# pinellolab/CRISPR-HAWK

Measured on AMD Instinct MI355X. Metric: candidate guides scored/sec, higher is better.
Workload: dtype u32

## Files before the change

### crispr-hawk_amd/crisprhawk_hip/_lib.py

```python

import ctypes as C
import os
from typing import Optional

_HERE = os.path.dirname(os.path.abspath(__file__))
LIB_PATH = os.environ.get("CRISPRHAWK_HIP_LIB", os.path.join(_HERE, "libhawk_hip.so"))

HAWK_OK = 0
HAWK_E_INVALID = -1
HAWK_E_HIP = -2
HAWK_E_CAPACITY = -3
HAWK_E_IUPAC = -4
HAWK_E_CFD = -5
HAWK_E_NODEVICE = -6
HAWK_E_UNSUPPORTED = -7
HAWK_E_COMM = -8
HAWK_E_OVERLAP = -9
HAWK_E_CLAMP = -10

EXPORTS = [
    "hawk_device_count", "hawk_init", "hawk_destroy", "hawk_strerror", "hawk_last_hip_error", "hawk_stream",
    "hawk_sync", "hawk_hapset_create", "hawk_hapset_destroy", "hawk_hapset_pack_ascii", "hawk_hapset_set_meta",
    "hawk_hapset_stride", "hawk_hapset_download_plane", "hawk_hapset_upload_planes", "hawk_pam_scan", "hawk_pam_scan_time",
    "hawk_search", "hawk_table_destroy", "hawk_table_counts", "hawk_table_download", "hawk_table_device_columns", "hawk_table_layout", "hawk_table_download_rows", "hawk_table_device_rows", "hawk_cfd",
    "hawk_genome_finalize", "hawk_offtarget_scan", "hawk_offtarget_summary", "hawk_deepcpf1", "hawk_azimuth", "hawk_tm_nn",
    "hawk_table_collapse", "hawk_table_collapse_download", "hawk_gt_parse", "hawk_gt_destroy", "hawk_gt_codes", "hawk_gt_lists",
    "hawk_gt_lists_download", "hawk_gt_lists_indels", "hawk_release_cached_memory", "hawk_xplan_run", "hawk_xplan_view", "hawk_xplan_cluster_stats", "hawk_xplan_cluster_rebuild", "hawk_host_gather_plan", "hawk_xplan_create_gt", "hawk_xplan_rows",
    "hawk_xplan_finish_meta", "hawk_xplan_segments", "hawk_xplan_install_meta", "hawk_host_alloc", "hawk_host_free", "hawk_hapset_rows_equal",
    "hawk_xplan_destroy", "hawk_hapset_set_ref_partner_range", "hawk_xplan_set_ref_partner_range", "hawk_table_collapse_ex", "hawk_table_collapse_export", "hawk_comm_unique_id", "hawk_comm_init",
    "hawk_comm_destroy", "hawk_comm_last_error", "hawk_comm_allgather_u64", "hawk_comm_gatherv", "hawk_table_gather", "hawk_host_ragged_join", "hawk_host_tsv_write", "hawk_host_vcf_index", "hawk_host_polish_rows", "hawk_host_variant_window", "hawk_host_polish_windows", "hawk_host_group_join", "hawk_host_group_samples", "hawk_gbt_predict", "hawk_gt_from_codes",
    "hawk_annot_create", "hawk_annot_query", "hawk_annot_download", "hawk_annot_free", "hawk_xplan_text",
]


class HawkLibraryError(RuntimeError):
    """libhawk_hip.so is missing or does not export the C ABI — build it (python -c
    'import __graft_entry__ as g; g.build()' or make -C crispr-hawk_amd/csrc)."""


class HawkDeviceError(RuntimeError):
    """No MI355X visible / HIP failure.  There is deliberately no CPU path."""


class HawkCommError(RuntimeError):
    """RCCL failure (or librccl.so missing) in the multi-GPU exchange."""


class HawkStatusError(RuntimeError):
    def __init__(self, status: int, where: str, detail: str = ""):
        self.status = status
        super().__init__(f"{where}: {strerror(status)} (status {status}){': ' + detail if detail else ''}")


class SearchParams(C.Structure):
    _fields_ = [
        ("pam_fwd", C.c_uint64), ("pam_rev", C.c_uint64), ("pamlen", C.c_uint32), ("guidelen", C.c_uint32),
        ("right", C.c_uint32), ("score_cfdon", C.c_uint32), ("cfd_mm", C.c_void_p), ("cfd_pam", C.c_void_p),
    ]


class Timing(C.Structure):
    _fields_ = [
        ("count_ms", C.c_float), ("offsets_ms", C.c_float), ("emit_ms", C.c_float), ("total_ms", C.c_float),
        ("scanned_positions", C.c_uint64), ("emit_list_ms", C.c_float), ("v_count_ms", C.c_float), ("v_emit_ms", C.c_float),
        ("v_templates_ms", C.c_float), ("v_path", C.c_uint32), ("v_emit_rows_ms", C.c_float), ("reserved", C.c_float),
    ]


class GbtModel(C.Structure):
    _fields_ = [("n_trees", C.c_uint32), ("n_nodes", C.c_uint32), ("tree_off", C.c_void_p), ("feature", C.c_void_p),
                ("left", C.c_void_p), ("right", C.c_void_p), ("threshold", C.c_void_p), ("value", C.c_void_p),
                ("init", C.c_double), ("learning_rate", C.c_double)]


class OtParams(C.Structure):
    _fields_ = [("pam_fwd", C.c_uint64), ("pam_rev", C.c_uint64), ("pamlen", C.c_uint32), ("guidelen", C.c_uint32),
                ("right", C.c_uint32), ("max_mm", C.c_uint32)]


class AnnotTiming(C.Structure):
    _fields_ = [("upload_ms", C.c_float), ("count_ms", C.c_float), ("scan_ms", C.c_float), ("fill_ms", C.c_float),
                ("reserved", C.c_float), ("total_ms", C.c_float), ("out_bytes", C.c_uint64), ("walk_steps", C.c_uint64)]


class OtTiming(C.Structure):
    _fields_ = [("scan_ms", C.c_float), ("sites_ms", C.c_float), ("match_ms", C.c_float), ("total_ms", C.c_float),
                ("n_sites", C.c_uint64), ("scanned_positions", C.c_uint64)]


_lib: Optional[C.CDLL] = None
_ctx = {}


def lib() -> C.CDLL:
    global _lib
    if _lib is None:
        if not os.path.exists(LIB_PATH):
            raise HawkLibraryError(f"{LIB_PATH} not found: the HIP extension has not been built")
        try:
            L = C.CDLL(LIB_PATH)
        except OSError as e:
            raise HawkLibraryError(f"cannot load {LIB_PATH}: {e}") from e
        missing = [s for s in EXPORTS if not hasattr(L, s)]
        if missing:
            raise HawkLibraryError(f"{LIB_PATH} lacks symbols {missing}")
        L.hawk_strerror.restype = C.c_char_p
        L.hawk_last_hip_error.restype = C.c_char_p
        L.hawk_stream.restype = C.c_void_p
        L.hawk_destroy.restype = None
        L.hawk_hapset_destroy.restype = None
# ... 112 lines not shown
```

### crispr-hawk_amd/crisprhawk_hip/hapset.py

```python

import ctypes as C
from dataclasses import dataclass
from typing import List, Optional, Sequence, Tuple

import numpy as np

from . import _lib

GUIDESEQPAD = 10
_CODE2CHAR = np.frombuffer(b"?ACMGRSVTWYHKDBN?acmgrsvtwyhkdbn", dtype=np.uint8)


def _p(a: Optional[np.ndarray]):
    return None if a is None else a.ctypes.data_as(C.c_void_p)


def _as_u8(seq) -> np.ndarray:
    if isinstance(seq, np.ndarray):
        return seq if seq.dtype == np.uint8 else seq.astype(np.uint8)
    if isinstance(seq, str):
        seq = seq.encode("ascii")
    return np.frombuffer(seq, dtype=np.uint8)


# ... 132 lines not shown
        nf, nr = int(off_f[-1]), int(off_r[-1])
        hf = np.empty(max(nf, 1), dtype=np.uint32)
        hr = np.empty(max(nr, 1), dtype=np.uint32)
        if rc == _lib.HAWK_E_CAPACITY:
            _lib.check(L.hawk_pam_scan(self._h, C.c_uint64(pam_bits), C.c_uint64(pam_bitsrc), pamlen, _p(hf), _p(hr),
                                       C.c_uint64(len(hf)), C.c_uint64(len(hr)), _p(off_f), _p(off_r)), "hawk_pam_scan")
        return [(hf[int(off_f[h]):int(off_f[h + 1])].copy(), hr[int(off_r[h]):int(off_r[h + 1])].copy())
                for h in range(self.n_hap)]

    def search(self, pam_bits: int, pam_bitsrc: int, pamlen: int, guidelen: int, right: bool,
               cfd_mm: Optional[np.ndarray] = None, cfd_pam: Optional[np.ndarray] = None,
               download: bool = True, collapse: bool = False, cfd_na_on_ambiguous: bool = False) -> "GuideTable":
        L = self._L
        sp = _lib.SearchParams()
        sp.pam_fwd, sp.pam_rev, sp.pamlen, sp.guidelen, sp.right = pam_bits, pam_bitsrc, pamlen, guidelen, int(bool(right))
        keep = []
        if cfd_mm is not None:
            mm = np.ascontiguousarray(cfd_mm, dtype=np.float64).reshape(20, 4, 4)
            pt = np.ascontiguousarray(cfd_pam, dtype=np.float64).reshape(16)
            keep = [mm, pt]
            sp.score_cfdon, sp.cfd_mm, sp.cfd_pam = (2 if cfd_na_on_ambiguous else 1), mm.ctypes.data, pt.ctypes.data
        t = C.c_void_p()
        tm = _lib.Timing()
        _lib.check(L.hawk_search(self._h, C.byref(sp), C.byref(t), C.byref(tm)), "hawk_search")
        del keep
        self.last_timing = tm
        tab = GuideTable(self, t, guidelen, pamlen, bool(right), tm)
        if collapse:
            tab.collapse()
        if download:
            tab.download()
        return tab


class ExpansionPlan:

    def __init__(self, handle, hap_len: np.ndarray, device: Optional[int] = None):
        self._L = _lib.lib()
        self._x = handle
        self.hap_len = np.asarray(hap_len, dtype=np.uint32)
        self.n_hap = len(self.hap_len)
        self.device = device
        self.ref_index = -1
        self.is_ref = None

    def run(self, want_hash: bool = False, timed: bool = False):
        handle = C.c_void_p()
        hashes = np.zeros((self.n_hap, 2), dtype=np.uint64) if want_hash else None
        ms = C.c_float(0)
        _lib.check(self._L.hawk_xplan_run(self._x, C.byref(handle), _p(hashes), C.byref(ms) if (timed or want_hash) else None),
                   "hawk_xplan_run")
        ds = DeviceHapSet.from_handle(handle, self.hap_len, self.device)
        ds.ref_index, ds.is_ref = self.ref_index, self.is_ref
        return ds, hashes, (ms.value if (timed or want_hash) else None)

    def view(self) -> "DeviceHapSet":
        v = getattr(self, "_view", None)
        if v is None or v._h is None:
            handle = C.c_void_p()
            _lib.check(self._L.hawk_xplan_view(self._x, C.byref(handle)), "hawk_xplan_view")
            v = DeviceHapSet.from_handle(handle, self.hap_len, self.device)
            v.ref_index, v.is_ref = self.ref_index, self.is_ref
            v._plan_ref = self
            for k in ("alias", "host_meta"):
                if hasattr(self, k):
                    setattr(v, k, getattr(self, k))
            self._view = v
        return v

    def text(self, rows=None, timed: bool = False):
        rows = np.arange(self.n_hap, dtype=np.uint32) if rows is None else np.ascontiguousarray(rows, dtype=np.uint32).reshape(-1)
        if len(rows) and int(rows.max()) >= self.n_hap:
            raise IndexError(f"row {int(rows.max())} of a plan of {self.n_hap} rows")
        off = np.zeros(len(rows) + 1, dtype=np.uint64)
        np.cumsum(self.hap_len[rows], dtype=np.uint64, out=off[1:])
        buf = _lib.pinned_empty(int(off[-1]), np.uint8, self.device)
        ms = C.c_float(0)
        _lib.check(self._L.hawk_xplan_text(self._x, len(rows), _p(rows), _p(off), _p(buf), C.byref(ms) if timed else None), "hawk_xplan_text")
        return (buf, off, ms.value) if timed else (buf, off)

    def rebuild_dictionary(self) -> None:
        _lib.check(self._L.hawk_xplan_cluster_rebuild(self._x), "hawk_xplan_cluster_rebuild")

    def cluster_stats(self) -> dict:
        u, ni, nd, st = C.c_uint32(), C.c_uint32(), C.c_uint32(), C.c_uint32()
        slots, ms = C.c_uint64(), C.c_float()
        _lib.check(self._L.hawk_xplan_cluster_stats(self._x, C.byref(u), C.byref(ni), C.byref(nd), C.byref(slots), C.byref(ms), C.byref(st)),
                   "hawk_xplan_cluster_stats")
        return {"usable": bool(u.value), "instances": ni.value, "distinct": nd.value, "template_slots": slots.value, "build_ms": ms.value,
                "status": st.value}

    def close(self) -> None:
        v = getattr(self, "_view", None)
        if v is not None:
            v._plan_ref = None
            v.close()
            self._view = None
        if getattr(self, "_x", None):
            self._L.hawk_xplan_destroy(self._x)
            self._x = None

    def __del__(self):
        try:
            self.close()
        except Exception:
            pass


def _meta_arrays(haps: Sequence["HostHaplotype"]):
    n = len(haps)
    is_ref = np.array([1 if h.is_ref else 0 for h in haps], dtype=np.uint8)
    ss = np.array([h.scan[0] for h in haps], dtype=np.int32)
    se = np.array([h.scan[1] for h in haps], dtype=np.int32)
    seg_off = np.zeros(n + 1, dtype=np.uint32)
    seg_off[1:] = np.cumsum([len(h.seg.rel) for h in haps])
    seg_rel = np.concatenate([h.seg.rel for h in haps]).astype(np.uint32)
    seg_gen = np.concatenate([h.seg.gen for h in haps]).astype(np.int64)
    refs = np.flatnonzero(is_ref)
    return is_ref, ss, se, seg_off, seg_rel, seg_gen, (int(refs[0]) if len(refs) else -1)


class GroupTable:

    def __init__(self, guidelen: int, pamlen: int, right: bool, n_groups: int, n_rows: int, device: Optional[int] = None):
        self.guidelen, self.pamlen, self.right, self.n_groups, self.n_rows = guidelen, pamlen, right, n_groups, n_rows
        ng = n_groups

        def pe(n, dt):
            return _lib.pinned_empty(n, dt, device)
        self.rep_row = pe(ng, np.uint32); self.pos = pe(ng, np.uint32); self.strand = np.empty(ng, np.uint8)
        self.start = pe(ng, np.int64); self.stop = pe(ng, np.int64); self.flags = np.empty(ng, np.uint8)
        self.cfdon = pe(ng, np.float64); self.win = pe(5 * ng, np.uint64).reshape(5, ng)
        self.member_hap = pe(n_rows, np.uint32)
        self.member_off = np.zeros(ng + 1, np.int64)
        self.gc_num = np.zeros(ng, np.uint8); self.gc_den = np.zeros(ng, np.uint8)

    @property
    def window_len(self) -> int:
        return self.guidelen + self.pamlen + 2 * GUIDESEQPAD

    def windows(self, rows: Optional[np.ndarray] = None) -> List[str]:
        return decode_windows(self.win if rows is None else self.win[:, rows], self.window_len)


def decode_windows(win: np.ndarray, W: int) -> List[str]:
    n = win.shape[1]
    if n == 0:
        return []
    sh = np.arange(W, dtype=np.uint64)
    code = np.zeros((n, W), dtype=np.uint8)
    for p in range(5):
        code |= (((win[p][:, None] >> sh) & np.uint64(1)).astype(np.uint8) << p)
    raw = _CODE2CHAR[code].tobytes()
    return [raw[i * W:(i + 1) * W].decode("ascii") for i in range(n)]


class GuideTable:

    def __init__(self, hs: DeviceHapSet, handle, guidelen: int, pamlen: int, right: bool, timing):
        self._hs, self._t = hs, handle
        self.guidelen, self.pamlen, self.right = guidelen, pamlen, right
        self._timing_struct = timing
        self.timing = {k: getattr(timing, k) for k, _ in timing._fields_}
        n, c, h = C.c_uint64(), C.c_uint64(), C.c_uint64()
        _lib.check(hs._L.hawk_table_counts(handle, C.byref(n), C.byref(c), C.byref(h)), "hawk_table_counts")
        self.n_rows, self.n_candidates, self.n_hits = n.value, c.value, h.value
# ... 101 lines not shown
```

### crispr-hawk_amd/csrc/hawk_api.hip

```cpp
#include <hip/hip_runtime.h>

#include <algorithm>
#include <cmath>
#include <cstdio>
#include <cstdlib>
#include <cstring>
#include <map>
#include <mutex>
#include <new>
#include <unordered_map>
#include <vector>

#include "hawk_host.h"

static thread_local char g_hip_err[256] = "";
char* hawk_hip_err_buf() { return g_hip_err; }

namespace {
struct DevPool {
  std::multimap<size_t, void*> free_;
  std::unordered_map<void*, size_t> live_;
  size_t cached = 0;
};
DevPool g_pool[HAWK_MAX_DEVICES];
// ... 34 lines not shown
    (void)hipGetLastError();
    pool_trim_locked(P);
    e = hipMalloc(p, want);
  }
  if (e != hipSuccess) {
    snprintf(g_hip_err, sizeof(g_hip_err), "hipMalloc(%zu bytes): %s", want, hipGetErrorString(e));
    *p = nullptr;
    return HAWK_E_HIP;
  }
  P->live_[*p] = want;
  return HAWK_OK;
}

void hawk_pool_free(void* p) {
  if (!p) return;
  std::lock_guard<std::mutex> g(g_pool_mu);
  for (int d = 0; d < HAWK_MAX_DEVICES; ++d) {
    DevPool* P = &g_pool[d];
    auto it = P->live_.find(p);
    if (it == P->live_.end()) continue;
    const size_t sz = it->second;
    P->live_.erase(it);
    if (P->cached + sz > pool_cap()) { (void)hipFree(p); return; }
    P->free_.emplace(sz, p);
    P->cached += sz;
    return;
  }
  (void)hipFree(p);
}

void hawk_pool_trim() {
  std::lock_guard<std::mutex> g(g_pool_mu);
  if (DevPool* P = cur_pool()) pool_trim_locked(P);
}

extern "C" {

const char* hawk_strerror(int s) {
  switch (s) {
    case HAWK_OK: return "ok";
    case HAWK_E_INVALID: return "invalid argument";
    case HAWK_E_HIP: return "HIP runtime error";
    case HAWK_E_CAPACITY: return "output capacity too small";
    case HAWK_E_IUPAC: return "non-IUPAC character in sequence";
    case HAWK_E_CFD: return "non-ACGT base under a CFD table lookup";
    case HAWK_E_NODEVICE: return "no GPU device visible";
    case HAWK_E_UNSUPPORTED: return "parameter outside supported range";
    case HAWK_E_COMM: return "RCCL failure";
    case HAWK_E_OVERLAP: return "a chromosome copy carries overlapping variants";
    case HAWK_E_CLAMP: return "variant beyond the original region length";
    default: return "unknown status";
  }
}
const char* hawk_last_hip_error(void) { return g_hip_err; }

int hawk_device_count(int* n) {
  int c = 0;
  hipError_t e = hipGetDeviceCount(&c);
  if (e != hipSuccess) { c = 0; (void)hipGetLastError(); }
  if (n) *n = c;
  return HAWK_OK;
}

namespace {
hawk_ctx* g_ctx_of[HAWK_MAX_DEVICES] = {};
int g_ctx_refs[HAWK_MAX_DEVICES] = {};
std::mutex g_ctx_mu;
}

int hawk_init(int device, hawk_ctx** out) {
  if (!out) return HAWK_E_INVALID;
  int c = 0;
  hawk_device_count(&c);
  if (c <= 0) return HAWK_E_NODEVICE;
  if (device < 0 || device >= c || device >= HAWK_MAX_DEVICES) return HAWK_E_INVALID;
  std::lock_guard<std::mutex> g(g_ctx_mu);
  if (g_ctx_of[device]) { ++g_ctx_refs[device]; *out = g_ctx_of[device]; return HAWK_OK; }
  HIPCHK(hipSetDevice(device));
  hawk_ctx* ctx = new (std::nothrow) hawk_ctx();
  if (!ctx) return HAWK_E_INVALID;
  ctx->device = device;
  HIPCHK(hipStreamCreateWithFlags(&ctx->stream, hipStreamNonBlocking));
  for (auto& e : ctx->ev) HIPCHK(hipEventCreate(&e));
  HIPCHK(hipHostMalloc(&ctx->pinned, 256, hipHostMallocDefault));
  g_ctx_of[device] = ctx; g_ctx_refs[device] = 1;
  *out = ctx;
  return HAWK_OK;
}

void hawk_destroy(hawk_ctx* ctx) {
  if (!ctx) return;
  {
    std::lock_guard<std::mutex> g(g_ctx_mu);
    const int d = ctx->device;
    if (d >= 0 && d < HAWK_MAX_DEVICES && g_ctx_of[d] == ctx) {
      if (--g_ctx_refs[d] > 0) return;
      g_ctx_of[d] = nullptr;
    }
  }
  (void)hipSetDevice(ctx->device);
  (void)hipStreamSynchronize(ctx->stream);
  for (auto& e : ctx->ev) (void)hipEventDestroy(e);
  (void)hipStreamDestroy(ctx->stream);
  if (ctx->pinned) (void)hipHostFree(ctx->pinned);
  delete ctx;
}

int hawk_host_alloc(hawk_ctx* ctx, uint64_t bytes, void** out) {
  if (!ctx || !out) return HAWK_E_INVALID;
  HIPCHK(hipSetDevice(ctx->device));
  HIPCHK(hipHostMalloc(out, std::max<uint64_t>(bytes, 1), hipHostMallocDefault));
  return HAWK_OK;
}
void hawk_host_free(void* p) { if (p) (void)hipHostFree(p); }

void* hawk_stream(hawk_ctx* ctx) { return ctx ? (void*)ctx->stream : nullptr; }
int hawk_sync(hawk_ctx* ctx) {
  if (!ctx) return HAWK_E_INVALID;
  HIPCHK(hipStreamSynchronize(ctx->stream));
  return HAWK_OK;
}

int hawk_release_cached_memory(hawk_ctx* ctx) {
  if (!ctx) return HAWK_E_INVALID;
  HIPCHK(hipSetDevice(ctx->device));
  HIPCHK(hipStreamSynchronize(ctx->stream));
  hawk_pool_trim();
  return HAWK_OK;
}

}
```

### crispr-hawk_amd/csrc/hawk_api_collapse.hip

```cpp
#include <hip/hip_runtime.h>

#include <algorithm>
#include <cmath>
#include <cstdio>
#include <cstdlib>
#include <cstring>
#include <map>
#include <mutex>
#include <new>
#include <unordered_map>
#include <vector>

#include "hawk_host.h"

extern "C" {

static int collapse_rows(hawk_table* t, uint32_t flank_up, uint32_t flank_down, uint64_t* n_groups, float* kernel_ms);
static int collapse_by_templates(hawk_table* t, uint32_t flank_up, uint32_t flank_down, uint64_t* n_groups, float* kernel_ms);
int hawk_table_collapse_ex(hawk_table* t, uint32_t flank_up, uint32_t flank_down, uint64_t* n_groups, float* kernel_ms) {
  if (!t || !n_groups || !t->hs || hawk_table_stale(t)) return HAWK_E_INVALID;
  if (flank_up > HAWK_PAD || flank_down > HAWK_PAD) return HAWK_E_UNSUPPORTED;
  if (t->by_cluster && t->n_rows) return collapse_by_templates(t, flank_up, flank_down, n_groups, kernel_ms);
  return collapse_rows(t, flank_up, flank_down, n_groups, kernel_ms);
}
// ... 46 lines not shown
          (rc = hs->ccnt.reserve(32)))
        return rc;
      for (int attempt = 0; attempt < 2; ++attempt) {
        unsigned long long hc[4] = {0, 0, 0, 0};
        HIPCHK(hipMemsetAsync(hs->ccnt.p, 0, 32, ctx->stream));
        HIPCHK(hipEventRecord(ctx->ev[0], ctx->stream));
        if (hawk_launch_collapse_hash1(ctx->stream, t->cols, hs->d_is_ref, n, (int)t->guidelen, (int)t->pamlen, (int)flank_up, (int)flank_down,
                                       hs->min_gen, 0x9e3779b97f4a7c15ull * (uint64_t)(attempt + 1), hs->ctemp.p, tb, hs->ctable.p, (uint32_t)C,
                                       hs->cocc.as<uint32_t>(), hs->cdense.as<uint32_t>(), hs->cgkey.as<uint64_t>(), hs->cgslot.as<uint32_t>(),
                                       hs->cflags.as<uint32_t>(), hs->ccnt.as<unsigned long long>()))
          return HAWK_E_HIP;
        HIPCHK(hipGetLastError());
        HIPCHK(hipMemcpyAsync(hc, hs->ccnt.p, 24, hipMemcpyDeviceToHost, ctx->stream));
        HIPCHK(hipStreamSynchronize(ctx->stream));
        if (hc[1]) { hs->last_groups = n; if (hs->plan_groups) *hs->plan_groups = n; break; }
        if (hc[0]) continue;
        const uint64_t ng = hc[2];
        if (hawk_launch_collapse_hash2(ctx->stream, t->cols, n, (uint32_t)ng, (int)t->guidelen, (int)t->pamlen, (int)t->right, end_bit, hs->ctemp.p, tb,
                                       hs->cgkey.as<uint64_t>(), hs->cgslot.as<uint32_t>(), (uint32_t)C, hs->cocc.as<uint32_t>(),
                                       hs->cflags.as<uint32_t>(), hs->ckeys.as<uint32_t>(), hs->cvals.as<uint32_t>(), hs->cgoff.as<uint64_t>(),
                                       hs->cgc.as<uint8_t>(), hs->cgc.as<uint8_t>() + n))
          return HAWK_E_HIP;
        if (verify) {
          if ((rc = hs->cfull.reserve(ng * 64 + 64))) return rc;
          hawk_launch_collapse_verify_rows(ctx->stream, t->cols, hs->d_is_ref, n, (uint32_t)ng, (int)t->guidelen, (int)t->pamlen, (int)flank_up,
                                           (int)flank_down, hs->cvals.as<uint32_t>() + n, hs->cflags.as<uint32_t>(), hs->cocc.as<uint32_t>(),
                                           hs->cgoff.as<uint64_t>(), hs->cfull.p, hs->ccnt.as<unsigned long long>() + 3);
        }
        HIPCHK(hipEventRecord(ctx->ev[1], ctx->stream));
        HIPCHK(hipGetLastError());
        HIPCHK(hipMemcpyAsync(hs->cgoff.as<uint64_t>() + ng, &n, 8, hipMemcpyHostToDevice, ctx->stream));
        HIPCHK(hipMemcpyAsync(&hc[3], hs->ccnt.as<unsigned long long>() + 3, 8, hipMemcpyDeviceToHost, ctx->stream));
        HIPCHK(hipStreamSynchronize(ctx->stream));
        if (kernel_ms) { float ms = 0.f; (void)hipEventElapsedTime(&ms, ctx->ev[0], ctx->ev[1]); *kernel_ms += ms; }
        if (hc[3]) { verified_bad = true; break; }
        hs->last_groups = ng;
        if (hs->plan_groups) *hs->plan_groups = ng;
        t->n_groups = ng; t->collapsed = true;
        *n_groups = ng;
        return HAWK_OK;
      }
    }
  }
  if (verified_bad) continue;
  unsigned long long cnt[3] = {0, 0, 0};
  for (int attempt = 0; attempt < 4; ++attempt) {
    HIPCHK(hipMemsetAsync(hs->ccnt.p, 0, 32, ctx->stream));
    HIPCHK(hipEventRecord(ctx->ev[0], ctx->stream));
    if (hawk_launch_collapse(ctx->stream, t->cols, hs->d_is_ref, n, (int)t->guidelen, (int)t->pamlen, (int)t->right, (int)flank_up,
                             (int)flank_down, hs->min_gen, exact ? 0u : begin_bit, end_bit, 0x9e3779b97f4a7c15ull * (uint64_t)(attempt + 1), hs->ctemp.p,
                             temp_bytes, hs->ckeys.as<uint64_t>(), hs->cvals.as<uint32_t>(), hs->cflags.as<uint32_t>(),
                             hs->cgidx.as<uint32_t>(), hs->ccnt.as<unsigned long long>(), hs->cgoff.as<uint64_t>(), hs->cgc.as<uint8_t>(),
                             hs->cgc.as<uint8_t>() + n, hs->cgidx.as<uint32_t>(), exact ? hs->cfull.p : nullptr, weak && !exact))
      return HAWK_E_HIP;
    if (verify && !exact)
      hawk_launch_collapse_verify(ctx->stream, t->cols, hs->d_is_ref, n, (int)t->guidelen, (int)t->pamlen, (int)flank_up, (int)flank_down,
                                  hs->cvals.as<uint32_t>() + n, hs->cgidx.as<uint32_t>(), hs->cflags.as<uint32_t>(), hs->cgoff.as<uint64_t>(),
                                  hs->ccnt.as<unsigned long long>() + 2);
    HIPCHK(hipEventRecord(ctx->ev[1], ctx->stream));
    HIPCHK(hipGetLastError());
    HIPCHK(hipMemcpyAsync(cnt, hs->ccnt.p, 24, hipMemcpyDeviceToHost, ctx->stream));
    HIPCHK(hipStreamSynchronize(ctx->stream));
    if (kernel_ms) { float ms = 0.f; (void)hipEventElapsedTime(&ms, ctx->ev[0], ctx->ev[1]); *kernel_ms += ms; }
    if (cnt[0] == cnt[1]) break;
  }
  if (cnt[0] != cnt[1]) { if (!exact) continue; return HAWK_E_UNSUPPORTED; }
  if (cnt[2]) continue;
  const uint64_t ng = cnt[1];
  HIPCHK(hipMemcpyAsync(hs->cgoff.as<uint64_t>() + ng, &n, 8, hipMemcpyHostToDevice, ctx->stream));
  HIPCHK(hipStreamSynchronize(ctx->stream));
  hs->last_groups = ng;
  if (hs->plan_groups) *hs->plan_groups = ng;
  t->n_groups = ng; t->collapsed = true;
  *n_groups = ng;
  return HAWK_OK;
  }
  return HAWK_E_UNSUPPORTED;
}

static int collapse_by_templates(hawk_table* t, uint32_t flank_up, uint32_t flank_down, uint64_t* n_groups, float* kernel_ms) {
  hawk_hapset* hs = t->hs;
  hawk_ctx* ctx = hs->ctx;
  HIPCHK(hipSetDevice(ctx->device));
  const hawk_xplan* vx = hs->vplan;
  if (!vx || !vx->cl.usable) return HAWK_E_INVALID;
  const uint64_t n = t->n_rows;
  if (n > 0xffffffffull) return HAWK_E_UNSUPPORTED;
  t->collapsed = false;
  *n_groups = 0;
  if (kernel_ms) *kernel_ms = 0.f;
  const uint32_t nu = vx->cl.n_uniq;
  PoolScope tmp;
  uint32_t* d_ucnt;
  uint64_t* d_moff;
  unsigned long long *d_partial, *d_shards;
  ScanTotals* d_tot;
  TEMPCHK(tmp, &d_ucnt, (size_t)std::max<uint32_t>(nu, 1) * 4);
  TEMPCHK(tmp, &d_moff, ((size_t)nu + 2) * 8);
  TEMPCHK(tmp, &d_partial, ((size_t)nu / 1024 + 2) * 8);
  TEMPCHK(tmp, &d_shards, 512 * 8);
  TEMPCHK(tmp, &d_tot, sizeof(ScanTotals));
  HIPCHK(hipMemsetAsync(d_shards, 0, 512 * 8, ctx->stream));
  HIPCHK(hipMemsetAsync(d_tot, 0, sizeof(ScanTotals), ctx->stream));
  uint64_t r0 = 0;
  ScanTotals tot;
  memset(&tot, 0, sizeof(tot));
  if (nu) {
    hawk_launch_cc_ucnt(ctx->stream, hs->cs_res.p, nu, d_ucnt);
    hawk_launch_mscan(ctx->stream, d_ucnt, nu, d_partial, d_shards, d_moff, d_tot);
    HIPCHK(hipMemcpyAsync(&tot, d_tot, sizeof(tot), hipMemcpyDeviceToHost, ctx->stream));
  }
  HIPCHK(hipMemcpyAsync(&r0, hs->offsets.as<uint64_t>() + t->plane_tiles, 8, hipMemcpyDeviceToHost, ctx->stream));
  HIPCHK(hipStreamSynchronize(ctx->stream));
  HIPCHK(hipGetLastError());
  const uint64_t t_live = tot.n_keep;
  const uint64_t nm = r0 + t_live;
  if (r0 > n || nm == 0 || nm > 0xffffffffull || r0 + 0 > n) return HAWK_E_INVALID;
  int rc;
  GuideCols mini;
  if ((rc = hawk_reserve_cols(hs->cmini, nm, &mini)) || (rc = hs->cm_gid.reserve(nm * 4))) return rc;
  float ms_a = 0.f, ms_b = 0.f, ms_c = 0.f;
  HIPCHK(hipEventRecord(ctx->ev[8], ctx->stream));
  hawk_launch_cc_mini(ctx->stream, t->cols, r0, hs->cs_trows.p, t_live, d_moff, hs->cs_tbase.as<uint32_t>(), nu, hs->ref_startp, mini);
  HIPCHK(hipEventRecord(ctx->ev[9], ctx->stream));
  HIPCHK(hipGetLastError());
  {
    const size_t tb_full = hawk_collapse_expand_temp_bytes(n);
    if ((rc = hs->ckeys.reserve(std::max<size_t>(2 * nm * 8, 2 * n * 4))) || (rc = hs->cvals.reserve(2 * n * 4)) ||
        (rc = hs->cgoff.reserve((nm + 1) * 8)) || (rc = hs->cgc.reserve(2 * n)) || (rc = hs->ctemp.reserve(tb_full + 16)) ||
        (rc = hs->cflags.reserve(n * 4)))
      return rc;
  }
  hawk_table tm;
  tm.hs = hs; tm.ctx = ctx; tm.n_rows = nm; tm.n_cand = tm.n_hits = 0; tm.cap = mini.cap; tm.cols = mini;
  tm.guidelen = t->guidelen; tm.pamlen = t->pamlen; tm.right = t->right; tm.n_groups = 0; tm.collapsed = false; tm.gen = t->gen;
  uint64_t G = 0;
  if ((rc = collapse_rows(&tm, flank_up, flank_down, &G, &ms_b))) return rc;
  HIPCHK(hipStreamSynchronize(ctx->stream));
  (void)hipEventElapsedTime(&ms_a, ctx->ev[8], ctx->ev[9]);
  unsigned gbits = 1;
  while (gbits < 32 && (G >> gbits) != 0) ++gbits;
  const size_t tb = hawk_collapse_expand_temp_bytes(n);
  HIPCHK(hipEventRecord(ctx->ev[8], ctx->stream));
  hawk_launch_cc_gidm(ctx->stream, hs->cvals.as<uint32_t>() + nm, hs->cgoff.as<uint64_t>(), nm, G, hs->cm_gid.as<uint32_t>());
  if ((rc = hs->ckeys.reserve(2 * n * 4)) || (rc = hs->cvals.reserve(2 * n * 4)) || (rc = hs->cgoff.reserve((std::max<uint64_t>(G, nm) + 1) * 8)) ||
      (rc = hs->cgc.reserve(2 * n)) || (rc = hs->ctemp.reserve(tb + 16)) || (rc = hs->cflags.reserve(n * 4)))
    return rc;
  ClDict cd;
  memset(&cd, 0, sizeof(cd));
  cd.n_inst = vx->cl.n_inst; cd.n_uniq = vx->cl.n_uniq; cd.inst_uid = vx->cl.inst_uid.as<uint32_t>();
  hawk_launch_cs_gid(ctx->stream, cd, hs->cs_res.p, d_moff, hs->offsets.as<uint64_t>() + t->plane_tiles, r0, n,
                     hs->cm_gid.as<uint32_t>(), hs->ckeys.as<uint32_t>(), hs->cvals.as<uint32_t>());
  if (hawk_launch_collapse_expand(ctx->stream, t->cols, n, gbits, (int)t->guidelen, (int)t->pamlen, (int)t->right, hs->ctemp.p, tb, hs->ckeys.as<uint32_t>(),
                                  hs->cvals.as<uint32_t>(), hs->cgoff.as<uint64_t>(), hs->cgc.as<uint8_t>(), hs->cgc.as<uint8_t>() + n))
    return HAWK_E_HIP;
  HIPCHK(hipMemcpyAsync(hs->cgoff.as<uint64_t>() + G, &n, 8, hipMemcpyHostToDevice, ctx->stream));
  HIPCHK(hipEventRecord(ctx->ev[9], ctx->stream));
  HIPCHK(hipGetLastError());
  HIPCHK(hipStreamSynchronize(ctx->stream));
  (void)hipEventElapsedTime(&ms_c, ctx->ev[8], ctx->ev[9]);
  if (kernel_ms) *kernel_ms = ms_a + ms_b + ms_c;
  hs->collapse_gen = t->gen;
  hs->last_groups = G;
  if (hs->plan_groups) *hs->plan_groups = G;
  t->n_groups = G; t->collapsed = true;
  *n_groups = G;
  return HAWK_OK;
// ... 62 lines not shown
```

### crispr-hawk_amd/csrc/hawk_api_search.hip

```cpp
#include <hip/hip_runtime.h>

#include <algorithm>
#include <cmath>
#include <cstdio>
#include <cstdlib>
#include <cstring>
#include <map>
#include <mutex>
#include <new>
#include <unordered_map>
#include <vector>

#include "hawk_host.h"

int hawk_reserve_cols(DevBuf (&b)[8], uint64_t cap, GuideCols* c) {
  int rc;
  const size_t sz[8] = {cap * 4, cap * 4, cap, cap * 8, cap * 8, cap, cap * 8, cap * 8 * HAWK_PLANES};
  for (int i = 0; i < 8; ++i) if ((rc = b[i].reserve(std::max<size_t>(sz[i], 16)))) return rc;
  c->hap = b[0].as<uint32_t>(); c->pos = b[1].as<uint32_t>(); c->strand = b[2].as<uint8_t>();
  c->start = b[3].as<int64_t>(); c->stop = b[4].as<int64_t>(); c->flags = b[5].as<uint8_t>();
  c->cfdon = b[6].as<double>(); c->win = b[7].as<uint64_t>(); c->cap = cap;
  c->rows = nullptr; c->startp = 0;
  return HAWK_OK;
}

#define HAWK_RETRY_TEMPLATES (-100)

enum SearchEvent {
  EV_BEGIN, EV_COUNT_DONE, EV_OFFSETS_DONE, EV_EMIT_BEGIN, EV_EMIT_END, EV_LIST_EMIT_END,
  EV_VIEW_COUNT_BEGIN, EV_VIEW_EMIT_BEGIN,
  EV_TEMPLATES_DONE, EV_REF_ROWS_PACKED,
  EV_SLOTS
};
static_assert(EV_SLOTS == sizeof(hawk_ctx::ev) / sizeof(hipEvent_t), "hawk_ctx::ev holds exactly the search's events");

struct SearchRun {
  hawk_hapset* hs; hawk_ctx* ctx; hipStream_t st;
  const hawk_xplan* vx;
  bool by_cluster;
  HapSetDev d; ScanParams sp; GuideParams gp; RefInfo ri; VcArgs va; ClDict cd;
  uint64_t ntile, nscan;
  uint32_t plane_tiles, v_tiles;
  uint64_t tcap, t_rows_used;
  uint64_t stage_cap;
  unsigned long long* shards;
  SearchStatusBlock* blk;
  SearchStatusBlock* h;
  uint64_t* table_cap;
};

static int search_classify(hawk_hapset* hs, const hawk_search_params* p, SearchRun* r) {
  if (!hs || !p || !hs->has_meta || p->score_cfdon > 2) return HAWK_E_INVALID;
  if (p->score_cfdon && (p->right || !p->cfd_mm || !p->cfd_pam || p->pamlen < 2)) return HAWK_E_INVALID;
  r->hs = hs; r->ctx = hs->ctx; r->st = hs->ctx->stream; r->vx = hs->vplan;
  HIPCHK(hipSetDevice(r->ctx->device));
  const int rc = make_scan_params(hs, p->pam_fwd, p->pam_rev, p->pamlen, p->guidelen, p->right, true, &r->sp);
  if (rc) return rc;
  r->d = make_dev(hs);
  ++hs->cols_gen;
  const hawk_xplan* vx = r->vx;
  if (vx && (hs->ref_index != 0 || hs->n_ref_rows != 1)) return HAWK_E_INVALID;
  r->by_cluster = vx && vx->cl.built && vx->cl.usable;
  if (r->by_cluster) { const char* e = getenv("HAWK_VIEW_SEARCH"); if (e && e[0] == 'w') r->by_cluster = false; }
  r->ntile = (uint64_t)hs->n_hap * r->sp.bph;
  r->nscan = r->by_cluster ? (uint64_t)r->sp.bph + ((uint64_t)vx->cl.n_inst + 63) / 64 : r->ntile;
  r->plane_tiles = vx ? r->sp.bph : (uint32_t)r->ntile;
  r->v_tiles = (uint32_t)r->ntile - r->plane_tiles;
  r->stage_cap = r->by_cluster ? 2ull * hs->hap_len[hs->ref_index] + 64 : 0;
  r->table_cap = r->by_cluster ? &hs->rows_cap : &hs->cols_cap;
  r->tcap = r->t_rows_used = 0;
  return HAWK_OK;
}
static int search_reserve(SearchRun* r, const hawk_search_params* p) {
  hawk_hapset* hs = r->hs;
  const ScanParams& sp = r->sp;
  const uint64_t n_ref_tiles = (uint64_t)sp.bph * hs->n_ref_rows;
  int rc;
  if ((rc = hs->counts.reserve(r->nscan * 4)) || (rc = hs->offsets.reserve((r->nscan + 1) * 8)) || (rc = hs->misc.reserve(sizeof(SearchMisc))) ||
      (rc = hs->cfd.reserve(336 * 8)) || (rc = hs->partial.reserve((r->nscan / 1024 + 2) * 8)) ||
      (rc = hs->lists.reserve((size_t)r->plane_tiles * HAWK_LIST_CAP * 4 + 16)) || (rc = hs->big.reserve(((size_t)r->plane_tiles + 128 * n_ref_tiles) * 8 + 16)))
    return rc;
  r->shards = &hs->misc.as<SearchMisc>()->shards[0][0];
  r->blk = &hs->misc.as<SearchMisc>()->blk;
  r->h = static_cast<SearchStatusBlock*>(r->ctx->pinned);
  GuideParams& gp = r->gp;
  gp.pamlen = sp.pamlen; gp.guidelen = sp.guidelen; gp.right = sp.right; gp.L = sp.L;
  gp.score_cfdon = (int32_t)p->score_cfdon;
  gp.cfd_mm = hs->cfd.as<double>(); gp.cfd_pam = hs->cfd.as<double>() + 320; gp.bph = sp.bph;
  return HAWK_OK;
}
static int search_upload_cfd(SearchRun* r, const hawk_search_params* p) {
  hawk_hapset* hs = r->hs;
  if (!p->score_cfdon) return HAWK_OK;
  if (hs->cfd_host.size() == 336 && memcmp(hs->cfd_host.data(), p->cfd_mm, 320 * 8) == 0 && memcmp(hs->cfd_host.data() + 320, p->cfd_pam, 16 * 8) == 0) return HAWK_OK;
  hs->cfd_host.assign(336, 0.0);
  memcpy(hs->cfd_host.data(), p->cfd_mm, 320 * 8);
  memcpy(hs->cfd_host.data() + 320, p->cfd_pam, 16 * 8);
  HIPCHK(hipMemcpyAsync(hs->cfd.p, hs->cfd_host.data(), 336 * 8, hipMemcpyHostToDevice, r->st));
  HIPCHK(hipStreamSynchronize(r->st));
  return HAWK_OK;
}
static int search_ref(SearchRun* r, const hawk_search_params* p) {
  hawk_hapset* hs = r->hs;
  const ScanParams& sp = r->sp;
  RefInfo& ri = r->ri;
  ri.index = hs->ref_index; ri.startp = hs->ref_startp;
  ri.bits[0] = ri.bits[1] = nullptr; ri.n_bits = 0;
  for (int s = 0; s < 2; ++s) {
    ri.lo[s] = 0; ri.hi[s] = 0;
    if (hs->ref_index < 0) continue;
    const bool pamfirst = (sp.right != 0) != (s != 0);
    const int po = pamfirst ? 0 : sp.guidelen;
    const int haplen = (int)hs->hap_len[hs->ref_index];
    const int rs = hs->has_partner ? hs->partner_start : hs->scan_start[hs->ref_index];
    const int re = hs->has_partner ? hs->partner_stop : hs->scan_stop[hs->ref_index];
    ri.lo[s] = std::max(rs - po, HAWK_PAD);
    ri.hi[s] = std::min(re - po, haplen - sp.L - HAWK_PAD + 1);
  }
  if (hs->ref_index < 0) return HAWK_OK;
  const uint64_t key[6] = {p->pam_fwd, p->pam_rev, ((uint64_t)p->pamlen << 32) | p->guidelen, (uint64_t)(p->right ? 1 : 0),
                           ((uint64_t)(uint32_t)ri.lo[0] << 32) | (uint32_t)ri.hi[0], ((uint64_t)(uint32_t)ri.lo[1] << 32) | (uint32_t)ri.hi[1]};
  int rc;
  if ((rc = hs->refbits.reserve((size_t)hs->S * 4 * 2))) return rc;
  ri.bits[0] = hs->refbits.as<uint32_t>(); ri.bits[1] = hs->refbits.as<uint32_t>() + hs->S;
  ri.n_bits = hs->S * 32u;
  if (r->vx && ((rc = hs->refhp.reserve(((size_t)hs->S + 1) * 8 * 2)) || (rc = hs->vcnt0.reserve(r->by_cluster ? 16 : r->ntile * 4)))) return rc;
  if (hs->refbits_valid && memcmp(hs->refbits_key, key, sizeof(key)) == 0) return HAWK_OK;
  hawk_launch_ref_bits(r->st, r->d, sp, ri, hs->refbits.as<uint32_t>(), hs->refbits.as<uint32_t>() + hs->S);
  if (r->vx) hawk_launch_ref_hits(r->st, r->d, sp, hs->ref_index, hs->refhp.p);
  HIPCHK(hipGetLastError());
  memcpy(hs->refbits_key, key, sizeof(key));
  hs->refbits_valid = true;
  return HAWK_OK;
}
static int search_view_args(SearchRun* r) {
  hawk_hapset* hs = r->hs;
  const hawk_xplan* vx = r->vx;
  VcArgs& va = r->va; ClDict& cd = r->cd;
  memset(&va, 0, sizeof(va)); memset(&cd, 0, sizeof(cd));
  if (!vx) return HAWK_OK;
  for (int pl = 0; pl < 4; ++pl) va.ref[pl] = vx->ref5[pl].as<uint32_t>();
  va.ref_S = hs->S; va.hp = hs->refhp.as<uint4>();
  va.recs_ = vx->recs.p; va.alt_codes = vx->codes.as<uint8_t>(); va.hv_off = vx->off.as<uint64_t>(); va.tiles_ = vx->tiles.p;
  if (!r->by_cluster) return HAWK_OK;
  const auto& cl = vx->cl;
  cd.n_inst = cl.n_inst; cd.n_uniq = cl.n_uniq;
  cd.inst_uid = cl.inst_uid.as<uint32_t>(); cd.inst_o = cl.inst_o.as<int32_t>(); cd.inst_row = cl.inst_row.as<uint32_t>();
  cd.inst_pa = cl.inst_pa.as<int32_t>(); cd.inst_rb = cl.inst_rb.as<int32_t>();
  cd.u_rec = cl.u_rec.as<uint32_t>(); cd.u_n = cl.u_n.as<uint32_t>(); cd.u_row = cl.u_row.as<uint32_t>(); cd.u_o = cl.u_o.as<int32_t>();
  cd.u_seg = cl.u_seg.as<uint32_t>();
  const char* e0 = getenv("HAWK_CLUSTER_ROWS0");
  const uint64_t first = e0 ? strtoull(e0, nullptr, 10) : 16ull * cl.n_uniq + 65536;
  r->tcap = std::max<uint64_t>(std::min<uint64_t>(cl.slots, std::max<uint64_t>(hs->cs_tcap, first)), 1);
  const size_t n_uniq = std::max<uint32_t>(cl.n_uniq, 1), n_inst = std::max<uint32_t>(cl.n_inst, 1);
  int rc;
  if ((rc = hs->cs_res.reserve(n_uniq * 32)) || (rc = hs->cs_tbase.reserve(n_uniq * 4)) || (rc = hs->cs_trows.reserve((size_t)r->tcap * hawk_cs_row_bytes())) ||
      (rc = hs->cs_itb.reserve(n_inst * 4)) || (rc = hs->cs_icnt.reserve(n_inst * 4)))
    return rc;
  return HAWK_OK;
}
static int search_count(SearchRun* r) {
  hawk_hapset* hs = r->hs; hipStream_t st = r->st; hipEvent_t* ev = r->ctx->ev;
  SearchStatusBlock* blk = r->blk; uint32_t* counts = hs->counts.as<uint32_t>();
  HIPCHK(hipEventRecord(ev[EV_BEGIN], st));
  hawk_launch_search(st, 0, r->d, r->sp, r->gp, r->ri, hs->d_tile_meta, counts, r->shards, nullptr, GuideCols{}, &blk->status, hs->lists.as<uint32_t>(),
                     &blk->big_count, hs->big.as<unsigned long long>(), nullptr, r->plane_tiles);
  if (r->vx) HIPCHK(hipEventRecord(ev[EV_VIEW_COUNT_BEGIN], st));
  if (r->by_cluster) {
    hawk_launch_cs_templates(st, r->d, r->va, r->cd, r->sp, r->gp, r->ri, hs->cs_res.p, hs->cs_tbase.as<uint32_t>(), hs->cs_trows.p, &blk->template_rows,
                             r->tcap, &blk->status);
    (void)hipEventRecord(ev[EV_TEMPLATES_DONE], st);
    hawk_launch_cs_count(st, r->d, r->va, r->cd, r->sp, hs->cs_res.p, &blk->template_rows, r->tcap, counts + r->plane_tiles, hs->cs_icnt.as<uint32_t>(),
                         hs->cs_itb.as<uint32_t>(), r->shards);
  } else if (r->vx) {
    hawk_launch_vsearch(st, 0, r->d, r->va, r->sp, r->gp, r->ri, hs->d_tile_meta, counts, hs->vcnt0.as<uint32_t>(), r->shards, nullptr, GuideCols{}, &blk->status,
                        r->plane_tiles, r->v_tiles);
  }
  HIPCHK(hipEventRecord(ev[EV_COUNT_DONE], st));
  hawk_launch_mscan(st, counts, r->nscan, hs->partial.as<unsigned long long>(), r->shards, hs->offsets.as<uint64_t>(), &blk->totals);
  HIPCHK(hipEventRecord(ev[EV_OFFSETS_DONE], st));
  HIPCHK(hipGetLastError());
  return HAWK_OK;
}
static int search_reserve_table(SearchRun* r, uint64_t cap, GuideCols* cols, GuideCols* table) {
  hawk_hapset* hs = r->hs;
  int rc;
  if ((rc = hawk_reserve_cols(hs->colsA, r->by_cluster ? r->stage_cap : cap, cols))) return rc;
  *table = *cols;
  if (!r->by_cluster) return HAWK_OK;
  if ((rc = hs->rowsA.reserve(cap * 64))) return rc;
  memset(table, 0, sizeof(*table));
  table->rows = hs->rowsA.as<uint4>(); table->cap = cap; table->startp = r->ri.startp;
  return HAWK_OK;
}
static int search_emit(SearchRun* r, const GuideCols& cols, const GuideCols& packed, bool launch) {
  hawk_hapset* hs = r->hs; hipStream_t st = r->st; hipEvent_t* ev = r->ctx->ev;
  SearchStatusBlock* blk = r->blk; const uint64_t* offsets = hs->offsets.as<uint64_t>();
  HIPCHK(hipEventRecord(ev[EV_EMIT_BEGIN], st));
  if (launch) {
    hawk_launch_search(st, 1, r->d, r->sp, r->gp, r->ri, hs->d_tile_meta, hs->counts.as<uint32_t>(), r->shards, offsets, cols, &blk->status, hs->lists.as<uint32_t>(),
                       &blk->big_count, hs->big.as<unsigned long long>(), ev[EV_LIST_EMIT_END], r->plane_tiles);
    if (r->vx) (void)hipEventRecord(ev[EV_VIEW_EMIT_BEGIN], st);
    if (r->by_cluster) {
      hawk_launch_rows_pack(st, cols, offsets + r->plane_tiles, 0, std::min<uint64_t>(r->stage_cap, packed.cap), packed.rows, packed.startp, &blk->status);
      (void)hipEventRecord(ev[EV_REF_ROWS_PACKED], st);
      hawk_launch_cs_emit_rows(st, r->cd, hs->cs_icnt.as<uint32_t>(), hs->cs_itb.as<uint32_t>(), hs->cs_trows.p, offsets + r->plane_tiles, &blk->template_rows,
                               r->tcap, packed.rows, packed.cap, &blk->status);
    } else if (r->vx) {
      hawk_launch_vsearch(st, 1, r->d, r->va, r->sp, r->gp, r->ri, hs->d_tile_meta, hs->counts.as<uint32_t>(), hs->vcnt0.as<uint32_t>(), r->shards, offsets, cols,
                          &blk->status, r->plane_tiles, r->v_tiles);
    }
  }
  HIPCHK(hipEventRecord(ev[EV_EMIT_END], st));
  HIPCHK(hipGetLastError());
  return HAWK_OK;
}
static int search_read_block(SearchRun* r) {
  HIPCHK(hipMemcpyAsync(r->h, r->blk, sizeof(SearchStatusBlock), hipMemcpyDeviceToHost, r->st));
  HIPCHK(hipStreamSynchronize(r->st));
  if (!r->by_cluster) return HAWK_OK;
  const uint64_t tcu = r->h->template_rows;
  if (tcu > r->tcap) { r->hs->cs_tcap = std::min<uint64_t>(r->vx->cl.slots, tcu + tcu / 8 + 64); return HAWK_RETRY_TEMPLATES; }
  r->t_rows_used = tcu;
  return HAWK_OK;
}

static void search_timing(const SearchRun* r, uint64_t nrows, hawk_timing* timing) {
  const hawk_hapset* hs = r->hs; hipEvent_t* ev = r->ctx->ev;
  memset(timing, 0, sizeof(*timing));
  (void)hipEventElapsedTime(&timing->count_ms, ev[EV_BEGIN], ev[EV_COUNT_DONE]);
  (void)hipEventElapsedTime(&timing->offsets_ms, ev[EV_COUNT_DONE], ev[EV_OFFSETS_DONE]);
  (void)hipEventElapsedTime(&timing->emit_ms, ev[EV_EMIT_BEGIN], ev[EV_EMIT_END]);
  if (nrows) (void)hipEventElapsedTime(&timing->emit_list_ms, ev[EV_EMIT_BEGIN], ev[EV_LIST_EMIT_END]);
  (void)hipEventElapsedTime(&timing->total_ms, ev[EV_BEGIN], ev[EV_EMIT_END]);
  if (r->vx) {
    (void)hipEventElapsedTime(&timing->v_count_ms, ev[EV_VIEW_COUNT_BEGIN], ev[EV_COUNT_DONE]);
    if (nrows) (void)hipEventElapsedTime(&timing->v_emit_ms, ev[EV_VIEW_EMIT_BEGIN], ev[EV_EMIT_END]);
    timing->v_path = r->by_cluster ? 2u : 1u;
    if (r->by_cluster) (void)hipEventElapsedTime(&timing->v_templates_ms, ev[EV_VIEW_COUNT_BEGIN], ev[EV_TEMPLATES_DONE]);
    if (r->by_cluster && nrows) (void)hipEventElapsedTime(&timing->v_emit_rows_ms, ev[EV_REF_ROWS_PACKED], ev[EV_EMIT_END]);
  }
  uint64_t pos = 0;
  for (uint32_t h = 0; h < hs->n_hap; ++h) pos += (uint64_t)std::max(0, hs->scan_stop[h] - hs->scan_start[h]);
  timing->scanned_positions = pos;
}

static int search_make_table(const SearchRun* r, const hawk_search_params* p, const GuideCols& tc, hawk_table** out) {
  hawk_table* t = new (std::nothrow) hawk_table();
  if (!t) return HAWK_E_INVALID;
  const ScanTotals& tot = r->h->totals;
  t->hs = r->hs; t->ctx = r->ctx; t->gen = r->hs->cols_gen;
  t->n_rows = tot.n_keep; t->n_cand = tot.n_cand; t->n_hits = tot.n_hits; t->cols = tc; t->cap = tc.cap;
  t->guidelen = p->guidelen; t->pamlen = p->pamlen; t->right = p->right ? 1 : 0; t->n_groups = 0; t->collapsed = false;
  t->by_cluster = r->by_cluster; t->plane_tiles = r->plane_tiles; t->t_rows = r->by_cluster ? r->t_rows_used : 0;
  *out = t;
  return HAWK_OK;
}

static int hawk_search_once(hawk_hapset* hs, const hawk_search_params* p, hawk_table** out, hawk_timing* timing) {
  if (!out) return HAWK_E_INVALID;
  SearchRun r;
  int rc;
  if ((rc = search_classify(hs, p, &r)) || (rc = search_reserve(&r, p)) || (rc = search_upload_cfd(&r, p))) return rc;
  HIPCHK(hipMemsetAsync(r.hs->misc.p, 0, sizeof(SearchMisc), r.st));
  if ((rc = search_ref(&r, p)) || (rc = search_view_args(&r)) || (rc = search_count(&r))) return rc;
  uint64_t& table_cap = *r.table_cap;
  const bool speculative = table_cap != 0;
  GuideCols cols, table;
  if (speculative && ((rc = search_reserve_table(&r, table_cap, &cols, &table)) || (rc = search_emit(&r, cols, table, true)))) return rc;
  if ((rc = search_read_block(&r))) return rc;
  const uint64_t nrows = r.h->totals.n_keep;
  if (!speculative || nrows > table_cap) {
    const int status = r.h->status;
    if (status && !(speculative && status == HAWK_E_CAPACITY)) return status;
    if (speculative) HIPCHK(hipMemsetAsync(&r.blk->status, 0, sizeof(int), r.st));
    if ((rc = search_reserve_table(&r, std::max<uint64_t>(std::max<uint64_t>(nrows, 1), table_cap), &cols, &table))) return rc;
    table_cap = table.cap;
    if ((rc = search_emit(&r, cols, table, nrows != 0))) return rc;
    HIPCHK(hipMemcpyAsync(&r.h->status, &r.blk->status, sizeof(int), hipMemcpyDeviceToHost, r.st));
    HIPCHK(hipStreamSynchronize(r.st));
  }
  if (timing) search_timing(&r, nrows, timing);
  if (r.h->status) return r.h->status;
  return search_make_table(&r, p, table, out);
}

extern "C" {

int hawk_search(hawk_hapset* hs, const hawk_search_params* p, hawk_table** out, hawk_timing* timing) {
  int rc = hawk_search_once(hs, p, out, timing);
  if (rc == HAWK_RETRY_TEMPLATES) rc = hawk_search_once(hs, p, out, timing);
  return rc == HAWK_RETRY_TEMPLATES ? HAWK_E_CAPACITY : rc;
}

void hawk_table_destroy(hawk_table* t) {
  if (!t) return;
  if (!t->hs) {
    (void)hipSetDevice(t->ctx->device);
    (void)hipStreamSynchronize(t->ctx->stream);
    for (auto& b : t->own) b.release();
  }
  delete t;
}

int hawk_table_counts(const hawk_table* t, uint64_t* n_rows, uint64_t* n_candidates, uint64_t* n_hits) {
  if (!t) return HAWK_E_INVALID;
  if (n_rows) *n_rows = t->n_rows;
  if (n_candidates) *n_candidates = t->n_cand;
  if (n_hits) *n_hits = t->n_hits;
  return HAWK_OK;
}

int hawk_table_download(hawk_table* t, uint32_t* hap, uint32_t* pos, uint8_t* strand, int64_t* start, int64_t* stop,
                        uint8_t* flags, double* cfdon, uint64_t* win) {
  if (!t || hawk_table_stale(t)) return HAWK_E_INVALID;
  hawk_ctx* ctx = t->ctx;
  HIPCHK(hipSetDevice(ctx->device));
  const uint64_t n = t->n_rows;
  if (!n) return HAWK_OK;
  GuideCols c = t->cols;
  PoolScope tmp;
  if (c.rows) {
    GuideCols u;
    memset(&u, 0, sizeof(u));
    u.cap = n;
    if (hap) TEMPCHK(tmp, &u.hap, n * 4);
    if (pos) TEMPCHK(tmp, &u.pos, n * 4);
    if (strand) TEMPCHK(tmp, &u.strand, n);
    if (start) TEMPCHK(tmp, &u.start, n * 8);
    if (stop) TEMPCHK(tmp, &u.stop, n * 8);
    if (flags) TEMPCHK(tmp, &u.flags, n);
    if (cfdon) TEMPCHK(tmp, &u.cfdon, n * 8);
    if (win) TEMPCHK(tmp, &u.win, n * 8 * HAWK_PLANES);
    hawk_launch_rows_unpack(ctx->stream, c.rows, n, c.startp, u);
    HIPCHK(hipGetLastError());
    c = u;
  }
  if (hap) HIPCHK(hipMemcpyAsync(hap, c.hap, n * 4, hipMemcpyDefault, ctx->stream));
  if (pos) HIPCHK(hipMemcpyAsync(pos, c.pos, n * 4, hipMemcpyDefault, ctx->stream));
  if (strand) HIPCHK(hipMemcpyAsync(strand, c.strand, n, hipMemcpyDefault, ctx->stream));
  if (start) HIPCHK(hipMemcpyAsync(start, c.start, n * 8, hipMemcpyDefault, ctx->stream));
  if (stop) HIPCHK(hipMemcpyAsync(stop, c.stop, n * 8, hipMemcpyDefault, ctx->stream));
  if (flags) HIPCHK(hipMemcpyAsync(flags, c.flags, n, hipMemcpyDefault, ctx->stream));
  if (cfdon) HIPCHK(hipMemcpyAsync(cfdon, c.cfdon, n * 8, hipMemcpyDefault, ctx->stream));
  if (win)
    for (int p = 0; p < HAWK_PLANES; ++p)
      HIPCHK(hipMemcpyAsync(win + (size_t)p * n, c.win + (size_t)p * c.cap, n * 8, hipMemcpyDefault, ctx->stream));
  HIPCHK(hipStreamSynchronize(ctx->stream));
  return HAWK_OK;
}

int hawk_table_layout(const hawk_table* t, uint32_t* layout, int64_t* startp) {
  if (!t || !layout) return HAWK_E_INVALID;
  *layout = t->cols.rows ? HAWK_LAYOUT_ROWS : HAWK_LAYOUT_COLUMNS;
  if (startp) *startp = t->cols.rows ? t->cols.startp : 0;
  return HAWK_OK;
}

int hawk_table_download_rows(hawk_table* t, void* rows64) {
  if (!t || hawk_table_stale(t) || !rows64) return HAWK_E_INVALID;
  if (!t->cols.rows) return HAWK_E_UNSUPPORTED;
  HIPCHK(hipSetDevice(t->ctx->device));
  if (t->n_rows) HIPCHK(hipMemcpyAsync(rows64, t->cols.rows, t->n_rows * 64, hipMemcpyDefault, t->ctx->stream));
  HIPCHK(hipStreamSynchronize(t->ctx->stream));
  return HAWK_OK;
}

int hawk_table_device_rows(hawk_table* t, void** rows64, int64_t* startp) {
  if (!t || hawk_table_stale(t) || !rows64) return HAWK_E_INVALID;
  if (!t->cols.rows) return HAWK_E_UNSUPPORTED;
  *rows64 = t->cols.rows;
  if (startp) *startp = t->cols.startp;
  return HAWK_OK;
}

// ... 19 lines not shown
```

### crispr-hawk_amd/csrc/hawk_api_xplan.hip

```cpp
#include <hip/hip_runtime.h>

#include <algorithm>
#include <cmath>
#include <cstdio>
#include <cstdlib>
#include <cstring>
#include <map>
#include <mutex>
#include <new>
#include <unordered_map>
#include <vector>

#include "hawk_host.h"

enum XplanEvent { EV_KERNELS_BEGIN = 0, EV_KERNELS_END = 1, EV_BUILD_BEGIN = 8, EV_BUILD_END = 9 };

extern "C" {

void hawk_xplan_destroy(hawk_xplan* x) {
  if (!x) return;
  (void)hipSetDevice(x->ctx->device);
  (void)hipStreamSynchronize(x->ctx->stream);
  for (auto& p : x->ref_plane) hawk_pool_free(p);
  for (auto& b : x->ref5) b.release();
  DevBuf* bufs[] = {&x->recs, &x->heads, &x->tiles, &x->codes, &x->off, &x->hlen, &x->hash,
                    &x->m_is_ref, &x->m_ss, &x->m_se, &x->m_seg_off, &x->m_seg_rel, &x->m_seg_gen, &x->m_tile,
                    &x->cl.inst_uid, &x->cl.inst_o, &x->cl.inst_row, &x->cl.inst_pa, &x->cl.inst_rb, &x->cl.u_rec, &x->cl.u_n, &x->cl.u_row,
                    &x->cl.u_o, &x->cl.u_seg};
  for (auto* b : bufs) b->release();
  delete x;
}

static int xplan_build(hawk_hapset* ref_set, uint32_t n_var, const uint32_t* v_r0, const uint32_t* v_span, const uint32_t* v_alt_off,
                       const uint32_t* v_alt_len, const uint8_t* alt_codes, uint32_t alt_codes_len, uint32_t n_hap, const uint64_t* hv_off,
                       const uint32_t* d_idx, const int32_t* d_o, const uint32_t* hap_len, uint32_t maxlen, hawk_xplan** out) {
  hawk_ctx* ctx = ref_set->ctx;
  const uint32_t ref_len = ref_set->hap_len[0];
  const uint64_t ncar = hv_off[n_hap];
  HIPCHK(hipSetDevice(ctx->device));
  hawk_xplan* x = new (std::nothrow) hawk_xplan();
  if (!x) return HAWK_E_INVALID;
  x->ctx = ctx; x->n_var = n_var; x->n_hap = n_hap; x->ref_len = ref_len; x->ncar = ncar;
  x->hap_len.assign(hap_len, hap_len + n_hap);
  x->has_meta = false; x->nseg = 0; x->ref_index = -1; x->ref_startp = 0; x->min_gen = 0; x->max_gen = 0;
  for (auto& p : x->ref_plane) p = nullptr;
  x->ref_S = ref_set->S;
  x->S = ((maxlen + 31) / 32 + 2 + 3) / 4 * 4;
  x->bph = (x->S / 4 + HAWK_BLOCK - 1) / HAWK_BLOCK;
  const size_t nwg = (size_t)n_hap * hawk_hx_tiles_per_row(x->S);
  const size_t nv = std::max<size_t>(n_var, 1), nc = std::max<size_t>(ncar, 1);
  int rc = HAWK_OK;
  for (int p = 0; p < 4 && !rc; ++p) rc = hawk_pool_alloc((void**)&x->ref_plane[p], (size_t)x->ref_S * 4);
  DevBuf t_r0, t_span, t_ao, t_al, t_am;
  DevBuf* temps[] = {&t_r0, &t_span, &t_ao, &t_al, &t_am};
  if (!rc) rc = t_r0.reserve(nv * 4);
  if (!rc) rc = t_span.reserve(nv * 4);
  if (!rc) rc = t_ao.reserve(nv * 4);
  if (!rc) rc = t_al.reserve(nv * 4);
  if (!rc) rc = t_am.reserve(nv * 16);
  if (!rc) rc = x->recs.reserve(nc * hawk_hx_record_bytes());
  if (!rc) rc = x->heads.reserve(nc * 16);
  if (!rc) rc = x->tiles.reserve(nwg * hawk_hx_tile_bytes());
  if (!rc) rc = x->codes.reserve(std::max<size_t>(alt_codes_len, 1));
  if (!rc) rc = x->off.reserve((size_t)(n_hap + 1) * 8);
  if (!rc) rc = x->hlen.reserve((size_t)n_hap * 4);
  if (!rc) rc = x->hash.reserve((size_t)n_hap * 16);
  for (int p = 0; p < HAWK_PLANES && !rc; ++p) rc = x->ref5[p].reserve((size_t)x->S * 4);
  if (rc) { for (auto* b : temps) b->release(); hawk_xplan_destroy(x); return rc; }
  hipStream_t st = ctx->stream;
  hipError_t e = hipSuccess;
  for (int p = 0; p < HAWK_PLANES && e == hipSuccess; ++p) {
    e = hipMemsetAsync(x->ref5[p].p, 0, (size_t)x->S * 4, st);
    if (p < 4 && e == hipSuccess)
      e = hipMemcpyAsync(x->ref5[p].p, ref_set->plane[p], (size_t)std::min(x->S, x->ref_S) * 4, hipMemcpyDeviceToDevice, st);
  }
  std::vector<uint32_t> am(nv * 4, 0);
  for (uint32_t i = 0; i < n_var; ++i)
    for (uint32_t j = 0; j < v_alt_len[i] && j < 32; ++j) {
      const uint8_t c = alt_codes[v_alt_off[i] + j];
      for (int pl = 0; pl < 4; ++pl) am[(size_t)i * 4 + pl] |= (uint32_t)((c >> pl) & 1u) << j;
    }
  for (int p = 0; p < 4 && e == hipSuccess; ++p)
    e = hipMemcpyAsync(x->ref_plane[p], ref_set->plane[p], (size_t)x->ref_S * 4, hipMemcpyDeviceToDevice, st);
  if (n_var && e == hipSuccess) {
    e = hipMemcpyAsync(t_r0.p, v_r0, (size_t)n_var * 4, hipMemcpyHostToDevice, st);
    if (e == hipSuccess) e = hipMemcpyAsync(t_span.p, v_span, (size_t)n_var * 4, hipMemcpyHostToDevice, st);
    if (e == hipSuccess) e = hipMemcpyAsync(t_ao.p, v_alt_off, (size_t)n_var * 4, hipMemcpyHostToDevice, st);
    if (e == hipSuccess) e = hipMemcpyAsync(t_al.p, v_alt_len, (size_t)n_var * 4, hipMemcpyHostToDevice, st);
    if (e == hipSuccess) e = hipMemcpyAsync(x->codes.p, alt_codes, alt_codes_len, hipMemcpyHostToDevice, st);
    if (e == hipSuccess) e = hipMemcpyAsync(t_am.p, am.data(), (size_t)n_var * 16, hipMemcpyHostToDevice, st);
  }
  if (e == hipSuccess) e = hipMemcpyAsync(x->off.p, hv_off, (size_t)(n_hap + 1) * 8, hipMemcpyHostToDevice, st);
  if (e == hipSuccess) e = hipMemcpyAsync(x->hlen.p, hap_len, (size_t)n_hap * 4, hipMemcpyHostToDevice, st);
  if (e == hipSuccess) {
    hawk_launch_hx_prepare(st, x->off.as<uint64_t>(), d_idx, d_o, ncar, t_r0.as<uint32_t>(), t_span.as<uint32_t>(), t_ao.as<uint32_t>(),
                           t_al.as<uint32_t>(), t_am.p, x->hlen.as<uint32_t>(), n_hap, x->S, x->recs.p, x->tiles.p);
    hawk_launch_hx_heads(st, x->recs.p, d_idx, ncar, x->heads.p);
    e = hipGetLastError();
  }
  if (e == hipSuccess) e = hipStreamSynchronize(st);
  for (auto* b : temps) b->release();
  if (e != hipSuccess) {
    snprintf(hawk_hip_err_buf(), 256, "hawk_xplan_create_gt: %s", hipGetErrorString(e));
    hawk_xplan_destroy(x);
    return HAWK_E_HIP;
  }
  *out = x;
  return HAWK_OK;
}

int hawk_xplan_set_ref_partner_range(hawk_xplan* x, int32_t start, int32_t stop) {
  if (!x || !x->has_meta || x->ref_index < 0) return HAWK_E_INVALID;
  if (start < 0 || stop > (int32_t)x->hap_len[x->ref_index] || stop < start) return HAWK_E_INVALID;
  x->has_partner = true; x->partner_start = start; x->partner_stop = stop;
  return HAWK_OK;
}

static int xplan_install(const hawk_xplan* x, hawk_hapset* hs) {
  if (!x->has_meta || hs->n_hap != x->n_hap || hs->S != x->S) return HAWK_E_INVALID;
  hipStream_t st = x->ctx->stream;
  const uint32_t n = x->n_hap;
  hawk_pool_free(hs->d_seg_rel); hs->d_seg_rel = nullptr;
  hawk_pool_free(hs->d_seg_gen); hs->d_seg_gen = nullptr;
  int rc = hawk_pool_alloc((void**)&hs->d_seg_rel, (size_t)x->nseg * 4);
  if (!rc) rc = hawk_pool_alloc((void**)&hs->d_seg_gen, (size_t)x->nseg * 8);
  if (rc) return rc;
  HIPCHK(hipMemcpyAsync(hs->d_is_ref, x->m_is_ref.p, n, hipMemcpyDeviceToDevice, st));
  HIPCHK(hipMemcpyAsync(hs->d_scan_start, x->m_ss.p, (size_t)n * 4, hipMemcpyDeviceToDevice, st));
  HIPCHK(hipMemcpyAsync(hs->d_scan_stop, x->m_se.p, (size_t)n * 4, hipMemcpyDeviceToDevice, st));
  HIPCHK(hipMemcpyAsync(hs->d_seg_off, x->m_seg_off.p, (size_t)(n + 1) * 4, hipMemcpyDeviceToDevice, st));
  HIPCHK(hipMemcpyAsync(hs->d_seg_rel, x->m_seg_rel.p, (size_t)x->nseg * 4, hipMemcpyDeviceToDevice, st));
  HIPCHK(hipMemcpyAsync(hs->d_seg_gen, x->m_seg_gen.p, (size_t)x->nseg * 8, hipMemcpyDeviceToDevice, st));
  HIPCHK(hipMemcpyAsync(hs->d_tile_meta, x->m_tile.p, (size_t)n * x->bph * sizeof(TileMeta), hipMemcpyDeviceToDevice, st));
  hs->ref_startp = x->ref_startp; hs->min_gen = x->min_gen; hs->max_gen = x->max_gen;
  hs->scan_start = x->scan_start; hs->scan_stop = x->scan_stop;
  hs->ref_index = x->ref_index; hs->has_meta = true; hs->n_ref_rows = x->n_ref_rows;
  hs->plan_groups = x->groups; hs->last_groups = *x->groups;
  hs->has_partner = x->has_partner; hs->partner_start = x->partner_start; hs->partner_stop = x->partner_stop;
  hs->refbits_valid = false;
  ++hs->cols_gen;
  return HAWK_OK;
}

int hawk_xplan_run(hawk_xplan* x, hawk_hapset** out, uint64_t* hash_out, float* kernel_ms) {
  if (!x || !out) return HAWK_E_INVALID;
  hawk_ctx* ctx = x->ctx;
  hawk_hapset* hs = nullptr;
  int rc = hapset_create_impl(ctx, x->n_hap, x->hap_len.data(), false, &hs);
  if (rc) return rc;
  if (hs->S != x->S) { hawk_hapset_destroy(hs); return HAWK_E_INVALID; }
  hipStream_t st = ctx->stream;
  hipError_t e = hipMemsetAsync(x->hash.p, 0, (size_t)x->n_hap * 16, st);
  if (e == hipSuccess) e = hipEventRecord(ctx->ev[EV_KERNELS_BEGIN], st);
  if (e == hipSuccess) {
    hawk_launch_hx_build(st, x->ref_plane, x->ref_S, x->recs.p, x->codes.as<uint8_t>(), x->off.as<uint64_t>(), hs->d_hap_len, x->n_hap,
                         hs->S, hs->plane, x->tiles.p);
    if (hash_out) hawk_launch_hx_hash(st, hs->plane, x->n_hap, hs->S, x->hash.as<unsigned long long>());
    e = hipEventRecord(ctx->ev[EV_KERNELS_END], st);
  }
  if (e == hipSuccess) e = hipGetLastError();
  if (e == hipSuccess && hash_out) e = hipMemcpyAsync(hash_out, x->hash.p, (size_t)x->n_hap * 16, hipMemcpyDeviceToHost, st);
  if (e == hipSuccess && x->has_meta) {
    rc = xplan_install(x, hs);
    if (rc) { hawk_hapset_destroy(hs); return rc; }
  }
  if (e == hipSuccess && (hash_out || kernel_ms)) e = hipStreamSynchronize(st);
  if (e != hipSuccess) {
    snprintf(hawk_hip_err_buf(), 256, "hawk_xplan_run: %s", hipGetErrorString(e));
    hawk_hapset_destroy(hs);
    return HAWK_E_HIP;
  }
  if (kernel_ms) (void)hipEventElapsedTime(kernel_ms, ctx->ev[EV_KERNELS_BEGIN], ctx->ev[EV_KERNELS_END]);
  *out = hs;
  return HAWK_OK;
}

static int xplan_build_dict(hawk_xplan* x) {
  auto& cl = x->cl;
  if (cl.built) return HAWK_OK;
  cl.built = true; cl.usable = false; cl.status = 0; cl.n_inst = cl.n_uniq = cl.n_real = 0; cl.slots = 0; cl.build_ms = 0.f;
  hawk_ctx* ctx = x->ctx;
  hipStream_t st = ctx->stream;
  const uint32_t n = x->n_hap;
  if (x->ncar == 0 || x->ncar >= (1ull << 32) - 2 || n < 2) { cl.status = 4; return HAWK_OK; }
  PoolScope tmp;
  const uint32_t n_var = x->n_var;
  const uint32_t ch_bound = hawk_cl_chunk_bound(x->ncar, n);
  const uint32_t inst_bound = (uint32_t)x->ncar + n;
  const uint32_t bm_words = n_var / 32 + 1;
  uint32_t tsize = 1024;
  while (tsize < 2u * inst_bound && tsize < (1u << 30)) tsize <<= 1;
  uint32_t tsmall = std::min<uint32_t>(1u << 16, tsize);
  { const uint64_t expect = cl.last_uniq ? (uint64_t)cl.last_uniq * 2 : (uint64_t)inst_bound / 8; while (tsmall < expect && tsmall < tsize) tsmall <<= 1; }
  const uint32_t u_bound0 = n_var + std::min<uint32_t>(tsmall, inst_bound);
  auto up = [](size_t v) { return (v + 255) & ~(size_t)255; };
  const size_t z_status = 0, z_counters = 256, z_results = 512, z_cnt = 768,
               z_claim = z_cnt + up(((size_t)ch_bound + 4) * 8), z_vdesc = z_claim + up((size_t)bm_words * 4),
               z_span2 = z_vdesc + up((size_t)std::max<uint32_t>(n_var, 1) * 8), z_tab = z_span2 + up((size_t)u_bound0 * 4),
               z_end = z_tab + (size_t)tsmall * hawk_cl_slot_bytes();
  char* d_zero;
  TEMPCHK(tmp, &d_zero, z_end);
  uint32_t* const d_status = reinterpret_cast<uint32_t*>(d_zero + z_status);
  uint32_t* const d_counters = reinterpret_cast<uint32_t*>(d_zero + z_counters);
  unsigned long long* const d_results = reinterpret_cast<unsigned long long*>(d_zero + z_results);
  uint32_t* const d_cnt = reinterpret_cast<uint32_t*>(d_zero + z_cnt);
  uint32_t* const d_lcnt = d_cnt + ((ch_bound + 3) & ~3u);
  uint32_t* const d_claim = reinterpret_cast<uint32_t*>(d_zero + z_claim);
  void* const d_vdesc = d_zero + z_vdesc;
  uint32_t *d_ch_off, *d_ch_row, *d_base, *d_lbase, *d_state;
  void* d_list;
  TEMPCHK(tmp, &d_ch_off, (size_t)(n + 1) * 4);
  TEMPCHK(tmp, &d_ch_row, (size_t)ch_bound * 4);
  TEMPCHK(tmp, &d_base, (size_t)(ch_bound + 1) * 4);
  TEMPCHK(tmp, &d_lbase, (size_t)(ch_bound + 1) * 4);
  TEMPCHK(tmp, &d_list, (size_t)inst_bound * hawk_cl_listed_bytes());
  TEMPCHK(tmp, &d_state, (size_t)inst_bound * 4);
  int rc;
  if ((rc = cl.inst_uid.reserve((size_t)inst_bound * 4)) || (rc = cl.inst_o.reserve((size_t)inst_bound * 4)) ||
      (rc = cl.inst_row.reserve((size_t)inst_bound * 4)) || (rc = cl.inst_pa.reserve((size_t)inst_bound * 4)) ||
      (rc = cl.inst_rb.reserve((size_t)inst_bound * 4)))
    return rc;
  uint32_t* const t_uid = cl.inst_uid.as<uint32_t>();
  uint32_t* const t_row = cl.inst_row.as<uint32_t>();
  int32_t* const t_o = cl.inst_o.as<int32_t>();
  int32_t* const t_pa = cl.inst_pa.as<int32_t>();
  int32_t* const t_rb = cl.inst_rb.as<int32_t>();
  HIPCHK(hipEventRecord(ctx->ev[EV_BUILD_BEGIN], st));
  HIPCHK(hipMemsetAsync(d_zero, 0, z_end, st));
  hawk_launch_cl_chunks(st, x->off.as<uint64_t>(), x->m_is_ref.as<uint8_t>(), x->m_ss.as<int32_t>(), x->m_se.as<int32_t>(), n, d_ch_off, d_ch_row);
  hawk_launch_cl_count(st, x->heads.p, x->off.as<uint64_t>(), x->hlen.as<uint32_t>(), x->m_ss.as<int32_t>(), x->m_se.as<int32_t>(), d_ch_off, d_ch_row, n,
                       n_var, ch_bound, d_cnt, d_lcnt);
  hawk_launch_scan2_u32(st, d_cnt, d_lcnt, ch_bound, d_base, d_lbase);
  const uint32_t* const d_n_inst = d_base + ch_bound;
  const uint32_t* const d_n_list = d_lbase + ch_bound;
  unsigned long long res[8] = {0, 0, 0, 0, 0, 0, 0, 0};
  uint32_t status = 0, n_inst = 0, n_uniq = 0, n_real = 0;
  auto pass = [&](uint32_t tsz, uint32_t max_probe, uint32_t fail_bit, bool first) -> int {
    const uint32_t u_bound = n_var + std::min<uint32_t>(tsz, inst_bound);
    uint32_t* d_span2 = reinterpret_cast<uint32_t*>(d_zero + z_span2);
    void* d_tab = d_zero + z_tab;
    if (!first) {
      TEMPCHK(tmp, &d_span2, (size_t)u_bound * 4);
      TEMPCHK(tmp, &d_tab, (size_t)tsz * hawk_cl_slot_bytes());
      HIPCHK(hipMemsetAsync(d_tab, 0, (size_t)tsz * hawk_cl_slot_bytes(), st));
      HIPCHK(hipMemsetAsync(d_span2, 0, (size_t)u_bound * 4, st));
      HIPCHK(hipMemsetAsync(d_zero + z_counters, 0, z_cnt - z_counters, st));
      HIPCHK(hipMemsetAsync(d_zero + z_claim, 0, z_span2 - z_claim, st));
    }
    int rc2;
    if ((rc2 = cl.u_rec.reserve((size_t)u_bound * 4)) || (rc2 = cl.u_n.reserve((size_t)u_bound * 4)) || (rc2 = cl.u_row.reserve((size_t)u_bound * 4)) ||
        (rc2 = cl.u_o.reserve((size_t)u_bound * 4)) || (rc2 = cl.u_seg.reserve((size_t)u_bound * 4)))
      return rc2;
    hawk_launch_cl_fill(st, x->heads.p, x->off.as<uint64_t>(), x->hlen.as<uint32_t>(), x->m_ss.as<int32_t>(), x->m_se.as<int32_t>(), n, d_ch_off, d_ch_row,
                        ch_bound, d_base, d_lbase, t_o, t_row, t_pa, t_rb, t_uid, d_vdesc, d_claim, n_var, d_list, d_status);
    hawk_launch_cl_finish(st, inst_bound, d_n_inst, d_n_list, d_counters, d_results, n_var, u_bound, d_tab, tsz - 1, max_probe, fail_bit, d_list, d_state, d_vdesc, x->heads.p,
                          t_uid, t_row, x->m_seg_off.as<uint32_t>(), x->m_seg_rel.as<uint32_t>(), cl.u_rec.as<uint32_t>(), cl.u_n.as<uint32_t>(),
                          cl.u_row.as<uint32_t>(), cl.u_o.as<int32_t>(), cl.u_seg.as<uint32_t>(), d_span2, d_status);
    HIPCHK(hipMemcpyAsync(res, d_results, 64, hipMemcpyDeviceToHost, st));
    HIPCHK(hipEventRecord(ctx->ev[EV_BUILD_END], st));
    HIPCHK(hipStreamSynchronize(st));
    HIPCHK(hipGetLastError());
    n_inst = (uint32_t)res[0]; status = (uint32_t)res[4];
    n_uniq = std::min<uint32_t>(n_var + (uint32_t)res[1], u_bound);
    n_real = (uint32_t)(res[1] + res[2]);
    return HAWK_OK;
  };
  if ((rc = pass(tsmall, tsmall < tsize ? 64u : 0xffffffffu, tsmall < tsize ? 8u : 2u, true))) return rc;
  if (status & 8u) {
    status &= ~8u;
    HIPCHK(hipMemcpyAsync(d_status, &status, 4, hipMemcpyHostToDevice, st));
    if ((rc = pass(tsize, 0xffffffffu, 2u, false))) return rc;
  }
  if (n_inst == 0) { cl.status = 4; return HAWK_OK; }
  if (n_inst > inst_bound) { snprintf(hawk_hip_err_buf(), 256, "hawk_xplan_view: instance count beyond its bound"); return HAWK_E_HIP; }
  cl.n_inst = n_inst; cl.n_uniq = n_uniq; cl.n_real = n_real; cl.last_uniq = (uint32_t)res[1];
  (void)hipEventElapsedTime(&cl.build_ms, ctx->ev[EV_BUILD_BEGIN], ctx->ev[EV_BUILD_END]);
  cl.slots = n_uniq ? res[3] : 0;
  cl.status = status;
  const char* e1 = getenv("HAWK_CLUSTER_MAX_SLOTS");
  const char* e2 = getenv("HAWK_CLUSTER_MIN_SHARE");
  const uint64_t max_slots = e1 ? strtoull(e1, nullptr, 10) : (1ull << 27);
  const double min_share = e2 ? atof(e2) : 3.0;
  if (!status && (cl.slots > max_slots || (double)n_inst < min_share * (double)std::max<uint32_t>(n_real, 1))) cl.status = 4;
  cl.usable = cl.status == 0;
  return HAWK_OK;
}

int hawk_xplan_cluster_stats(const hawk_xplan* x, uint32_t* usable, uint32_t* n_instances, uint32_t* n_distinct, uint64_t* template_slots,
                             float* build_ms, uint32_t* status) {
  if (!x) return HAWK_E_INVALID;
  if (usable) *usable = x->cl.built && x->cl.usable ? 1u : 0u;
  if (n_instances) *n_instances = x->cl.n_inst;
  if (n_distinct) *n_distinct = x->cl.n_real;
  if (template_slots) *template_slots = x->cl.slots;
  if (build_ms) *build_ms = x->cl.build_ms;
  if (status) *status = x->cl.built ? x->cl.status : 0xffffffffu;
  return HAWK_OK;
}

int hawk_xplan_cluster_rebuild(hawk_xplan* x) {
  if (!x || !x->has_meta || x->ref_index != 0) return HAWK_E_INVALID;
  HIPCHK(hipSetDevice(x->ctx->device));
  x->cl.built = false;
  return xplan_build_dict(x);
}

int hawk_xplan_view(hawk_xplan* x, hawk_hapset** out) {
  if (!x || !out || !x->has_meta || x->ref_index != 0) return HAWK_E_INVALID;
  hawk_ctx* ctx = x->ctx;
  hawk_hapset* hs = nullptr;
  int rc = hapset_create_impl(ctx, x->n_hap, x->hap_len.data(), false, &hs, false);
  if (rc) return rc;
  if (hs->S != x->S) { hawk_hapset_destroy(hs); return HAWK_E_INVALID; }
  hs->vplan = x;
  for (int p = 0; p < HAWK_PLANES; ++p) hs->plane[p] = x->ref5[p].as<uint32_t>();
  rc = xplan_install(x, hs);
  if (!rc && hipStreamSynchronize(ctx->stream) != hipSuccess) rc = HAWK_E_HIP;
  if (!rc) rc = xplan_build_dict(x);
  if (rc) { hs->vplan = nullptr; for (int p = 0; p < HAWK_PLANES; ++p) hs->plane[p] = nullptr; hawk_hapset_destroy(hs); return rc; }
  *out = hs;
  return HAWK_OK;
}

int hawk_xplan_install_meta(hawk_xplan* x, hawk_hapset* hs) {
  if (!x || !hs || hs->vplan) return HAWK_E_INVALID;
  HIPCHK(hipSetDevice(x->ctx->device));
  int rc = xplan_install(x, hs);
  if (rc) return rc;
  HIPCHK(hipStreamSynchronize(x->ctx->stream));
  return HAWK_OK;
}

int hawk_xplan_create_gt(hawk_hapset* ref_set, hawk_gt* g, uint32_t n_var, const uint32_t* v_r0, const uint32_t* v_span,
                         const uint32_t* v_alt_off, const uint32_t* v_alt_len, const int32_t* v_chain, const uint8_t* alt_codes,
                         uint32_t alt_codes_len, int64_t startp, int check_clamp, int64_t rev_g0, int64_t rev_g1, uint32_t* n_hap_out,
                         hawk_xplan** out) {
  if (!ref_set || !g || !out || !n_hap_out || !g->d_col_off || g->n_var != n_var || !n_var || !v_r0 || !v_span || !v_alt_off || !v_alt_len ||
      !v_chain || !alt_codes)
    return HAWK_E_INVALID;
  hawk_ctx* ctx = ref_set->ctx;
  if (g->ctx != ctx) return HAWK_E_INVALID;
  const uint32_t ref_len = ref_set->hap_len[0];
  for (uint32_t i = 0; i < n_var; ++i) {
    if ((uint64_t)v_r0[i] + v_span[i] > ref_len || v_span[i] == 0 || v_alt_len[i] == 0) return HAWK_E_INVALID;
    if ((uint64_t)v_alt_off[i] + v_alt_len[i] > alt_codes_len) return HAWK_E_INVALID;
    if (i && v_r0[i] < v_r0[i - 1]) return HAWK_E_INVALID;
    if ((int64_t)v_chain[i] != (int64_t)v_alt_len[i] - (int64_t)v_span[i]) return HAWK_E_INVALID;
  }
  const uint32_t n_cols = 2 * g->n_samples;
  std::vector<uint64_t> hv_off(2, 0), ioff(2, 0);
  std::vector<uint32_t> hap_len(1, ref_len);
  uint32_t maxlen = ref_len;
  for (uint32_t c = 0; c < n_cols; ++c) {
    if (g->h_off[c + 1] == g->h_off[c]) continue;
    const int64_t len = (int64_t)ref_len + g->h_delta[c];
    if (len <= 0 || len >= (int64_t)((1u << 31) - 256)) return HAWK_E_UNSUPPORTED;
    hv_off.push_back(g->h_off[c + 1]);
    ioff.push_back(g->h_ioff[c + 1]);
    hap_len.push_back((uint32_t)len);
    maxlen = std::max(maxlen, (uint32_t)len);
  }
  const uint32_t n_hap = (uint32_t)hap_len.size();
  *n_hap_out = n_hap;
  hawk_xplan* x = nullptr;
  int rc = xplan_build(ref_set, n_var, v_r0, v_span, v_alt_off, v_alt_len, alt_codes, alt_codes_len, n_hap, hv_off.data(), g->d_idx, g->d_o,
                       hap_len.data(), maxlen, &x);
  if (rc) return rc;
  hipStream_t st = ctx->stream;
  DevBuf t_r0, t_span, t_ch, t_ioff, t_cnt, t_status, t_rev;
  DevBuf* temps[] = {&t_r0, &t_span, &t_ch, &t_ioff, &t_cnt, &t_status, &t_rev};
  auto done = [&](int code) { for (auto* b : temps) b->release(); if (code) hawk_xplan_destroy(x); return code; };
  if ((rc = t_r0.reserve((size_t)n_var * 4)) || (rc = t_span.reserve((size_t)n_var * 4)) || (rc = t_ch.reserve((size_t)n_var * 4)) ||
      (rc = t_ioff.reserve((size_t)(n_hap + 1) * 8)) || (rc = t_cnt.reserve((size_t)n_hap * 4)) || (rc = t_status.reserve(16)) ||
      (rc = t_rev.reserve((size_t)n_hap * 16)) || (rc = x->m_seg_off.reserve((size_t)(n_hap + 1) * 4)))
    return done(rc);
#define HIPCHK_X(expr)                                                                         \
  do {                                                                                         \
    hipError_t e_ = (expr);                                                                    \
    if (e_ != hipSuccess) {                                                                    \
      snprintf(hawk_hip_err_buf(), 256, "%s: %s (%s:%d)", #expr, hipGetErrorString(e_), __FILE__, __LINE__); \
      return done(HAWK_E_HIP);                                                                 \
    }                                                                                          \
  } while (0)
  HIPCHK_X(hipMemcpyAsync(t_r0.p, v_r0, (size_t)n_var * 4, hipMemcpyHostToDevice, st));
  HIPCHK_X(hipMemcpyAsync(t_span.p, v_span, (size_t)n_var * 4, hipMemcpyHostToDevice, st));
  HIPCHK_X(hipMemcpyAsync(t_ch.p, v_chain, (size_t)n_var * 4, hipMemcpyHostToDevice, st));
  HIPCHK_X(hipMemcpyAsync(t_ioff.p, ioff.data(), (size_t)(n_hap + 1) * 8, hipMemcpyHostToDevice, st));
  HIPCHK_X(hipMemsetAsync(t_status.p, 0, 16, st));
  hawk_launch_list_check(st, x->off.as<uint64_t>(), n_hap, g->d_idx, g->d_o, t_r0.as<int32_t>(), t_span.as<int32_t>(), t_ch.as<int32_t>(), n_var,
                         ref_len, check_clamp, t_status.as<uint32_t>());
  hawk_launch_segments(st, t_ioff.as<uint64_t>(), g->d_indel, g->d_idx, g->d_o, t_r0.as<int32_t>(), t_ch.as<int32_t>(), x->hlen.as<uint32_t>(), n_hap,
                       startp, t_cnt.as<uint32_t>(), x->m_seg_off.as<uint32_t>(), nullptr, nullptr);
  HIPCHK_X(hipGetLastError());
  uint32_t status = 0, nseg = 0;
  HIPCHK_X(hipMemcpyAsync(&status, t_status.p, 4, hipMemcpyDeviceToHost, st));
  HIPCHK_X(hipMemcpyAsync(&nseg, x->m_seg_off.as<uint32_t>() + n_hap, 4, hipMemcpyDeviceToHost, st));
  HIPCHK_X(hipStreamSynchronize(st));
  if (status & 4u) return done(HAWK_E_INVALID);
  if (status & 1u) return done(HAWK_E_OVERLAP);
  if (status & 2u) return done(HAWK_E_CLAMP);
  if ((rc = x->m_seg_rel.reserve((size_t)nseg * 4)) || (rc = x->m_seg_gen.reserve((size_t)nseg * 8))) return done(rc);
// ... 1 lines not shown
                       startp, t_cnt.as<uint32_t>(), x->m_seg_off.as<uint32_t>(), x->m_seg_rel.as<uint32_t>(), x->m_seg_gen.as<int64_t>());
  hawk_launch_rev_lookup(st, x->m_seg_off.as<uint32_t>(), x->m_seg_rel.as<uint32_t>(), x->m_seg_gen.as<int64_t>(), x->hlen.as<uint32_t>(), n_hap,
                         rev_g0, rev_g1, t_rev.as<int64_t>(), t_rev.as<int64_t>() + n_hap);
  HIPCHK_X(hipGetLastError());
  x->rev0.resize(n_hap); x->rev1.resize(n_hap);
  HIPCHK_X(hipMemcpyAsync(x->rev0.data(), t_rev.p, (size_t)n_hap * 8, hipMemcpyDeviceToHost, st));
  HIPCHK_X(hipMemcpyAsync(x->rev1.data(), t_rev.as<int64_t>() + n_hap, (size_t)n_hap * 8, hipMemcpyDeviceToHost, st));
  HIPCHK_X(hipStreamSynchronize(st));
#undef HIPCHK_X
  x->nseg = nseg; x->ref_startp = startp;
  x->min_gen = startp; x->max_gen = startp + (int64_t)ref_len;
  (void)done(HAWK_OK);
  *out = x;
  return HAWK_OK;
}

int hawk_xplan_rows(hawk_xplan* x, uint32_t* hap_len, int64_t* rev0, int64_t* rev1) {
  if (!x) return HAWK_E_INVALID;
  if (hap_len) memcpy(hap_len, x->hap_len.data(), (size_t)x->n_hap * 4);
  if ((rev0 || rev1) && x->rev0.size() != x->n_hap) return HAWK_E_INVALID;
  if (rev0) memcpy(rev0, x->rev0.data(), (size_t)x->n_hap * 8);
  if (rev1) memcpy(rev1, x->rev1.data(), (size_t)x->n_hap * 8);
  return HAWK_OK;
}

int hawk_xplan_text(hawk_xplan* x, uint32_t n_rows, const uint32_t* rows, const uint64_t* out_off, char* out, float* kernel_ms) {
  if (!x) return HAWK_E_INVALID;
  if (kernel_ms) *kernel_ms = 0.f;
  if (n_rows == 0) return HAWK_OK;
  if (!rows || !out_off || !out) return HAWK_E_INVALID;
  for (uint32_t i = 0; i < n_rows; ++i) {
    if (rows[i] >= x->n_hap || out_off[i + 1] < out_off[i]) return HAWK_E_INVALID;
    if (out_off[i + 1] - out_off[i] != (uint64_t)x->hap_len[rows[i]]) return HAWK_E_INVALID;
  }
  hawk_ctx* ctx = x->ctx;
  HIPCHK(hipSetDevice(ctx->device));
  const uint64_t total = out_off[n_rows] - out_off[0];
  std::vector<uint64_t> rel(n_rows);
  const uint64_t phase = out_off[0] & 15u;
  for (uint32_t i = 0; i < n_rows; ++i) rel[i] = out_off[i] - out_off[0] + phase;
  PoolScope tmp;
  uint32_t* d_rows; uint64_t* d_off; uint8_t* d_text;
  TEMPCHK(tmp, &d_rows, (size_t)n_rows * 4);
  TEMPCHK(tmp, &d_off, (size_t)n_rows * 8);
  TEMPCHK(tmp, &d_text, (size_t)(total + phase));
  hipStream_t st = ctx->stream;
  HIPCHK(hipMemcpyAsync(d_rows, rows, (size_t)n_rows * 4, hipMemcpyHostToDevice, st));
  HIPCHK(hipMemcpyAsync(d_off, rel.data(), (size_t)n_rows * 8, hipMemcpyHostToDevice, st));
  HIPCHK(hipEventRecord(ctx->ev[EV_KERNELS_BEGIN], st));
  hawk_launch_hx_text(st, x->ref_plane, x->ref_S, x->recs.p, x->codes.as<uint8_t>(), x->off.as<uint64_t>(), x->hlen.as<uint32_t>(), x->S,
                      x->tiles.p, n_rows, d_rows, d_off, d_text);
  HIPCHK(hipEventRecord(ctx->ev[EV_KERNELS_END], st));
  HIPCHK(hipGetLastError());
  HIPCHK(hipMemcpyAsync(out + out_off[0], d_text + phase, (size_t)total, hipMemcpyDeviceToHost, st));
  HIPCHK(hipStreamSynchronize(st));
  if (kernel_ms) (void)hipEventElapsedTime(kernel_ms, ctx->ev[EV_KERNELS_BEGIN], ctx->ev[EV_KERNELS_END]);
  return HAWK_OK;
}

int hawk_xplan_finish_meta(hawk_xplan* x, const int32_t* scan_start, const int32_t* scan_stop) {
  if (!x || !scan_start || !scan_stop || !x->nseg) return HAWK_E_INVALID;
  hawk_ctx* ctx = x->ctx;
  HIPCHK(hipSetDevice(ctx->device));
  const uint32_t n = x->n_hap;
  for (uint32_t h = 0; h < n; ++h)
    if (scan_start[h] < 0 || scan_stop[h] > (int32_t)x->hap_len[h]) return HAWK_E_INVALID;
  int rc;
  if ((rc = x->m_is_ref.reserve(n)) || (rc = x->m_ss.reserve((size_t)n * 4)) || (rc = x->m_se.reserve((size_t)n * 4)) ||
      (rc = x->m_tile.reserve((size_t)n * x->bph * sizeof(TileMeta))))
    return rc;
  hipStream_t st = ctx->stream;
  std::vector<uint8_t> is_ref(n, 0);
  is_ref[0] = 1;
  HIPCHK(hipMemcpyAsync(x->m_is_ref.p, is_ref.data(), n, hipMemcpyHostToDevice, st));
  HIPCHK(hipMemcpyAsync(x->m_ss.p, scan_start, (size_t)n * 4, hipMemcpyHostToDevice, st));
  HIPCHK(hipMemcpyAsync(x->m_se.p, scan_stop, (size_t)n * 4, hipMemcpyHostToDevice, st));
  hawk_launch_tile_meta(st, x->m_seg_off.as<uint32_t>(), x->m_seg_rel.as<uint32_t>(), x->hlen.as<uint32_t>(), x->m_is_ref.as<uint8_t>(),
                        x->m_ss.as<int32_t>(), x->m_se.as<int32_t>(), n, x->bph, x->m_tile.as<TileMeta>());
  HIPCHK(hipGetLastError());
  HIPCHK(hipStreamSynchronize(st));
  x->scan_start.assign(scan_start, scan_start + n);
  x->scan_stop.assign(scan_stop, scan_stop + n);
  x->ref_index = 0; x->n_ref_rows = 1; x->has_meta = true; x->cl.built = false; x->cl.usable = false;
  return HAWK_OK;
}

int hawk_xplan_segments(hawk_xplan* x, uint32_t* seg_off, uint32_t* seg_rel, int64_t* seg_gen, uint64_t cap, uint64_t* n_seg) {
  if (!x || !x->nseg) return HAWK_E_INVALID;
  if (n_seg) *n_seg = x->nseg;
  if (!seg_off && !seg_rel && !seg_gen) return HAWK_OK;
  if (cap < x->nseg) return HAWK_E_CAPACITY;
  hawk_ctx* ctx = x->ctx;
  HIPCHK(hipSetDevice(ctx->device));
  if (seg_off) HIPCHK(hipMemcpyAsync(seg_off, x->m_seg_off.p, (size_t)(x->n_hap + 1) * 4, hipMemcpyDeviceToHost, ctx->stream));
  if (seg_rel) HIPCHK(hipMemcpyAsync(seg_rel, x->m_seg_rel.p, (size_t)x->nseg * 4, hipMemcpyDeviceToHost, ctx->stream));
  if (seg_gen) HIPCHK(hipMemcpyAsync(seg_gen, x->m_seg_gen.p, (size_t)x->nseg * 8, hipMemcpyDeviceToHost, ctx->stream));
  HIPCHK(hipStreamSynchronize(ctx->stream));
  return HAWK_OK;
}


}
```

### crispr-hawk_amd/csrc/hawk_csearch.hip

```cpp
#include "hawk_vc.h"

#define CL_LINK 64
#define CL_NONE 0xffffffffu
#define CL_FAR (1 << 29)
#define CL_MAXWALK 4096
#define CS_G 8

struct __attribute__((aligned(16))) CsRow { uint4 a, b, c, d; };
static_assert(sizeof(CsRow) == 64, "template row layout");
size_t hawk_cs_row_bytes() { return sizeof(CsRow); }

__device__ __forceinline__ uint64_t cl_mix(uint64_t h, uint64_t v) {
  h = (h ^ v) * 0x9E3779B97F4A7C15ull;
  return h ^ (h >> 29);
}
struct __attribute__((aligned(16))) HxHead { int32_t o; uint32_t rs; uint32_t alt_len; uint32_t var; };
static_assert(sizeof(HxHead) == 16, "record head layout");
__global__ __launch_bounds__(256) void k_hx_heads(const HxVar* __restrict__ recs, const uint32_t* __restrict__ hv_idx, uint64_t n, uint4* __restrict__ heads) {
  const uint64_t j = (uint64_t)blockIdx.x * 256 + threadIdx.x;
  if (j >= n) return;
  const uint4 r = *reinterpret_cast<const uint4*>(recs + j);
  heads[j] = make_uint4(r.x, r.y, r.z, hv_idx[j]);
}
void hawk_launch_hx_heads(hipStream_t st, const void* recs, const uint32_t* hv_idx, uint64_t n, void* heads) {
// ... 300 lines not shown
      s = (s + 1u) & mask;
    }
    sl[u] = s;
    const uint32_t t = t0 + u * 256;
    if (!placed) { won[u] = false; cx_state[t] = CL_NONE; inst_uid[ent[u].x] = CL_NONE; atomicOr(status, fail_bit); continue; }
    cx_state[t] = won[u] ? CL_NONE : (CL_PENDING | s);
  }
  unsigned long long wb[CL_UID_U];
#pragma unroll
  for (int u = 0; u < CL_UID_U; ++u) { wb[u] = __ballot(won[u]); if (lane == 0) s_n[wv][u] = (uint32_t)__popcll(wb[u]); }
  __syncthreads();
  uint32_t tot = 0, mine[CL_UID_U];
#pragma unroll
  for (int u = 0; u < CL_UID_U; ++u) {
    mine[u] = tot;
#pragma unroll
    for (int w = 0; w < 256 / WAVE; ++w) { const uint32_t x = s_n[w][u]; if (w < (int)wv) mine[u] += x; tot += x; }
  }
  if (!tot) return;
  if (threadIdx.x == 0) s_base = atomicAdd(n_table, tot);
  __syncthreads();
  const uint32_t base = n_var + s_base;
#pragma unroll
  for (int u = 0; u < CL_UID_U; ++u) {
    if (!won[u]) continue;
    const uint32_t un = base + mine[u] + (uint32_t)__popcll(wb[u] & ((1ull << lane) - 1ull));
    const uint32_t i = ent[u].x;
    if (un >= u_cap) { inst_uid[i] = CL_NONE; atomicOr(status, fail_bit); continue; }
    const uint4 e1 = reinterpret_cast<const uint4*>(cx_list + (t0 + u * 256))[1];
    *reinterpret_cast<uint4*>(&tab[sl[u]].up1) = make_uint4(un + 1u, e1.x, e1.y, e1.w);
    inst_uid[i] = un;
    cu.rec[un] = ent[u].w; cu.n[un] = e1.x & 0xffffu; cu.row[un] = inst_row[i]; cu.o[un] = (int32_t)e1.z;
  }
}

__global__ __launch_bounds__(256) void k_cl_describe(const uint32_t* __restrict__ n_table_dev, uint32_t n_var, uint32_t u_cap,
                                                     const unsigned long long* __restrict__ var_desc, ClUniq cu, const HxHead* __restrict__ recs,
                                                     const uint32_t* __restrict__ seg_off, const uint32_t* __restrict__ seg_rel,
                                                     uint32_t* __restrict__ n_variant_clusters, unsigned long long* __restrict__ slots_total) {
  const uint32_t u = blockIdx.x * 256 + threadIdx.x;
  uint32_t span_u = 0;
  const uint32_t nu = n_var + *n_table_dev < u_cap ? n_var + *n_table_dev : u_cap;
  bool variant_cluster = false;
  if (u < nu) {
    uint32_t n, r, row;
    int32_t o_first;
    if (u < n_var) {
      const unsigned long long d = var_desc[u];
      variant_cluster = d != 0ull;
      r = (uint32_t)d; row = (uint32_t)(d >> 32); n = variant_cluster ? 1u : 0u;
      o_first = variant_cluster ? recs[r].o : 0;
      cu.rec[u] = r; cu.n[u] = n; cu.row[u] = row; cu.o[u] = o_first;
    } else {
      n = cu.n[u]; r = cu.rec[u]; row = cu.row[u]; o_first = cu.o[u];
    }
    if (n == 0) { cu.span2[u] = 0; cu.seg[u] = 0; }
    else {
      const int32_t o_end = recs[r + n - 1].o + (int32_t)recs[r + n - 1].alt_len;
      span_u = 2u * ((uint32_t)(o_end - o_first) + CL_LINK);
      cu.span2[u] = span_u;
      const uint32_t rel = o_first > CL_LINK + HAWK_PAD ? (uint32_t)(o_first - CL_LINK - HAWK_PAD) : 0u;
      uint32_t lo = seg_off[row], hi = seg_off[row + 1];
      while (hi - lo > 1) {
        const uint32_t mid = (lo + hi) >> 1;
        if (seg_rel[mid] <= rel) lo = mid; else hi = mid;
      }
      cu.seg[u] = lo;
    }
  }
  __shared__ uint32_t s_red[256 / WAVE][2];
  const unsigned long long vb = __ballot(variant_cluster);
  const uint32_t ssum = wave_sum(span_u);
  if ((threadIdx.x & (WAVE - 1)) == 0) { s_red[threadIdx.x / WAVE][0] = (uint32_t)__popcll(vb); s_red[threadIdx.x / WAVE][1] = ssum; }
  __syncthreads();
  if (threadIdx.x == 0) {
    uint32_t a = 0, b = 0;
#pragma unroll
    for (int w = 0; w < 256 / WAVE; ++w) { a += s_red[w][0]; b += s_red[w][1]; }
    if (a) atomicAdd(n_variant_clusters, a);
    if (b) atomicAdd(slots_total, (unsigned long long)b);
  }
}
__global__ void k_cl_results(const uint32_t* __restrict__ n_inst, const uint32_t* __restrict__ counters, const unsigned long long* __restrict__ slots_total,
                             const uint32_t* __restrict__ status, unsigned long long* __restrict__ out) {
  out[0] = *n_inst; out[1] = counters[0]; out[2] = counters[1]; out[3] = *slots_total; out[4] = *status;
}
__global__ __launch_bounds__(256) void k_cl_uid(const ClListed* __restrict__ cx_list, const uint32_t* __restrict__ n_list_dev, uint32_t t_end,
                                                const uint32_t* __restrict__ cx_state, const ClSlot* __restrict__ tab, uint32_t* __restrict__ inst_uid,
                                                ClUniq cu, const HxHead* __restrict__ recs, uint32_t* __restrict__ status) {
  const uint32_t n_list = *n_list_dev < t_end ? *n_list_dev : t_end;
  if (blockIdx.x * (256 * CL_UID_U) >= n_list) return;
  const uint32_t t0 = blockIdx.x * (256 * CL_UID_U) + threadIdx.x;
  uint32_t v[CL_UID_U];
  bool pend[CL_UID_U];
  bool any = false;
#pragma unroll
  for (int u = 0; u < CL_UID_U; ++u) {
    const uint32_t t = t0 + u * 256;
    v[u] = t < n_list ? cx_state[t] : CL_NONE;
    pend[u] = v[u] != CL_NONE && (v[u] & CL_PENDING);
    any = any || pend[u];
  }
  if (!__any(any)) return;
  uint4 e1[CL_UID_U], la[CL_UID_U], lb[CL_UID_U];
#pragma unroll
  for (int u = 0; u < CL_UID_U; ++u) {
    e1[u] = reinterpret_cast<const uint4*>(tab + (pend[u] ? (v[u] & ~CL_PENDING) : 0u))[1];
    const uint4* l = reinterpret_cast<const uint4*>(cx_list + (pend[u] ? t0 + u * 256 : 0u));
    la[u] = l[0]; lb[u] = l[1];
  }
  uint32_t rrec[CL_UID_U];
#pragma unroll
  for (int u = 0; u < CL_UID_U; ++u) rrec[u] = (pend[u] && e1[u].x != 0u && (lb[u].x & 0xffffu) > 1u) ? cu.rec[e1[u].x - 1u] : 0u;
  bool bad = false;
#pragma unroll
  for (int u = 0; u < CL_UID_U; ++u) {
    if (!pend[u]) continue;
    const uint32_t i = la[u].x, ncls = lb[u].x;
    if (e1[u].x == 0u) { inst_uid[i] = CL_NONE; bad = true; continue; }
    inst_uid[i] = e1[u].x - 1u;
    bool b = ncls != e1[u].y || (ncls >> 16) != 1 || lb[u].y != e1[u].z || lb[u].w != e1[u].w;
    const uint32_t n = ncls & 0xffffu;
    if (!b && n > 1) {
      const HxHead* pa = recs + la[u].w;
      const HxHead* pb = recs + rrec[u];
      const int32_t oa = (int32_t)lb[u].z, ob = pb[0].o;
      for (uint32_t k = 1; k < n; ++k) {
        const uint4 xa = *reinterpret_cast<const uint4*>(pa + k), xb = *reinterpret_cast<const uint4*>(pb + k);
        b = b || xa.w != xb.w || xa.z != xb.z || xa.y != xb.y || (int32_t)xa.x - oa != (int32_t)xb.x - ob;
      }
    }
    bad = bad || b;
  }
  if (bad) atomicOr(status, 2u);
}

uint32_t hawk_cl_chunk_bound(uint64_t n_records, uint32_t n_rows) { return (uint32_t)(n_records / CL_CHUNK) + n_rows; }
void hawk_launch_cl_chunks(hipStream_t st, const uint64_t* hv_off, const uint8_t* is_ref, const int32_t* ss, const int32_t* se, uint32_t n_rows,
                           uint32_t* ch_off, uint32_t* ch_row) {
  hipLaunchKernelGGL(k_cl_chunks, dim3(1), dim3(1024), 0, st, hv_off, is_ref, ss, se, n_rows, ch_off, ch_row);
}
void hawk_launch_cl_count(hipStream_t st, const void* recs, const uint64_t* hv_off, const uint32_t* hap_len, const int32_t* ss, const int32_t* se,
                          const uint32_t* ch_off, const uint32_t* ch_row, uint32_t n_rows, uint32_t n_var, uint32_t ch_bound, uint32_t* cnt ,
                          uint32_t* lcnt ) {
  if (ch_bound)
    hipLaunchKernelGGL(k_cl_count, dim3(ch_bound), dim3(256), 0, st, static_cast<const HxHead*>(recs), hv_off, hap_len, ss, se, ch_off, ch_row, n_rows,
                       n_var, cnt, lcnt);
}
#define CL_HEAD_CHUNKS 96
#define CL_HEAD_LISTED 16384
void hawk_launch_cl_fill(hipStream_t st, const void* recs, const uint64_t* hv_off, const uint32_t* hap_len, const int32_t* ss, const int32_t* se,
                         uint32_t n_rows, const uint32_t* ch_off, const uint32_t* ch_row, uint32_t ch_bound, const uint32_t* inst_base,
                         const uint32_t* list_base, int32_t* o, uint32_t* row, int32_t* pa, int32_t* rb, uint32_t* inst_uid, void* var_desc,
                         uint32_t* claim_bits, uint32_t n_var, void* cx_list, uint32_t* status) {
  ClInst ci{o, row, pa, rb, inst_uid};
#ifdef HAWK_TEST_HOOKS
  {
    const char* wk = getenv("HAWK_CLUSTER_WEAK_HASH");
    const uint32_t weak = wk && wk[0] == '1' ? 1u : 0u;
    (void)hipMemcpyToSymbol(HIP_SYMBOL(cl_weak_hash), &weak, sizeof(weak));
  }
#endif
  const uint32_t n_head = ch_bound < 16 * CL_HEAD_CHUNKS ? 0u : CL_HEAD_CHUNKS;
  if (n_head)
    hipLaunchKernelGGL(k_cl_fill, dim3(n_head), dim3(256), 0, st, static_cast<const HxHead*>(recs), hv_off, hap_len, ss, se, ch_off, ch_row, inst_base,
                       list_base, ci, static_cast<unsigned long long*>(var_desc), claim_bits, n_var, static_cast<ClListed*>(cx_list), status, 0u, n_rows, 1u);
  if (ch_bound > n_head)
    hipLaunchKernelGGL(k_cl_fill, dim3(ch_bound - n_head), dim3(256), 0, st, static_cast<const HxHead*>(recs), hv_off, hap_len, ss, se, ch_off, ch_row,
                       inst_base, list_base, ci, static_cast<unsigned long long*>(var_desc), claim_bits, n_var, static_cast<ClListed*>(cx_list), status,
                       n_head, n_rows, 0u);
}
void hawk_launch_cl_finish(hipStream_t st, uint32_t list_bound, const uint32_t* n_inst_dev, const uint32_t* n_list_dev, uint32_t* counters,
                           unsigned long long* results, uint32_t n_var, uint32_t u_cap, void* tab,
                           uint32_t mask, uint32_t max_probe, uint32_t fail_bit, const void* cx_list, uint32_t* cx_state, const void* var_desc,
                           const void* recs, uint32_t* inst_uid, const uint32_t* inst_row, const uint32_t* seg_off, const uint32_t* seg_rel,
                           uint32_t* u_rec, uint32_t* u_n, uint32_t* u_row, int32_t* u_o, uint32_t* u_seg, uint32_t* u_span2, uint32_t* status) {
  ClUniq cu{u_rec, u_n, u_row, u_o, u_seg, u_span2};
  const uint32_t per = 256 * CL_UID_U;
  const uint32_t head = list_bound < 16 * CL_HEAD_LISTED ? 0u : CL_HEAD_LISTED;
  const ClListed* list = static_cast<const ClListed*>(cx_list);
  if (head)
    hipLaunchKernelGGL(k_cl_enter, dim3((head + per - 1) / per), dim3(256), 0, st, list, n_list_dev, 0u, head, static_cast<ClSlot*>(tab), mask, max_probe,
                       fail_bit, inst_uid, inst_row, cx_state, cu, counters, n_var, u_cap, status);
  if (list_bound > head)
    hipLaunchKernelGGL(k_cl_enter, dim3((list_bound - head + per - 1) / per), dim3(256), 0, st, list, n_list_dev, head, list_bound, static_cast<ClSlot*>(tab),
                       mask, max_probe, fail_bit, inst_uid, inst_row, cx_state, cu, counters, n_var, u_cap, status);
  hipLaunchKernelGGL(k_cl_describe, dim3((u_cap + 255) / 256), dim3(256), 0, st, counters, n_var, u_cap, static_cast<const unsigned long long*>(var_desc), cu,
                     static_cast<const HxHead*>(recs), seg_off, seg_rel, counters + 1, reinterpret_cast<unsigned long long*>(counters + 4));
  if (list_bound)
    hipLaunchKernelGGL(k_cl_uid, dim3((list_bound + per - 1) / per), dim3(256), 0, st, list, n_list_dev, list_bound, cx_state, static_cast<const ClSlot*>(tab),
                       inst_uid, cu, static_cast<const HxHead*>(recs), status);
  hipLaunchKernelGGL(k_cl_results, dim3(1), dim3(1), 0, st, n_inst_dev, counters, reinterpret_cast<const unsigned long long*>(counters + 4), status, results);
}

__device__ __forceinline__ VcRanges cs_ranges(const HapSetDev& hs, const ScanParams& p, uint32_t h) {
  VcRanges rg;
  const int ss = hs.scan_start[h], se = hs.scan_stop[h], haplen = (int)hs.hap_len[h];
  const int poF = p.right ? 0 : p.guidelen, poR = p.right ? p.guidelen : 0;
  const int qmin = HAWK_PAD, qmax = haplen - p.L - HAWK_PAD + 1;
  rg.slo[0] = ss - poF; rg.shi[0] = se - poF; rg.slo[1] = ss - poR; rg.shi[1] = se - poR;
  rg.lo[0] = rg.slo[0] > qmin ? rg.slo[0] : qmin; rg.hi[0] = rg.shi[0] < qmax ? rg.shi[0] : qmax;
  rg.lo[1] = rg.slo[1] > qmin ? rg.slo[1] : qmin; rg.hi[1] = rg.shi[1] < qmax ? rg.shi[1] : qmax;
  return rg;
}
__device__ __forceinline__ uint32_t group_incl_scan(uint32_t v, uint32_t gl) {
#pragma unroll
  for (int d = 1; d < CS_G; d <<= 1) {
    const uint32_t t = (uint32_t)__shfl_up((int)v, d, CS_G);
    if (gl >= (uint32_t)d) v += t;
  }
  return v;
}

__device__ __forceinline__ int64_t posmap_hint(const HapSetDev& hs, uint32_t k0, uint32_t kend, uint32_t rel) {
  uint32_t k = k0;
  while (k + 1 < kend && hs.seg_rel[k + 1] <= rel) ++k;
  return hs.seg_gen[k] + (int64_t)(rel - hs.seg_rel[k]);
}

__global__ __launch_bounds__(256) void k_cs_templates(HapSetDev hs, VcArgs va, ClDict cd, ScanParams p, GuideParams gp, RefInfo ri,
                                                      uint4* __restrict__ res, uint32_t* __restrict__ tbase, CsRow* __restrict__ trows, unsigned long long* __restrict__ t_count, uint64_t t_cap, int* status) {
  __shared__ double s_cfd[336];
  __shared__ uint32_t s_w[256 / WAVE];
  __shared__ unsigned long long s_base;
  __shared__ uint32_t s_X[15][256];
  __shared__ uint32_t s_k[2][256];
  __shared__ uint32_t s_e[256];
  const uint32_t tid = threadIdx.x;
  if (gp.score_cfdon) for (uint32_t i = tid; i < 336; i += 256) s_cfd[i] = gp.cfd_mm[i];
  __syncthreads();
  const uint32_t gl = tid & (CS_G - 1);
  const uint32_t u = (blockIdx.x * 256 + tid) / CS_G;
  const uint32_t nc_u = u < cd.n_uniq ? cd.u_n[u] : 0u;
  const bool live = nc_u != 0u;
  const bool hole = u < cd.n_uniq && !live;
  const HxVar* __restrict__ recs = static_cast<const HxVar*>(va.recs_);
  const uint32_t h = live ? cd.u_row[u] : 0u, r0 = live ? cd.u_rec[u] : 0u, nc = live ? nc_u : 1u;
  const uint32_t seg0 = live ? cd.u_seg[u] : hs.seg_off[0], seg_end = hs.seg_off[h + 1];
  const uint32_t back = (uint64_t)r0 > va.hv_off[h] ? 1u : 0u;
  const HxVar* __restrict__ sv = recs + r0 - back;
  const int nrec = (int)(nc + back);
  const int L = p.L;
  const int32_t haplen = (int32_t)hs.hap_len[h];
  const int32_t o_first = live ? cd.u_o[u] : 0;
  const int32_t o_end = live ? recs[r0 + nc - 1].o + (int32_t)recs[r0 + nc - 1].alt_len : 0;
  const int32_t qa = o_first - (L - 1) > 0 ? o_first - (L - 1) : 0;
  const int32_t qb = o_end < haplen ? o_end : haplen;
  const int nwords = qb > qa ? (qb - qa + 31) / 32 : 0;
  const VcRanges rg = cs_ranges(hs, p, h);
  auto hits_before = [&](int64_t x) -> uint32_t {
    const int64_t xm = (int64_t)va.ref_S * 32;
    const uint32_t xc = (uint32_t)(x < 0 ? 0 : (x > xm ? xm : x));
    const uint4 e = va.hp[xc >> 5];
    const uint32_t m = (1u << (xc & 31u)) - 1u;
    return e.y + (uint32_t)__popc(e.x & m) + e.w + (uint32_t)__popc(e.z & m);
  };
  const int32_t rb_front = back ? (int32_t)sv[0].rs - (sv[0].o + (int32_t)sv[0].alt_len) : 0;
  const uint32_t h_front = hits_before((int64_t)o_first + rb_front - (L - 1)), h_behind = hits_before((int64_t)recs[r0 + nc - 1].rs);
  const int poF = p.right ? 0 : p.guidelen, poR = p.right ? p.guidelen : 0;
  const uint32_t mlo = L >= 32 ? 0xffffffffu : ((1u << L) - 1u), mhi = L <= 32 ? 0u : ((1u << (L - 32)) - 1u);
  const int W = L + 2 * HAWK_PAD;
  const uint32_t whi = W >= 64 ? 0xffffffffu : ((1u << (W - 32)) - 1u);
  const int ncfd = gp.guidelen < 20 ? gp.guidelen : 20;
  const uint32_t cfdmask = (1u << ncfd) - 1u;
  auto ref32 = [&](int pl, uint32_t r) -> uint32_t {
    const uint32_t w = (r >> 5) < va.ref_S - 2 ? (r >> 5) : va.ref_S - 2;
    return ext32_glb(va.ref[pl], (w << 5) | (r & 31u));
  };
  auto word = [&](int32_t q0, uint32_t (&X)[5][3], uint32_t& kF, uint32_t& kR, uint32_t& hits, uint32_t& cand) {
    const int32_t p0 = q0 - HAWK_PAD;
    const int32_t p0c = p0 < 0 ? 0 : p0;
    int32_t shift_run = 0;
    if (!vc_string_fast(va, sv, nrec, p0c, haplen, q0 + 32, X, shift_run))
      hx_words_t<false, 3>(va.alt_codes, sv, sv, nrec, nrec, false, p0c, haplen, ref32, X[0], X[1], X[2], X[3], X[4]);
    if (p0 < 0) {
      const uint32_t sh = (uint32_t)(-p0);
#pragma unroll
      for (int pl = 0; pl < 5; ++pl) {
        X[pl][2] = fsh(X[pl][1], X[pl][2], 32u - sh);
        X[pl][1] = fsh(X[pl][0], X[pl][1], 32u - sh);
        X[pl][0] = X[pl][0] << sh;
      }
    }
    uint32_t v0 = X[4][0], v1 = X[4][1], v2 = X[4][2];
    int r = 1;
    while (2 * r <= L && r < 32) {
      v0 |= fsh(v0, v1, (uint32_t)r); v1 |= fsh(v1, v2, (uint32_t)r); v2 |= v2 >> r;
      r *= 2;
    }
    const int rem = L - r;
    if (rem > 0) {
      if (rem < 32) { v0 |= fsh(v0, v1, (uint32_t)rem); v1 |= fsh(v1, v2, (uint32_t)rem); v2 |= v2 >> rem; }
      else { v0 |= v1; v1 |= v2; }
    }
    const uint32_t E = fsh(v0, v1, HAWK_PAD);
    const uint32_t own = range_mask(q0, qa, qb);
    uint32_t f = pam_match96(X, p.pam_fwd, p.pamlen, HAWK_PAD + poF) & own;
    uint32_t rv = pam_match96(X, p.pam_rev, p.pamlen, HAWK_PAD + poR) & own;
    f &= range_mask(q0, rg.slo[0], rg.shi[0]);
    rv &= range_mask(q0, rg.slo[1], rg.shi[1]);
    hits += __popc(f) + __popc(rv);
    f &= range_mask(q0, rg.lo[0], rg.hi[0]);
    rv &= range_mask(q0, rg.lo[1], rg.hi[1]);
    cand += __popc(f) + __popc(rv);
    kF = f & E;
    kR = rv & E;
  };
  auto classify = [&](int32_t q0, const uint32_t (&X)[5][3], uint32_t kF, uint32_t kR, uint32_t& vF, uint32_t& vR) {
    vF = 0; vR = 0;
#pragma unroll 1
    for (int s = 0; s < 2; ++s) {
      uint32_t m = s ? kR : kF;
      while (m) {
        const uint32_t bpos = (uint32_t)__builtin_ctz(m);
        m &= m - 1u;
        const int64_t start = posmap_hint(hs, seg0, seg_end, (uint32_t)q0 + bpos);
        const int64_t qr64 = start - ri.startp;
        const bool inr = qr64 >= 0 && qr64 < (int64_t)ri.n_bits;
// ... 132 lines not shown
  uint32_t done = 0;
#pragma unroll 1
  for (int sd = 0; sd < 2; ++sd) {
    const uint32_t T = sd ? TR : TF, sh16 = sd ? 16u : 0u;
    uint32_t ns = 0;
#pragma unroll 1
    for (uint32_t j0 = 0; j0 < T; j0 += CS_G) {
      const uint32_t j = j0 + gl;
      const bool act = j < T;
      const uint32_t jj = act ? j : 0u;
      uint32_t l = 0;
#pragma unroll
      for (uint32_t step = CS_G / 2; step; step >>= 1) l += (((s_e[g0 + l + step] >> sh16) & 0xffffu) <= jj) ? step : 0u;
      const uint32_t src = g0 + l;
      const uint32_t bpos = select_bit(s_k[sd][src], jj - ((s_e[src] >> sh16) & 0xffffu));
      const uint32_t q = (uint32_t)(qa + 32 * (int32_t)l) + bpos;
      W2 win[5], core[4], rcore[4];
#pragma unroll
      for (int pl = 0; pl < 5; ++pl) {
        win[pl] = ext96(s_X[pl * 3 + 0][src], s_X[pl * 3 + 1][src], s_X[pl * 3 + 2][src], bpos);
        win[pl].hi &= whi;
        if (pl < 4) {
          core[pl].lo = fsh(win[pl].lo, win[pl].hi, HAWK_PAD) & mlo;
          core[pl].hi = (win[pl].hi >> HAWK_PAD) & mhi;
        }
      }
      const int64_t start = posmap_hint(hs, seg0, seg_end, q), stop = posmap_hint(hs, seg0, seg_end, q + (uint32_t)L);
      const int64_t qr64 = start - ri.startp;
      const bool inr = qr64 >= 0 && qr64 < (int64_t)ri.n_bits;
      const uint32_t qr = inr ? (uint32_t)qr64 : 0u;
      const uint32_t rw = (sd ? ri.bits[1] : ri.bits[0])[qr >> 5];
#pragma unroll
      for (int pl = 0; pl < 4; ++pl) rcore[pl] = ext_glb(va.ref[pl], qr);
      const bool has_ref = inr && ((rw >> (qr & 31u)) & 1u);
      bool same = has_ref;
#pragma unroll
      for (int pl = 0; pl < 4; ++pl) {
        rcore[pl].lo &= mlo; rcore[pl].hi &= mhi;
        same = same && rcore[pl].lo == core[pl].lo && rcore[pl].hi == core[pl].hi;
        if (!has_ref) rcore[pl] = core[pl];
      }
      const bool valid = act && !same;
      const uint32_t vinc = group_incl_scan(valid ? 1u : 0u, gl);
      const uint32_t vtot = (uint32_t)__shfl((int)vinc, CS_G - 1, CS_G);
      if (valid && live) {
        const uint64_t k = tb + done + ns + (vinc - 1u);
        if (k >= t_cap) atomicExch(status, -3 );
        else {
          double score = __longlong_as_double(0x7ff8000000000000ll);
          if (gp.score_cfdon && has_ref) {
            bool err;
            score = cfdon_from_slices(core, rcore, (uint32_t)sd, L, cfdmask, s_cfd, err);
            if (err && gp.score_cfdon == 1) atomicExch(status, -5 );
          }
          const bool pamfirst = (p.right != 0) != (sd != 0);
          const int64_t ds = start - ri.startp, de = stop - start;
          if (ds < INT32_MIN || ds > INT32_MAX || de < INT32_MIN || de > INT32_MAX) atomicExch(status, -7 );
          const uint64_t sc = (uint64_t)__double_as_longlong(score);
          uint4* __restrict__ tp = reinterpret_cast<uint4*>(trows + k);
          tp[0] = make_uint4((uint32_t)((int32_t)(pamfirst ? q : q + (uint32_t)p.guidelen) - o_first), (uint32_t)sd | (has_ref ? 2u : 0u),
                             (uint32_t)(int32_t)ds, (uint32_t)(int32_t)de);
          tp[1] = make_uint4((uint32_t)sc, (uint32_t)(sc >> 32), win[0].lo, win[0].hi);
          tp[2] = make_uint4(win[1].lo, win[1].hi, win[2].lo, win[2].hi);
          tp[3] = make_uint4(win[3].lo, win[3].hi, win[4].lo, win[4].hi);
        }
      }
      ns += vtot;
    }
    if (sd == 0) n0 = ns; else n1 = ns;
    done += ns;
  }
  if (leader) { res[2 * u] = make_uint4(n0, n1, hits, cand); res[2 * u + 1] = make_uint4((uint32_t)tb, h_front, h_behind, 0u); tbase[u] = (uint32_t)tb; }
}

#define CS_CNT_U 4
__global__ __launch_bounds__(256) void k_cs_count(HapSetDev hs, VcArgs va, ClDict cd, ScanParams p, const uint4* __restrict__ res,
                                                  const unsigned long long* __restrict__ t_count, uint64_t t_cap,
                                                  uint32_t* __restrict__ group_counts, uint32_t* __restrict__ counts, uint32_t* __restrict__ inst_tb,
                                                  unsigned long long* __restrict__ shards) {
  __shared__ uint32_t s_red[256 / WAVE][2];
  const uint32_t i0 = blockIdx.x * (256 * CS_CNT_U) + threadIdx.x;
  const uint32_t lane = threadIdx.x & (WAVE - 1);
  const bool ovf = *t_count > t_cap;
  uint32_t uid[CS_CNT_U], below[CS_CNT_U];
  int32_t paf[CS_CNT_U];
  bool in[CS_CNT_U];
#pragma unroll
  for (int u = 0; u < CS_CNT_U; ++u) {
    const uint32_t i = i0 + u * 256;
    in[u] = i < cd.n_inst;
    const uint32_t ic = in[u] ? i : 0u;
    uid[u] = cd.inst_uid[ic]; paf[u] = cd.inst_pa[ic];
    below[u] = CL_NONE;
    if (lane == 0 && in[u] && i > 0) below[u] = cd.inst_uid[i - 1];
  }
  uint4 r[CS_CNT_U], r2[CS_CNT_U];
  uint32_t behind0[CS_CNT_U];
#pragma unroll
  for (int u = 0; u < CS_CNT_U; ++u) {
    const bool has = in[u] && uid[u] != CL_NONE;
    r[u] = make_uint4(0u, 0u, 0u, 0u); r2[u] = r[u]; behind0[u] = 0u;
    if (cd.n_uniq) {
      const uint32_t us = has ? uid[u] : 0u;
      r[u] = res[2 * us]; r2[u] = res[2 * us + 1];
      if (lane == 0 && below[u] != CL_NONE) behind0[u] = res[2 * below[u] + 1].z;
    }
    if (!has) { r[u] = make_uint4(0u, 0u, 0u, 0u); r2[u] = r[u]; }
  }
  uint32_t cand = 0, hits = 0;
#pragma unroll
  for (int u = 0; u < CS_CNT_U; ++u) {
    const uint32_t i = i0 + u * 256;
    uint32_t behind = (uint32_t)__shfl_up((int)r2[u].z, 1);
    if (lane == 0) behind = behind0[u];
    uint32_t rows_i = 0;
    if (in[u]) {
      if (paf[u] < 0) {
        const uint32_t hc = r2[u].y - behind;
        hits += hc; cand += hc;
      } else {
        const int32_t pa = paf[u], pb = cd.inst_o[i] - (p.L - 1);
        if (pb > pa) {
          const VcRanges rg = cs_ranges(hs, p, cd.inst_row[i]);
          vc_count_run(va, rg, pa, pb, cd.inst_rb[i], cand, hits);
        }
      }
      hits += r[u].z; cand += r[u].w;
      rows_i = ovf ? 0u : r[u].x + r[u].y;
      counts[i] = rows_i;
      inst_tb[i] = r2[u].x;
    }
    const uint32_t gsum = wave_sum(rows_i);
    const uint32_t iw = blockIdx.x * (256 * CS_CNT_U) + u * 256 + (threadIdx.x & ~(uint32_t)(WAVE - 1));
    if (lane == 0 && iw < cd.n_inst) group_counts[iw / WAVE] = gsum;
  }
  const uint32_t a = wave_sum(cand), b = wave_sum(hits);
  if (lane == 0) { s_red[threadIdx.x / WAVE][0] = a; s_red[threadIdx.x / WAVE][1] = b; }
  __syncthreads();
  if (threadIdx.x == 0) {
    uint32_t t0 = 0, t1 = 0;
#pragma unroll
    for (int wv = 0; wv < 256 / WAVE; ++wv) { t0 += s_red[wv][0]; t1 += s_red[wv][1]; }
    if (t0 | t1) {
      atomicAdd(&shards[(blockIdx.x & 255u) * 2 + 0], (unsigned long long)t0);
      atomicAdd(&shards[(blockIdx.x & 255u) * 2 + 1], (unsigned long long)t1);
    }
  }
}

__device__ __forceinline__ void nt_store4(uint32_t* q, const uint4& v) {
  __builtin_nontemporal_store(v.x, q); __builtin_nontemporal_store(v.y, q + 1);
  __builtin_nontemporal_store(v.z, q + 2); __builtin_nontemporal_store(v.w, q + 3);
}
template <int NI, int CE_CH>
__global__ __launch_bounds__(256) void k_cs_emit_rows(uint32_t n_inst, const uint32_t* __restrict__ inst_row, const int32_t* __restrict__ inst_o,
                                                      const uint32_t* __restrict__ counts, const uint32_t* __restrict__ inst_tb,
                                                      const CsRow* __restrict__ trows, const uint64_t* __restrict__ offsets,
                                                      const unsigned long long* __restrict__ t_count, uint64_t t_cap, uint4* __restrict__ rows,
                                                      uint64_t cap, int* status) {
  constexpr int NE = NI * WAVE;
  constexpr int CE_SUB = CE_CH / 16;
  __shared__ uint32_t s_ex[4][NE + 1];
  __shared__ uint32_t s_tb[4][NE], s_h[4][NE];
  __shared__ int32_t s_dq[4][NE];
  __shared__ uint32_t s_src[4][2][CE_CH], s_rh[4][2][CE_CH];
  __shared__ int32_t s_rdq[4][2][CE_CH];
  if (*t_count > t_cap) return;
  const uint32_t wv = threadIdx.x / WAVE, lane = threadIdx.x & (WAVE - 1);
  const uint32_t i0 = (blockIdx.x * 4 + wv) * NE;
  if (i0 >= n_inst) return;
  uint32_t cnt[NI], tb[NI], h[NI];
  int32_t dq[NI];
#pragma unroll
  for (int c = 0; c < NI; ++c) {
    const uint32_t i = i0 + c * WAVE + lane;
    const bool in = i < n_inst;
    const uint32_t ii = in ? i : n_inst - 1;
    cnt[c] = counts[ii]; tb[c] = inst_tb[ii]; h[c] = inst_row[ii]; dq[c] = inst_o[ii];
    if (!in) cnt[c] = 0;
  }
  const uint64_t o0 = offsets[i0 / WAVE];
  uint32_t Wt = 0;
#pragma unroll
  for (int c = 0; c < NI; ++c) {
    const uint32_t inc = wave_incl_scan(cnt[c]);
    s_ex[wv][c * WAVE + lane] = Wt + inc - cnt[c];
    s_tb[wv][c * WAVE + lane] = tb[c]; s_h[wv][c * WAVE + lane] = h[c] << HAWK_ROW_HAP_SHIFT; s_dq[wv][c * WAVE + lane] = dq[c];
    Wt += (uint32_t)__builtin_amdgcn_readlane((int)inc, WAVE - 1);
  }
  if (Wt == 0) return;
  if (o0 + Wt > cap) { if (lane == 0) atomicCAS(status, 0, -3 ); return; }
  __builtin_amdgcn_wave_barrier();
  const uint32_t qd = lane & 3u, rq = lane >> 2;
  uint4* __restrict__ const dst = rows + o0 * 4 + qd;
  auto meta = [&](uint32_t c0, uint32_t buf) {
#pragma unroll
    for (uint32_t sub = 0; sub < (CE_CH + WAVE - 1) / WAVE; ++sub) {
      const uint32_t r = sub * WAVE + lane;
      if (CE_CH < WAVE && r >= CE_CH) break;
      const uint32_t t = c0 + r < Wt ? c0 + r : Wt - 1;
      uint32_t l = 0;
#pragma unroll
      for (uint32_t step = NE / 2; step; step >>= 1) l += (s_ex[wv][l + step] <= t) ? step : 0u;
      s_src[wv][buf][r] = s_tb[wv][l] + (t - s_ex[wv][l]);
      s_rh[wv][buf][r] = s_h[wv][l];
      s_rdq[wv][buf][r] = s_dq[wv][l];
    }
    __builtin_amdgcn_wave_barrier();
  };
  auto fetch = [&](uint4 (&v)[CE_SUB], uint32_t buf) {
#pragma unroll
    for (uint32_t j = 0; j < CE_SUB; ++j) v[j] = reinterpret_cast<const uint4*>(trows + s_src[wv][buf][j * 16 + rq])[qd];
  };
  auto store = [&](const uint4 (&v)[CE_SUB], uint32_t c0, uint32_t buf) {
#pragma unroll
    for (uint32_t j = 0; j < CE_SUB; ++j) {
      const uint32_t r = j * 16 + rq;
      uint4 w = v[j];
      if (qd == 0) {
        w.x = (uint32_t)((int32_t)w.x + s_rdq[wv][buf][r]);
        w.y |= s_rh[wv][buf][r];
      }
      if (c0 + r < Wt) nt_store4(reinterpret_cast<uint32_t*>(dst + (size_t)(c0 + r) * 4), w);
    }
  };
  uint4 va[CE_SUB], vb[CE_SUB];
  meta(0, 0);
  fetch(va, 0);
#pragma unroll 1
  for (uint32_t c0 = 0; c0 < Wt; c0 += 2 * CE_CH) {
    const bool more1 = c0 + CE_CH < Wt, more2 = c0 + 2 * CE_CH < Wt;
    if (more1) { meta(c0 + CE_CH, 1); fetch(vb, 1); }
    store(va, c0, 0);
    __builtin_amdgcn_wave_barrier();
    if (more1) {
      if (more2) { meta(c0 + 2 * CE_CH, 0); fetch(va, 0); }
      store(vb, c0 + CE_CH, 1);
      __builtin_amdgcn_wave_barrier();
    }
  }
}
void hawk_launch_cs_emit_rows(hipStream_t st, const ClDict& cd, const uint32_t* counts, const uint32_t* inst_tb, const void* trows, const uint64_t* offsets,
                              const unsigned long long* t_count, uint64_t t_cap, void* rows, uint64_t cap, int* status) {
  if (!cd.n_inst) return;
  constexpr int NI = 4, CH = 256;
  hipLaunchKernelGGL((k_cs_emit_rows<NI, CH>), dim3((cd.n_inst + 256 * NI - 1) / (256 * NI)), dim3(256), 0, st, cd.n_inst, cd.inst_row, cd.inst_o, counts,
                     inst_tb, static_cast<const CsRow*>(trows), offsets, t_count, t_cap, static_cast<uint4*>(rows), cap, status);
}

void hawk_launch_cs_templates(hipStream_t st, const HapSetDev& hs, const VcArgs& va, const ClDict& cd, const ScanParams& p, const GuideParams& gp,
                              const RefInfo& ri, void* res, uint32_t* tbase, void* trows, unsigned long long* t_count, uint64_t t_cap, int* status) {
  if (!cd.n_uniq) return;
  const uint32_t nb = (uint32_t)(((uint64_t)cd.n_uniq * CS_G + 255) / 256);
  hipLaunchKernelGGL(k_cs_templates, dim3(nb), dim3(256), 0, st, hs, va, cd, p, gp, ri, static_cast<uint4*>(res), tbase, static_cast<CsRow*>(trows),
                     t_count, t_cap, status);
}
void hawk_launch_cs_count(hipStream_t st, const HapSetDev& hs, const VcArgs& va, const ClDict& cd, const ScanParams& p, const void* res,
                          const unsigned long long* t_count, uint64_t t_cap, uint32_t* group_counts, uint32_t* counts, uint32_t* inst_tb,
                          unsigned long long* shards) {
  if (!cd.n_inst) return;
  hipLaunchKernelGGL(k_cs_count, dim3((cd.n_inst + 256 * CS_CNT_U - 1) / (256 * CS_CNT_U)), dim3(256), 0, st, hs, va, cd, p, static_cast<const uint4*>(res), t_count, t_cap,
                     group_counts, counts, inst_tb, shards);
}

__global__ __launch_bounds__(256) void k_rows_pack(GuideCols c, const uint64_t* __restrict__ n_dev, uint64_t n_host, uint4* __restrict__ rows, int64_t startp,
                                                   int* status) {
  const uint64_t n = n_dev ? *n_dev : n_host;
  const uint64_t i = (uint64_t)blockIdx.x * 256 + threadIdx.x;
  if (i >= n) return;
  const int64_t start = c.start[i], ds = start - startp, de = c.stop[i] - start;
  const uint32_t h = c.hap[i];
  if (ds < INT32_MIN || ds > INT32_MAX || de < INT32_MIN || de > INT32_MAX || h >= HAWK_ROW_MAX_HAP) atomicCAS(status, 0, -7 );
  const uint64_t sc = (uint64_t)__double_as_longlong(c.cfdon[i]);
  uint64_t w[HAWK_PLANES];
#pragma unroll
  for (int pl = 0; pl < HAWK_PLANES; ++pl) w[pl] = c.win[(size_t)pl * c.cap + i];
  uint4* __restrict__ r = rows + i * 4;
  r[0] = make_uint4(c.pos[i], (uint32_t)(c.strand[i] & 1u) | ((uint32_t)c.flags[i] << 1) | (h << HAWK_ROW_HAP_SHIFT), (uint32_t)(int32_t)ds, (uint32_t)(int32_t)de);
  r[1] = make_uint4((uint32_t)sc, (uint32_t)(sc >> 32), (uint32_t)w[0], (uint32_t)(w[0] >> 32));
  r[2] = make_uint4((uint32_t)w[1], (uint32_t)(w[1] >> 32), (uint32_t)w[2], (uint32_t)(w[2] >> 32));
  r[3] = make_uint4((uint32_t)w[3], (uint32_t)(w[3] >> 32), (uint32_t)w[4], (uint32_t)(w[4] >> 32));
}
__global__ __launch_bounds__(256) void k_rows_unpack(const uint4* __restrict__ rows, uint64_t n, int64_t startp, GuideCols d) {
  const uint64_t i = (uint64_t)blockIdx.x * 256 + threadIdx.x;
  if (i >= n) return;
  const uint4* __restrict__ r = rows + i * 4;
  const uint4 a = r[0], b = r[1], cc = r[2], e = r[3];
  const int64_t start = startp + (int64_t)(int32_t)a.z;
  if (d.hap) d.hap[i] = a.y >> HAWK_ROW_HAP_SHIFT;
  if (d.pos) d.pos[i] = a.x;
  if (d.strand) d.strand[i] = (uint8_t)(a.y & 1u);
  if (d.flags) d.flags[i] = (uint8_t)((a.y >> 1) & 0xffu);
  if (d.start) d.start[i] = start;
  if (d.stop) d.stop[i] = start + (int64_t)(int32_t)a.w;
  if (d.cfdon) d.cfdon[i] = __longlong_as_double((long long)((uint64_t)b.x | ((uint64_t)b.y << 32)));
  if (d.win) {
    d.win[i] = (uint64_t)b.z | ((uint64_t)b.w << 32);
    d.win[d.cap + i] = (uint64_t)cc.x | ((uint64_t)cc.y << 32);
    d.win[2 * d.cap + i] = (uint64_t)cc.z | ((uint64_t)cc.w << 32);
    d.win[3 * d.cap + i] = (uint64_t)e.x | ((uint64_t)e.y << 32);
    d.win[4 * d.cap + i] = (uint64_t)e.z | ((uint64_t)e.w << 32);
  }
}
void hawk_launch_rows_pack(hipStream_t st, const GuideCols& src, const uint64_t* n_dev, uint64_t n_host, uint64_t max_rows, uint4* rows, int64_t startp,
                           int* status) {
  if (!max_rows) return;
  hipLaunchKernelGGL(k_rows_pack, dim3((unsigned)((max_rows + 255) / 256)), dim3(256), 0, st, src, n_dev, n_host, rows, startp, status);
}
void hawk_launch_rows_unpack(hipStream_t st, const uint4* rows, uint64_t n, int64_t startp, const GuideCols& dst) {
  if (!n) return;
  hipLaunchKernelGGL(k_rows_unpack, dim3((unsigned)((n + 255) / 256)), dim3(256), 0, st, rows, n, startp, dst);
}

__global__ __launch_bounds__(256) void k_cc_ucnt(const uint4* __restrict__ res, uint32_t nu, uint32_t* __restrict__ cnt) {
  const uint32_t u = blockIdx.x * 256 + threadIdx.x;
  if (u < nu) { const uint4 r = res[2 * u]; cnt[u] = r.x + r.y; }
}
__global__ __launch_bounds__(256) void k_cc_mini(GuideCols c, uint64_t r0, const CsRow* __restrict__ trows, uint64_t t_rows,
                                                 const uint64_t* __restrict__ moff, const uint32_t* __restrict__ tbase, uint32_t nu, int64_t startp,
                                                 GuideCols m) {
  const uint64_t i = (uint64_t)blockIdx.x * 256 + threadIdx.x;
  if (i >= r0 + t_rows) return;
  if (i < r0) {
    m.hap[i] = gc_hap(c, i); m.pos[i] = gc_pos(c, i); m.strand[i] = (uint8_t)gc_strand(c, i); m.start[i] = gc_start(c, i); m.stop[i] = gc_stop(c, i);
    m.flags[i] = (uint8_t)gc_flags(c, i); m.cfdon[i] = gc_cfdon(c, i);
#pragma unroll
    for (int pl = 0; pl < HAWK_PLANES; ++pl) m.win[(size_t)pl * m.cap + i] = gc_win(c, pl, i);
    return;
  }
// ... 81 lines not shown
```

### crispr-hawk_amd/csrc/hawk_device.h

```cpp
#pragma once
#include <hip/hip_runtime.h>
#include <stdint.h>

#define HAWK_PLANES 5
#define HAWK_PAD 10
#define HAWK_BLOCK 256
#define HAWK_WPT 4

struct HapSetDev {
  uint32_t n_hap;
  uint32_t S;
  const uint32_t* plane[HAWK_PLANES];
  const uint32_t* hap_len;
  const uint8_t* is_ref;
  const int32_t* scan_start;
  const int32_t* scan_stop;
  const uint32_t* seg_off;
  const uint32_t* seg_rel;
  const int64_t* seg_gen;
  int32_t ref_index;
};

struct TileMeta {
  uint32_t h, blk;
// ... 11 lines not shown
  uint32_t need;
  int32_t poF, poR;
};

struct ScanTotals {
  uint64_t n_keep;
  uint64_t n_keep_fwd;
  uint64_t n_cand;
  uint64_t n_hits;
};

struct GuideCols {
  uint32_t* hap;
  uint32_t* pos;
  uint8_t* strand;
  int64_t* start;
  int64_t* stop;
  uint8_t* flags;
  double* cfdon;
  uint64_t* win;
  uint64_t cap;
  uint4* rows;
  int64_t startp;
};
#define HAWK_ROW_HAP_SHIFT 9
#define HAWK_ROW_MAX_HAP (1u << 23)
#ifdef __HIPCC__
__device__ __forceinline__ const uint32_t* gc_roww(const GuideCols& c, uint64_t i) { return reinterpret_cast<const uint32_t*>(c.rows) + i * 16; }
__device__ __forceinline__ uint32_t gc_hap(const GuideCols& c, uint64_t i) { return c.rows ? gc_roww(c, i)[1] >> HAWK_ROW_HAP_SHIFT : c.hap[i]; }
__device__ __forceinline__ uint32_t gc_pos(const GuideCols& c, uint64_t i) { return c.rows ? gc_roww(c, i)[0] : c.pos[i]; }
__device__ __forceinline__ uint32_t gc_strand(const GuideCols& c, uint64_t i) { return c.rows ? (gc_roww(c, i)[1] & 1u) : (uint32_t)c.strand[i]; }
__device__ __forceinline__ uint32_t gc_flags(const GuideCols& c, uint64_t i) { return c.rows ? ((gc_roww(c, i)[1] >> 1) & 0xffu) : (uint32_t)c.flags[i]; }
__device__ __forceinline__ int64_t gc_start(const GuideCols& c, uint64_t i) { return c.rows ? c.startp + (int64_t)(int32_t)gc_roww(c, i)[2] : c.start[i]; }
__device__ __forceinline__ int64_t gc_stop(const GuideCols& c, uint64_t i) {
  if (!c.rows) return c.stop[i];
  const uint32_t* w = gc_roww(c, i);
  return c.startp + (int64_t)(int32_t)w[2] + (int64_t)(int32_t)w[3];
}
__device__ __forceinline__ double gc_cfdon(const GuideCols& c, uint64_t i) {
  if (!c.rows) return c.cfdon[i];
  const uint32_t* w = gc_roww(c, i);
  return __longlong_as_double((long long)((uint64_t)w[4] | ((uint64_t)w[5] << 32)));
}
__device__ __forceinline__ uint64_t gc_win(const GuideCols& c, int pl, uint64_t i) {
  if (!c.rows) return c.win[(size_t)pl * c.cap + i];
  const uint32_t* w = gc_roww(c, i);
  return (uint64_t)w[6 + 2 * pl] | ((uint64_t)w[7 + 2 * pl] << 32);
}
#endif
void hawk_launch_rows_pack(hipStream_t st, const GuideCols& src, const uint64_t* n_dev, uint64_t n_host, uint64_t max_rows, uint4* rows, int64_t startp,
                           int* status);
void hawk_launch_rows_unpack(hipStream_t st, const uint4* rows, uint64_t n, int64_t startp, const GuideCols& dst);

struct GuideParams {
  int32_t pamlen, guidelen, right, L;
  int32_t score_cfdon;
  const double* cfd_mm;
  const double* cfd_pam;
  uint32_t bph;
};

struct RefInfo {
  int32_t index;
  int32_t lo[2], hi[2];
  int64_t startp;
  const uint32_t* bits[2];
  uint32_t n_bits;
};
struct VcArgs {
  const uint32_t* ref[4];
  uint32_t ref_S;
  const void* recs_;
  const uint8_t* alt_codes;
  const uint64_t* hv_off;
  const void* tiles_;
  const uint4* hp;
};
void hawk_launch_vsearch(hipStream_t st, int pass, const HapSetDev& hs, const VcArgs& va, const ScanParams& p, const struct GuideParams& gp,
                         const struct RefInfo& ri, const TileMeta* tmeta, uint32_t* counts, uint32_t* counts0, unsigned long long* shards,
                         const uint64_t* offsets, struct GuideCols out, int* status, uint32_t tile0, uint32_t n_tiles);
void hawk_launch_ref_hits(hipStream_t st, const HapSetDev& hs, const ScanParams& p, int32_t ref_index, void* hp);
struct ClDict {
  uint32_t n_inst, n_uniq;
  const uint32_t* inst_uid;
  const int32_t* inst_o;
  const uint32_t* inst_row;
  const int32_t* inst_pa;
  const int32_t* inst_rb;
  const uint32_t* u_rec;
  const uint32_t* u_n;
  const uint32_t* u_row;
  const int32_t* u_o;
  const uint32_t* u_seg;
};
size_t hawk_cs_row_bytes();
void hawk_launch_scan2_u32(hipStream_t st, const uint32_t* cnt_a, const uint32_t* cnt_b, uint32_t n, uint32_t* off_a, uint32_t* off_b);
void hawk_launch_hx_heads(hipStream_t st, const void* recs, const uint32_t* hv_idx, uint64_t n, void* heads);
uint32_t hawk_cl_chunk_bound(uint64_t n_records, uint32_t n_rows);
void hawk_launch_cl_chunks(hipStream_t st, const uint64_t* hv_off, const uint8_t* is_ref, const int32_t* ss, const int32_t* se, uint32_t n_rows,
                           uint32_t* ch_off, uint32_t* ch_row);
void hawk_launch_cl_count(hipStream_t st, const void* recs, const uint64_t* hv_off, const uint32_t* hap_len, const int32_t* ss, const int32_t* se,
                          const uint32_t* ch_off, const uint32_t* ch_row, uint32_t n_rows, uint32_t n_var, uint32_t ch_bound, uint32_t* cnt ,
                          uint32_t* lcnt );
void hawk_launch_cl_fill(hipStream_t st, const void* recs, const uint64_t* hv_off, const uint32_t* hap_len, const int32_t* ss, const int32_t* se,
                         uint32_t n_rows, const uint32_t* ch_off, const uint32_t* ch_row, uint32_t ch_bound, const uint32_t* inst_base,
                         const uint32_t* list_base, int32_t* o, uint32_t* row, int32_t* pa, int32_t* rb, uint32_t* inst_uid,
                         void* var_desc , uint32_t* claim_bits , uint32_t n_var,
                         void* cx_list , uint32_t* status);
size_t hawk_cl_slot_bytes();
size_t hawk_cl_listed_bytes();
void hawk_launch_cl_finish(hipStream_t st, uint32_t list_bound, const uint32_t* n_inst_dev, const uint32_t* n_list_dev, uint32_t* counters ,
                           unsigned long long* results , uint32_t n_var, uint32_t u_cap,
                           void* tab , uint32_t mask, uint32_t max_probe, uint32_t fail_bit, const void* cx_list, uint32_t* cx_state,
                           const void* var_desc, const void* recs, uint32_t* inst_uid, const uint32_t* inst_row, const uint32_t* seg_off,
                           const uint32_t* seg_rel, uint32_t* u_rec, uint32_t* u_n, uint32_t* u_row, int32_t* u_o, uint32_t* u_seg, uint32_t* u_span2,
                           uint32_t* status);
void hawk_launch_cs_templates(hipStream_t st, const HapSetDev& hs, const VcArgs& va, const ClDict& cd, const ScanParams& p, const struct GuideParams& gp,
                              const struct RefInfo& ri, void* res , uint32_t* tbase, void* trows,
                              unsigned long long* t_count, uint64_t t_cap, int* status);
void hawk_launch_cs_count(hipStream_t st, const HapSetDev& hs, const VcArgs& va, const ClDict& cd, const ScanParams& p, const void* res,
                          const unsigned long long* t_count, uint64_t t_cap, uint32_t* group_counts, uint32_t* counts, uint32_t* inst_tb,
                          unsigned long long* shards);
void hawk_launch_cs_emit_rows(hipStream_t st, const ClDict& cd, const uint32_t* counts, const uint32_t* inst_tb, const void* trows, const uint64_t* offsets,
                              const unsigned long long* t_count, uint64_t t_cap, void* rows, uint64_t cap, int* status);
void hawk_launch_list_check(hipStream_t st, const uint64_t* row_off, uint32_t n_rows, const uint32_t* hv_idx, const int32_t* hv_o,
                            const int32_t* v_r0, const int32_t* v_span, const int32_t* v_chain, uint32_t n_var, uint32_t ref_len,
                            int check_clamp, uint32_t* status);
void hawk_launch_segments(hipStream_t st, const uint64_t* ioff, const uint32_t* indel, const uint32_t* hv_idx, const int32_t* hv_o,
                          const int32_t* v_r0, const int32_t* v_chain, const uint32_t* hap_len, uint32_t n_rows, int64_t startp,
                          uint32_t* seg_cnt, uint32_t* seg_off, uint32_t* seg_rel , int64_t* seg_gen);
void hawk_launch_rev_lookup(hipStream_t st, const uint32_t* seg_off, const uint32_t* seg_rel, const int64_t* seg_gen, const uint32_t* hap_len,
                            uint32_t n_rows, int64_t g0, int64_t g1, int64_t* out0, int64_t* out1);
void hawk_launch_tile_meta(hipStream_t st, const uint32_t* seg_off, const uint32_t* seg_rel, const uint32_t* hap_len, const uint8_t* is_ref,
                           const int32_t* scan_start, const int32_t* scan_stop, uint32_t n_rows, uint32_t bph, TileMeta* tm);
void hawk_launch_ref_bits(hipStream_t st, const HapSetDev& hs, const ScanParams& p, const RefInfo& ri, uint32_t* bitsF, uint32_t* bitsR);

struct OtSite {
  uint64_t code;
  uint32_t nmask;
  uint32_t q;
  uint32_t row;
  uint32_t pad;
};
struct OtHit { uint64_t site; uint32_t guide; uint32_t mm; };
#define OT_MAX_BLOCKS 8
struct OtSeeds {
  int32_t nb;
  int32_t start[OT_MAX_BLOCKS], klen[OT_MAX_BLOCKS];
  uint32_t off_base[OT_MAX_BLOCKS];
  uint64_t pmask2[OT_MAX_BLOCKS];
};

#define OT_MAX_PAIRS (OT_MAX_BLOCKS * (OT_MAX_BLOCKS - 1) / 2)
struct OtPairSeeds {
  int32_t nb, n_pairs;
  int32_t start[OT_MAX_BLOCKS], klen[OT_MAX_BLOCKS];
  uint64_t pmask2[OT_MAX_BLOCKS];
  uint8_t pi[OT_MAX_PAIRS], pj[OT_MAX_PAIRS];
  uint32_t off_base[OT_MAX_PAIRS];
};
void hawk_launch_ot_match_pairs(hipStream_t st, const OtSite* sites, uint64_t n_sites, const OtPairSeeds& sd, const uint32_t* goff,
                                const uint64_t* gcode, const uint32_t* gid, uint32_t n_guides, int guidelen, int sp0, int max_mm,
                                OtHit* hits, uint64_t cap, unsigned long long* n_hits);

void hawk_launch_ot_onehot(hipStream_t st, uint32_t* const* plane, uint64_t nwords);
void hawk_launch_ot_sites(hipStream_t st, const HapSetDev& hs, const ScanParams& p, const uint32_t* keepF, const uint32_t* keepR,
                          const uint64_t* offsets, OtSite* sites);
void hawk_launch_ot_match(hipStream_t st, const OtSite* sites, uint64_t n_sites, const uint64_t* guides, uint32_t n_guides,
                          int guidelen, int sp0, int max_mm, OtHit* hits, uint64_t cap, unsigned long long* n_hits);
void hawk_launch_ot_match_seeded(hipStream_t st, const OtSite* sites, uint64_t n_sites, const OtSeeds& sd, const uint32_t* goff,
                                 const uint64_t* gcode, const uint32_t* gid, uint32_t n_guides, int guidelen, int sp0, int max_mm,
                                 OtHit* hits, uint64_t cap, unsigned long long* n_hits);
void hawk_launch_ot_gather(hipStream_t st, const OtSite* sites, const OtHit* hits, uint64_t n_hits, OtSite* out);
struct OtSummary {
  const OtSite* sites;
  const double* tab;
  uint32_t* hist;
  unsigned long long* cfd_e4;
  unsigned long long* counters;
  uint32_t stride;
  int32_t sp0, pam2, ncmp;
};
void hawk_launch_ot_match_sum(hipStream_t st, const OtSite* sites, uint64_t n_sites, const uint64_t* guides, uint32_t n_guides,
                              int guidelen, int sp0, int max_mm, const OtSummary& sm);
void hawk_launch_ot_match_seeded_sum(hipStream_t st, const OtSite* sites, uint64_t n_sites, const OtSeeds& sd, const uint32_t* goff,
                                     const uint64_t* gcode, const uint32_t* gid, uint32_t n_guides, int guidelen, int sp0, int max_mm,
                                     const OtSummary& sm);
void hawk_launch_ot_match_pairs_sum(hipStream_t st, const OtSite* sites, uint64_t n_sites, const OtPairSeeds& sd, const uint32_t* goff,
                                    const uint64_t* gcode, const uint32_t* gid, uint32_t n_guides, int guidelen, int sp0, int max_mm,
                                    const OtSummary& sm);
void hawk_launch_pack(hipStream_t st, const uint8_t* ascii, const uint64_t* seq_off, uint32_t hap0, uint32_t n_hap_batch,
                      uint64_t batch_base, const uint32_t* hap_len, uint32_t S, uint32_t* const* plane,
                      unsigned long long* bad_index);
void hawk_launch_scan_raw(hipStream_t st, const HapSetDev& hs, const ScanParams& p, uint32_t* keepF, uint32_t* keepR,
                          uint32_t* counts);
void hawk_launch_emit_hits(hipStream_t st, const HapSetDev& hs, uint32_t bph, const uint32_t* keepF, const uint32_t* keepR,
                           const uint64_t* offsets, uint64_t n_fwd_total, uint32_t* hits_fwd, uint32_t* hits_rev);
void hawk_launch_search(hipStream_t st, int pass, const HapSetDev& hs, const ScanParams& p, const GuideParams& gp,
                        const RefInfo& ri, const TileMeta* tmeta, uint32_t* counts, unsigned long long* shards,
// ... 85 lines not shown
```

### crispr-hawk_amd/csrc/hawk_host.h

```cpp
#pragma once
#include <hip/hip_runtime.h>

#include <cstddef>
#include <cstdio>
#include <memory>
#include <vector>

#include "../../include/hawk.h"
#include "hawk_device.h"

#define HAWK_MAX_DEVICES 16
char* hawk_hip_err_buf();

#define HIPCHK(expr)                                                                         \
  do {                                                                                       \
    hipError_t e_ = (expr);                                                                  \
    if (e_ != hipSuccess) {                                                                  \
      snprintf(hawk_hip_err_buf(), 256, "%s: %s (%s:%d)", #expr, hipGetErrorString(e_), __FILE__, __LINE__); \
      return HAWK_E_HIP;                                                                     \
    }                                                                                        \
  } while (0)

struct hawk_ctx {
  int device;
  hipStream_t stream;
  hipEvent_t ev[10];
  void* pinned = nullptr;
};

struct SearchStatusBlock {
  int status;
  int pad0;
  unsigned long long template_rows;
  uint32_t big_count;
  uint32_t pad1[3];
  ScanTotals totals;
};
struct SearchMisc {
  unsigned long long shards[256][2];
  SearchStatusBlock blk;
};
static_assert(sizeof(SearchStatusBlock) == 64 && sizeof(SearchMisc) == 4096 + 64, "status block layout");
static_assert(offsetof(SearchMisc, shards) == 0 && offsetof(SearchMisc, blk) == 4096, "status block layout");
static_assert(offsetof(SearchStatusBlock, status) == 0 && offsetof(SearchStatusBlock, template_rows) == 8 &&
              offsetof(SearchStatusBlock, big_count) == 16 && offsetof(SearchStatusBlock, totals) == 32, "status block layout");

int hawk_pool_alloc(void** p, size_t bytes);
void hawk_pool_free(void* p);
void hawk_pool_trim();
#define POOLCHK(ptr, bytes)                                                      \
  do {                                                                           \
    int rc_ = hawk_pool_alloc(reinterpret_cast<void**>(ptr), (bytes));           \
    if (rc_) return rc_;                                                         \
  } while (0)

struct PoolScope {
  std::vector<void*> held;
  ~PoolScope() { for (void* q : held) hawk_pool_free(q); }
  int alloc(void** out, size_t bytes) {
    int rc = hawk_pool_alloc(out, bytes);
    if (!rc) held.push_back(*out);
    return rc;
  }
};
#define TEMPCHK(scope, ptr, bytes)                                               \
  do {                                                                           \
    int rc_ = (scope).alloc(reinterpret_cast<void**>(ptr), (bytes));             \
    if (rc_) return rc_;                                                         \
  } while (0)

struct DevBuf {
  void* p = nullptr;
  size_t bytes = 0;
  int reserve(size_t need) {
    if (need <= bytes) return HAWK_OK;
    if (p) { hawk_pool_free(p); p = nullptr; bytes = 0; }
    size_t want = need + need / 8 + 256;
    int rc = hawk_pool_alloc(&p, want);
    if (rc) return rc;
    bytes = want;
    return HAWK_OK;
  }
  void release() { if (p) hawk_pool_free(p); p = nullptr; bytes = 0; }
  template <class T> T* as() const { return reinterpret_cast<T*>(p); }
};

struct hawk_hapset {
  hawk_ctx* ctx;
  uint32_t n_hap, S;
  uint64_t total_len;
  std::vector<uint32_t> hap_len;
  std::vector<int32_t> scan_start, scan_stop;
  uint32_t* plane[HAWK_PLANES];
  uint32_t* d_hap_len;
  uint8_t* d_is_ref;
  int32_t *d_scan_start, *d_scan_stop;
  uint32_t *d_seg_off, *d_seg_rel;
  int64_t* d_seg_gen;
  int32_t ref_index;
  uint32_t n_ref_rows = 0;
  bool has_meta;
  bool has_partner = false;
  int32_t partner_start = 0, partner_stop = 0;
  uint32_t bph;
  TileMeta* d_tile_meta;
  int64_t ref_startp;
  int64_t min_gen, max_gen;
  uint64_t cols_cap = 0;
  uint64_t cols_gen = 0;
  uint64_t collapse_gen = 0;
  std::vector<double> cfd_host;
  DevBuf keepF, keepR, counts, offsets, totals, misc, cfd, partial, sites, hits, guides, lists;
  DevBuf ckeys, cvals, cflags, cgidx, ctemp, cgoff, cgc, ccnt, cfull;
  DevBuf ctable, cocc, cdense, cgkey, cgslot;
  uint64_t last_groups = 0;
  std::shared_ptr<uint64_t> plan_groups;
  DevBuf otoff, otcode, otid, othit;
  DevBuf otsum;
  DevBuf big;
  DevBuf refbits;
  bool refbits_valid = false;
  uint64_t refbits_key[6] = {0, 0, 0, 0, 0, 0};
  const struct hawk_xplan* vplan = nullptr;
  DevBuf vcnt0;
  DevBuf refhp;
  uint64_t cs_tcap = 0;
  DevBuf cs_res, cs_tbase, cs_trows, cs_itb, cs_icnt;
  DevBuf cmini[8], cm_gid;
  DevBuf colsA[8];
  DevBuf rowsA;
  uint64_t rows_cap = 0;
  DevBuf crep[8];
};

struct hawk_xplan {
  hawk_ctx* ctx;
  uint32_t n_var, n_hap, ref_len;
  uint64_t ncar;
  std::vector<uint32_t> hap_len;
  uint32_t* ref_plane[4];
  uint32_t ref_S;
  DevBuf ref5[HAWK_PLANES];
  DevBuf recs, tiles, codes, off, hlen, hash;
  DevBuf heads;
  bool has_meta;
  std::vector<int32_t> scan_start, scan_stop;
  DevBuf m_is_ref, m_ss, m_se, m_seg_off, m_seg_rel, m_seg_gen, m_tile;
  uint32_t nseg, bph, S;
  int32_t ref_index;
  int64_t ref_startp, min_gen, max_gen;
  bool has_partner = false;
  int32_t partner_start = 0, partner_stop = 0;
  uint32_t n_ref_rows = 0;
  std::vector<int64_t> rev0, rev1;
  std::shared_ptr<uint64_t> groups = std::make_shared<uint64_t>(0);
  struct {
    bool built = false, usable = false;
    uint32_t n_inst = 0, n_uniq = 0;
    uint32_t n_real = 0;
    uint32_t last_uniq = 0;
    uint64_t slots = 0;
    uint32_t status = 0;
    float build_ms = 0.f;
    DevBuf inst_uid, inst_o, inst_row, inst_pa, inst_rb, u_rec, u_n, u_row, u_o, u_seg;
  } cl;
};

struct hawk_gt {
  hawk_ctx* ctx;
  uint64_t n_lines;
  uint32_t n_samples, n_var;
  uint8_t* d_codes;
  uint8_t* d_flags;
  uint64_t n_entries;
  uint64_t* d_col_off; uint32_t* d_idx; int32_t* d_o; int64_t* d_delta;
  uint64_t n_indel = 0;
  uint32_t* d_indel = nullptr;
  uint64_t* d_ioff = nullptr;
  std::vector<uint64_t> h_off, h_ioff;
  std::vector<int64_t> h_delta;
};

struct hawk_table {
  hawk_hapset* hs;
  hawk_ctx* ctx;
  uint64_t n_rows, n_cand, n_hits, cap;
  GuideCols cols;
  uint32_t guidelen, pamlen, right;
  uint64_t n_groups;
  bool collapsed;
  uint64_t gen;
  DevBuf own[8];
  bool by_cluster = false;
  uint32_t plane_tiles = 0;
  uint64_t t_rows = 0;
};
inline bool hawk_table_stale(const hawk_table* t) { return t->hs && t->gen != t->hs->cols_gen; }

int hawk_reserve_cols(DevBuf (&b)[8], uint64_t cap, GuideCols* c);

int hapset_create_impl(hawk_ctx* ctx, uint32_t n_hap, const uint32_t* hap_len, bool zero_planes, hawk_hapset** out, bool alloc_planes = true);
HapSetDev make_dev(const hawk_hapset* hs);
int make_scan_params(const hawk_hapset* hs, uint64_t pam_fwd, uint64_t pam_rev, uint32_t pamlen, uint32_t guidelen,
                            uint32_t right, bool need_v, ScanParams* sp);
int meta_build(uint32_t n, const std::vector<uint32_t>& hap_len, uint32_t bph, const uint8_t* is_ref, const int32_t* scan_start,
                      const int32_t* scan_stop, const uint32_t* seg_off, const uint32_t* seg_rel, const int64_t* seg_gen,
                      int32_t ref_index, std::vector<TileMeta>* t0, int64_t* min_gen, int64_t* max_gen);
```

### include/hawk.h

```cpp
#ifndef HAWK_H
#define HAWK_H

#include <stdint.h>

#ifdef __cplusplus
extern "C" {
#endif

typedef enum {
  HAWK_OK = 0,
  HAWK_E_INVALID = -1,
  HAWK_E_HIP = -2,
  HAWK_E_CAPACITY = -3,
  HAWK_E_IUPAC = -4,
  HAWK_E_CFD = -5,
  HAWK_E_NODEVICE = -6,
  HAWK_E_UNSUPPORTED = -7,
  HAWK_E_COMM = -8,
  HAWK_E_OVERLAP = -9,
  HAWK_E_CLAMP = -10
} hawk_status;

typedef struct hawk_ctx hawk_ctx;
typedef struct hawk_hapset hawk_hapset;
typedef struct hawk_table hawk_table;

#define HAWK_GUIDESEQPAD 10
#define HAWK_MAX_CORE 44

int hawk_device_count(int* n);
int hawk_init(int device, hawk_ctx** out);
void hawk_destroy(hawk_ctx* ctx);
const char* hawk_strerror(int status);
const char* hawk_last_hip_error(void);
void* hawk_stream(hawk_ctx* ctx);
int hawk_sync(hawk_ctx* ctx);
int hawk_release_cached_memory(hawk_ctx* ctx);
int hawk_host_alloc(hawk_ctx* ctx, uint64_t bytes, void** out);
void hawk_host_free(void* p);


int hawk_hapset_create(hawk_ctx* ctx, uint32_t n_hap, const uint32_t* hap_len, hawk_hapset** out);
void hawk_hapset_destroy(hawk_hapset* hs);

int hawk_hapset_pack_ascii(hawk_hapset* hs, const char* seqs, const uint64_t* seq_off, uint64_t* bad_index);

int hawk_hapset_set_meta(hawk_hapset* hs, const uint8_t* is_ref, const int32_t* scan_start, const int32_t* scan_stop,
                         const uint32_t* seg_off, const uint32_t* seg_rel, const int64_t* seg_gen, int32_t ref_index);

int hawk_hapset_set_ref_partner_range(hawk_hapset* hs, int32_t start, int32_t stop);

int hawk_hapset_stride(const hawk_hapset* hs, uint32_t* stride_words);
int hawk_hapset_download_plane(hawk_hapset* hs, int plane, uint32_t* out_words);
int hawk_hapset_rows_equal(hawk_hapset* hs, uint32_t n_pairs, const uint32_t* rows_a, const uint32_t* rows_b, uint8_t* equal);
int hawk_hapset_upload_planes(hawk_hapset* hs, const uint32_t* planes);

typedef struct hawk_xplan hawk_xplan;
typedef struct hawk_gt hawk_gt;
int hawk_xplan_create_gt(hawk_hapset* ref_set, hawk_gt* g, uint32_t n_var, const uint32_t* v_r0, const uint32_t* v_span,
                         const uint32_t* v_alt_off, const uint32_t* v_alt_len, const int32_t* v_chain, const uint8_t* alt_codes,
                         uint32_t alt_codes_len, int64_t startp, int check_clamp, int64_t rev_g0, int64_t rev_g1, uint32_t* n_hap_out,
                         hawk_xplan** out);
int hawk_xplan_rows(hawk_xplan* x, uint32_t* hap_len, int64_t* rev0, int64_t* rev1);
int hawk_xplan_finish_meta(hawk_xplan* x, const int32_t* scan_start, const int32_t* scan_stop);
int hawk_xplan_segments(hawk_xplan* x, uint32_t* seg_off, uint32_t* seg_rel, int64_t* seg_gen, uint64_t cap, uint64_t* n_seg);
int hawk_xplan_install_meta(hawk_xplan* x, hawk_hapset* hs);
int hawk_xplan_set_ref_partner_range(hawk_xplan* x, int32_t start, int32_t stop);
int hawk_xplan_run(hawk_xplan* x, hawk_hapset** out, uint64_t* hash_out, float* kernel_ms);
void hawk_xplan_destroy(hawk_xplan* x);
int hawk_xplan_text(hawk_xplan* x, uint32_t n_rows, const uint32_t* rows, const uint64_t* out_off, char* out, float* kernel_ms);
int hawk_xplan_view(hawk_xplan* x, hawk_hapset** out);
int hawk_xplan_cluster_stats(const hawk_xplan* x, uint32_t* usable, uint32_t* n_instances, uint32_t* n_distinct, uint64_t* template_slots,
                             float* build_ms, uint32_t* status);
int hawk_xplan_cluster_rebuild(hawk_xplan* x);

int hawk_pam_scan(hawk_hapset* hs, uint64_t pam_fwd, uint64_t pam_rev, uint32_t pamlen, uint32_t* hits_fwd,
                  uint32_t* hits_rev, uint64_t cap_fwd, uint64_t cap_rev, uint64_t* off_fwd, uint64_t* off_rev);

int hawk_pam_scan_time(hawk_hapset* hs, uint64_t pam_fwd, uint64_t pam_rev, uint32_t pamlen, uint32_t reps, float* avg_ms,
                       uint64_t* scanned_positions);

typedef struct {
  uint64_t pam_fwd, pam_rev;
  uint32_t pamlen, guidelen;
  uint32_t right;
  uint32_t score_cfdon;
  const double* cfd_mm;
  const double* cfd_pam;
} hawk_search_params;

typedef struct {
  float count_ms;
  float offsets_ms;
  float emit_ms;
  float total_ms;
  uint64_t scanned_positions;
  float emit_list_ms;
  float v_count_ms;
  float v_emit_ms;
  float v_templates_ms;
  uint32_t v_path;
  float v_emit_rows_ms;
  float reserved;
} hawk_timing;

int hawk_search(hawk_hapset* hs, const hawk_search_params* p, hawk_table** out, hawk_timing* timing);
void hawk_table_destroy(hawk_table* t);
int hawk_table_counts(const hawk_table* t, uint64_t* n_rows, uint64_t* n_candidates, uint64_t* n_hits);
int hawk_table_download(hawk_table* t, uint32_t* hap, uint32_t* pos, uint8_t* strand, int64_t* start, int64_t* stop,
                        uint8_t* flags, double* cfdon, uint64_t* win);
#define HAWK_LAYOUT_COLUMNS 0u
#define HAWK_LAYOUT_ROWS 1u
int hawk_table_layout(const hawk_table* t, uint32_t* layout, int64_t* startp);
int hawk_table_download_rows(hawk_table* t, void* rows64 );
int hawk_table_device_rows(hawk_table* t, void** rows64, int64_t* startp);
int hawk_table_device_columns(hawk_table* t, void** hap, void** pos, void** strand, void** start, void** stop,
                              void** flags, void** cfdon, void** win, uint64_t* win_plane_stride);

int hawk_table_collapse(hawk_table* t, uint64_t* n_groups, float* kernel_ms);
int hawk_table_collapse_download(hawk_table* t, uint32_t* perm, uint64_t* group_off, uint8_t* gc_num, uint8_t* gc_den);
int hawk_table_collapse_ex(hawk_table* t, uint32_t flank_up, uint32_t flank_down, uint64_t* n_groups, float* kernel_ms);
int hawk_table_collapse_export(hawk_table* t, uint32_t* rep_row, uint32_t* pos, uint8_t* strand, int64_t* start, int64_t* stop,
                               uint8_t* flags, double* cfdon, uint64_t* win, uint32_t* member_hap, float* kernel_ms);

int hawk_host_polish_rows(uint64_t n, uint32_t L, const uint8_t* cores, const uint32_t* hap, const int64_t* pivot, const int64_t* stop,
                          const uint64_t* cand_off, const uint32_t* cand_var, const uint64_t* seg_start, const uint32_t* seg_rel,
                          const int64_t* seg_gen, uint64_t n_haps, const int64_t* t_pos, const uint8_t* ref_pool, const uint64_t* ref_off,
                          const uint8_t* alt_pool, const uint64_t* alt_off, uint32_t n_var, const uint32_t* name_rank, uint64_t* out_off,
                          uint32_t* out_var, uint8_t* need_python);

int hawk_host_variant_window(uint64_t n, const uint32_t* hap, const int64_t* p_lo, const int64_t* p_hi, const uint64_t* var_off,
                             const int64_t* var_idx, const int64_t* t_pos, uint64_t n_haps, uint32_t n_var, uint64_t* first, uint32_t* count);
int hawk_host_polish_windows(uint64_t n, uint32_t L, const uint8_t* cores, const uint32_t* hap, const int64_t* pivot, const int64_t* stop,
                             const uint64_t* first, const uint64_t* cand_off, const int64_t* var_idx, uint64_t n_idx, const uint64_t* seg_start,
                             const uint32_t* seg_rel, const int64_t* seg_gen, uint64_t n_haps, const int64_t* t_pos, const uint8_t* ref_pool,
                             const uint64_t* ref_off, const uint8_t* alt_pool, const uint64_t* alt_off, uint32_t n_var, const uint32_t* name_rank,
                             uint64_t* out_off, uint32_t* out_var, uint8_t* need_python);

int hawk_host_vcf_index(const uint8_t* text, uint64_t len, uint64_t cap, uint64_t* line_start, int64_t* pos, uint64_t* gt_off,
                        uint32_t* chrom_len, uint64_t* n_lines, uint32_t* multi_contig);

#define HAWK_TSV_CONST 0u
#define HAWK_TSV_FIXED 1u
#define HAWK_TSV_RAGGED 2u
#define HAWK_TSV_INT64 3u
#define HAWK_TSV_VOCAB 4u
typedef struct {
  uint32_t kind, width;
  const void* data;
  const uint64_t* off;
  const void* pool;
  uint64_t n_vocab;
} hawk_tsv_col;
int hawk_host_tsv_write(const char* path, const char* header, uint64_t header_len, uint64_t n_rows, const uint64_t* order, uint32_t n_cols,
                        const hawk_tsv_col* cols, uint64_t* bytes_out);

int hawk_host_ragged_join(const uint32_t* item_label, const uint64_t* group_off, uint64_t n_groups, const uint8_t* pool,
// ... 86 lines not shown
```

Baseline: 562.0 billion.

## Queue cluster dictionary build asynchronously and let search consume it provisionally

The cluster dictionary build no longer blocks with its own host synchronisation. It is queued on the stream, and the search kernels read the actual instance and unique counts from a device-side 'live' buffer while launching with upper-bound grid sizes. After the search's status readback, the host resolves the dictionary. If the small-table pass overflowed, the search is redone with a full table. This removes a host round trip between dictionary build and search, at the cost of oversized launches, early-exit checks in kernels, and an occasional full redo.

```diff
diff --git a/crispr-hawk_amd/crisprhawk_hip/_lib.py b/crispr-hawk_amd/crisprhawk_hip/_lib.py
--- a/crispr-hawk_amd/crisprhawk_hip/_lib.py
+++ b/crispr-hawk_amd/crisprhawk_hip/_lib.py
@@ -25,7 +25,7 @@
     "hawk_search", "hawk_table_destroy", "hawk_table_counts", "hawk_table_download", "hawk_table_device_columns", "hawk_table_layout", "hawk_table_download_rows", "hawk_table_device_rows", "hawk_cfd",
     "hawk_genome_finalize", "hawk_offtarget_scan", "hawk_offtarget_summary", "hawk_deepcpf1", "hawk_azimuth", "hawk_tm_nn",
     "hawk_table_collapse", "hawk_table_collapse_download", "hawk_gt_parse", "hawk_gt_destroy", "hawk_gt_codes", "hawk_gt_lists",
-    "hawk_gt_lists_download", "hawk_gt_lists_indels", "hawk_release_cached_memory", "hawk_xplan_run", "hawk_xplan_view", "hawk_xplan_cluster_stats", "hawk_xplan_cluster_rebuild", "hawk_host_gather_plan", "hawk_xplan_create_gt", "hawk_xplan_rows",
+    "hawk_gt_lists_download", "hawk_gt_lists_indels", "hawk_release_cached_memory", "hawk_xplan_run", "hawk_xplan_view", "hawk_xplan_cluster_stats", "hawk_xplan_cluster_rebuild", "hawk_xplan_queue_counters", "hawk_host_gather_plan", "hawk_xplan_create_gt", "hawk_xplan_rows",
     "hawk_xplan_finish_meta", "hawk_xplan_segments", "hawk_xplan_install_meta", "hawk_host_alloc", "hawk_host_free", "hawk_hapset_rows_equal",
     "hawk_xplan_destroy", "hawk_hapset_set_ref_partner_range", "hawk_xplan_set_ref_partner_range", "hawk_table_collapse_ex", "hawk_table_collapse_export", "hawk_comm_unique_id", "hawk_comm_init",
     "hawk_comm_destroy", "hawk_comm_last_error", "hawk_comm_allgather_u64", "hawk_comm_gatherv", "hawk_table_gather", "hawk_host_ragged_join", "hawk_host_tsv_write", "hawk_host_vcf_index", "hawk_host_polish_rows", "hawk_host_variant_window", "hawk_host_polish_windows", "hawk_host_group_join", "hawk_host_group_samples", "hawk_gbt_predict", "hawk_gt_from_codes",
diff --git a/crispr-hawk_amd/crisprhawk_hip/hapset.py b/crispr-hawk_amd/crisprhawk_hip/hapset.py
--- a/crispr-hawk_amd/crisprhawk_hip/hapset.py
+++ b/crispr-hawk_amd/crisprhawk_hip/hapset.py
@@ -238,6 +238,11 @@
     def rebuild_dictionary(self) -> None:
         _lib.check(self._L.hawk_xplan_cluster_rebuild(self._x), "hawk_xplan_cluster_rebuild")
 
+    def queue_counters(self) -> dict:
+        a, b, c = C.c_uint64(), C.c_uint64(), C.c_uint64()
+        _lib.check(self._L.hawk_xplan_queue_counters(self._x, C.byref(a), C.byref(b), C.byref(c)), "hawk_xplan_queue_counters")
+        return {"provisional": a.value, "accepted": b.value, "redone": c.value}
+
     def cluster_stats(self) -> dict:
         u, ni, nd, st = C.c_uint32(), C.c_uint32(), C.c_uint32(), C.c_uint32()
         slots, ms = C.c_uint64(), C.c_float()
diff --git a/crispr-hawk_amd/csrc/hawk_api.hip b/crispr-hawk_amd/csrc/hawk_api.hip
--- a/crispr-hawk_amd/csrc/hawk_api.hip
+++ b/crispr-hawk_amd/csrc/hawk_api.hip
@@ -140,7 +140,7 @@
   ctx->device = device;
   HIPCHK(hipStreamCreateWithFlags(&ctx->stream, hipStreamNonBlocking));
   for (auto& e : ctx->ev) HIPCHK(hipEventCreate(&e));
-  HIPCHK(hipHostMalloc(&ctx->pinned, 256, hipHostMallocDefault));
+  HIPCHK(hipHostMalloc(&ctx->pinned, HAWK_PINNED_BYTES, hipHostMallocDefault));
   g_ctx_of[device] = ctx; g_ctx_refs[device] = 1;
   *out = ctx;
   return HAWK_OK;
diff --git a/crispr-hawk_amd/csrc/hawk_api_collapse.hip b/crispr-hawk_amd/csrc/hawk_api_collapse.hip
--- a/crispr-hawk_amd/csrc/hawk_api_collapse.hip
+++ b/crispr-hawk_amd/csrc/hawk_api_collapse.hip
@@ -152,7 +152,9 @@
   hawk_hapset* hs = t->hs;
   hawk_ctx* ctx = hs->ctx;
   HIPCHK(hipSetDevice(ctx->device));
-  const hawk_xplan* vx = hs->vplan;
+  hawk_xplan* vx = hs->vplan;
+  if (vx && t->dict_gen != vx->cl.gen) return HAWK_E_INVALID;
+  if (vx) { const int rc0 = hawk_dict_resolve(vx, false, nullptr); if (rc0) return rc0; }
   if (!vx || !vx->cl.usable) return HAWK_E_INVALID;
   const uint64_t n = t->n_rows;
   if (n > 0xffffffffull) return HAWK_E_UNSUPPORTED;
diff --git a/crispr-hawk_amd/csrc/hawk_api_search.hip b/crispr-hawk_amd/csrc/hawk_api_search.hip
--- a/crispr-hawk_amd/csrc/hawk_api_search.hip
+++ b/crispr-hawk_amd/csrc/hawk_api_search.hip
@@ -25,6 +25,7 @@
 }
 
 #define HAWK_RETRY_TEMPLATES (-100)
+#define HAWK_REDO_RESOLVED (-101)
 
 enum SearchEvent {
   EV_BEGIN, EV_COUNT_DONE, EV_OFFSETS_DONE, EV_EMIT_BEGIN, EV_EMIT_END, EV_LIST_EMIT_END,
@@ -32,12 +33,15 @@
   EV_TEMPLATES_DONE, EV_REF_ROWS_PACKED,
   EV_SLOTS
 };
-static_assert(EV_SLOTS == sizeof(hawk_ctx::ev) / sizeof(hipEvent_t), "hawk_ctx::ev holds exactly the search's events");
+static_assert(EV_SLOTS == HAWK_EV_BUILD_BEGIN && HAWK_EV_BUILD_END + 1 == sizeof(hawk_ctx::ev) / sizeof(hipEvent_t),
+              "hawk_ctx::ev holds the search's events, then the two of the dictionary build");
 
 struct SearchRun {
   hawk_hapset* hs; hawk_ctx* ctx; hipStream_t st;
-  const hawk_xplan* vx;
+  hawk_xplan* vx;
   bool by_cluster;
+  bool provisional;
+  uint32_t cl_inst, cl_uniq;
   HapSetDev d; ScanParams sp; GuideParams gp; RefInfo ri; VcArgs va; ClDict cd;
   uint64_t ntile, nscan;
   uint32_t plane_tiles, v_tiles;
@@ -58,12 +62,17 @@
   if (rc) return rc;
   r->d = make_dev(hs);
   ++hs->cols_gen;
-  const hawk_xplan* vx = r->vx;
+  hawk_xplan* vx = r->vx;
   if (vx && (hs->ref_index != 0 || hs->n_ref_rows != 1)) return HAWK_E_INVALID;
-  r->by_cluster = vx && vx->cl.built && vx->cl.usable;
-  if (r->by_cluster) { const char* e = getenv("HAWK_VIEW_SEARCH"); if (e && e[0] == 'w') r->by_cluster = false; }
+  r->by_cluster = vx && vx->cl.built && (vx->cl.pending || vx->cl.usable);
+  r->provisional = r->by_cluster && vx->cl.pending;
+  if (r->by_cluster) { const char* e = getenv("HAWK_VIEW_SEARCH"); if (e && e[0] == 'w') r->by_cluster = r->provisional = false; }
+  if (vx && vx->cl.pending && !r->provisional) { const int rc2 = hawk_dict_resolve(vx, false, nullptr); if (rc2) return rc2; }
+  if (r->provisional) ++vx->q_provisional;
+  r->cl_inst = !r->by_cluster ? 0u : r->provisional ? vx->cl.q_inst_bound : vx->cl.n_inst;
+  r->cl_uniq = !r->by_cluster ? 0u : r->provisional ? vx->cl.q_u_bound : vx->cl.n_uniq;
   r->ntile = (uint64_t)hs->n_hap * r->sp.bph;
-  r->nscan = r->by_cluster ? (uint64_t)r->sp.bph + ((uint64_t)vx->cl.n_inst + 63) / 64 : r->ntile;
+  r->nscan = r->by_cluster ? (uint64_t)r->sp.bph + ((uint64_t)r->cl_inst + 63) / 64 : r->ntile;
   r->plane_tiles = vx ? r->sp.bph : (uint32_t)r->ntile;
   r->v_tiles = (uint32_t)r->ntile - r->plane_tiles;
   r->stage_cap = r->by_cluster ? 2ull * hs->hap_len[hs->ref_index] + 64 : 0;
@@ -144,15 +153,15 @@
   va.recs_ = vx->recs.p; va.alt_codes = vx->codes.as<uint8_t>(); va.hv_off = vx->off.as<uint64_t>(); va.tiles_ = vx->tiles.p;
   if (!r->by_cluster) return HAWK_OK;
   const auto& cl = vx->cl;
-  cd.n_inst = cl.n_inst; cd.n_uniq = cl.n_uniq;
+  cd.n_inst = r->cl_inst; cd.n_uniq = r->cl_uniq; cd.live = cl.live.as<uint32_t>();
   cd.inst_uid = cl.inst_uid.as<uint32_t>(); cd.inst_o = cl.inst_o.as<int32_t>(); cd.inst_row = cl.inst_row.as<uint32_t>();
   cd.inst_pa = cl.inst_pa.as<int32_t>(); cd.inst_rb = cl.inst_rb.as<int32_t>();
   cd.u_rec = cl.u_rec.as<uint32_t>(); cd.u_n = cl.u_n.as<uint32_t>(); cd.u_row = cl.u_row.as<uint32_t>(); cd.u_o = cl.u_o.as<int32_t>();
   cd.u_seg = cl.u_seg.as<uint32_t>();
   const char* e0 = getenv("HAWK_CLUSTER_ROWS0");
-  const uint64_t first = e0 ? strtoull(e0, nullptr, 10) : 16ull * cl.n_uniq + 65536;
-  r->tcap = std::max<uint64_t>(std::min<uint64_t>(cl.slots, std::max<uint64_t>(hs->cs_tcap, first)), 1);
-  const size_t n_uniq = std::max<uint32_t>(cl.n_uniq, 1), n_inst = std::max<uint32_t>(cl.n_inst, 1);
+  const uint64_t first = e0 ? strtoull(e0, nullptr, 10) : 16ull * r->cl_uniq + 65536;
+  r->tcap = std::max<uint64_t>(std::min<uint64_t>(r->provisional ? ~0ull : cl.slots, std::max<uint64_t>(hs->cs_tcap, first)), 1);
+  const size_t n_uniq = std::max<uint32_t>(r->cl_uniq, 1), n_inst = std::max<uint32_t>(r->cl_inst, 1);
   int rc;
   if ((rc = hs->cs_res.reserve(n_uniq * 32)) || (rc = hs->cs_tbase.reserve(n_uniq * 4)) || (rc = hs->cs_trows.reserve((size_t)r->tcap * hawk_cs_row_bytes())) ||
       (rc = hs->cs_itb.reserve(n_inst * 4)) || (rc = hs->cs_icnt.reserve(n_inst * 4)))
@@ -218,6 +227,13 @@
 static int search_read_block(SearchRun* r) {
   HIPCHK(hipMemcpyAsync(r->h, r->blk, sizeof(SearchStatusBlock), hipMemcpyDeviceToHost, r->st));
   HIPCHK(hipStreamSynchronize(r->st));
+  if (r->provisional) {
+    bool redo = false;
+    const int rc = hawk_dict_resolve(r->vx, true, &redo);
+    if (rc) return rc;
+    if (redo) { ++r->vx->q_redone; return HAWK_REDO_RESOLVED; }
+    ++r->vx->q_accepted;
+  }
   if (!r->by_cluster) return HAWK_OK;
   const uint64_t tcu = r->h->template_rows;
   if (tcu > r->tcap) { r->hs->cs_tcap = std::min<uint64_t>(r->vx->cl.slots, tcu + tcu / 8 + 64); return HAWK_RETRY_TEMPLATES; }
@@ -253,6 +269,7 @@
   t->n_rows = tot.n_keep; t->n_cand = tot.n_cand; t->n_hits = tot.n_hits; t->cols = tc; t->cap = tc.cap;
   t->guidelen = p->guidelen; t->pamlen = p->pamlen; t->right = p->right ? 1 : 0; t->n_groups = 0; t->collapsed = false;
   t->by_cluster = r->by_cluster; t->plane_tiles = r->plane_tiles; t->t_rows = r->by_cluster ? r->t_rows_used : 0;
+  t->dict_gen = r->by_cluster ? r->vx->cl.gen : 0;
   *out = t;
   return HAWK_OK;
 }
@@ -289,8 +306,9 @@
 
 int hawk_search(hawk_hapset* hs, const hawk_search_params* p, hawk_table** out, hawk_timing* timing) {
   int rc = hawk_search_once(hs, p, out, timing);
+  if (rc == HAWK_REDO_RESOLVED) rc = hawk_search_once(hs, p, out, timing);
   if (rc == HAWK_RETRY_TEMPLATES) rc = hawk_search_once(hs, p, out, timing);
-  return rc == HAWK_RETRY_TEMPLATES ? HAWK_E_CAPACITY : rc;
+  return rc == HAWK_RETRY_TEMPLATES || rc == HAWK_REDO_RESOLVED ? HAWK_E_CAPACITY : rc;
 }
 
 void hawk_table_destroy(hawk_table* t) {
diff --git a/crispr-hawk_amd/csrc/hawk_api_xplan.hip b/crispr-hawk_amd/csrc/hawk_api_xplan.hip
--- a/crispr-hawk_amd/csrc/hawk_api_xplan.hip
+++ b/crispr-hawk_amd/csrc/hawk_api_xplan.hip
@@ -13,7 +13,7 @@
 
 #include "hawk_host.h"
 
-enum XplanEvent { EV_KERNELS_BEGIN = 0, EV_KERNELS_END = 1, EV_BUILD_BEGIN = 8, EV_BUILD_END = 9 };
+enum XplanEvent { EV_KERNELS_BEGIN = 0, EV_KERNELS_END = 1 };
 
 extern "C" {
 
@@ -21,12 +21,13 @@
   if (!x) return;
   (void)hipSetDevice(x->ctx->device);
   (void)hipStreamSynchronize(x->ctx->stream);
+  if (x->ctx->dict_pending == x) x->ctx->dict_pending = nullptr;
   for (auto& p : x->ref_plane) hawk_pool_free(p);
   for (auto& b : x->ref5) b.release();
   DevBuf* bufs[] = {&x->recs, &x->heads, &x->tiles, &x->codes, &x->off, &x->hlen, &x->hash,
                     &x->m_is_ref, &x->m_ss, &x->m_se, &x->m_seg_off, &x->m_seg_rel, &x->m_seg_gen, &x->m_tile,
                     &x->cl.inst_uid, &x->cl.inst_o, &x->cl.inst_row, &x->cl.inst_pa, &x->cl.inst_rb, &x->cl.u_rec, &x->cl.u_n, &x->cl.u_row,
-                    &x->cl.u_o, &x->cl.u_seg};
+                    &x->cl.u_o, &x->cl.u_seg, &x->cl.live};
   for (auto* b : bufs) b->release();
   delete x;
 }
@@ -175,14 +176,19 @@
   return HAWK_OK;
 }
 
-static int xplan_build_dict(hawk_xplan* x) {
+}
+
+int hawk_dict_queue(hawk_xplan* x, bool full_table) {
   auto& cl = x->cl;
   if (cl.built) return HAWK_OK;
-  cl.built = true; cl.usable = false; cl.status = 0; cl.n_inst = cl.n_uniq = cl.n_real = 0; cl.slots = 0; cl.build_ms = 0.f;
-  hawk_ctx* ctx = x->ctx;
+  hawk_ctx* ctx = x->ctx;
+  if (ctx->dict_pending) { const int rc0 = hawk_dict_resolve(ctx->dict_pending, false, nullptr); if (rc0) return rc0; }
+  ++cl.gen;
+  cl.built = true; cl.usable = false; cl.pending = false; cl.status = 0; cl.n_inst = cl.n_uniq = cl.n_real = 0; cl.slots = 0;
+  if (!full_table) cl.build_ms = 0.f;
   hipStream_t st = ctx->stream;
   const uint32_t n = x->n_hap;
-  if (x->ncar == 0 || x->ncar >= (1ull << 32) - 2 || n < 2) { cl.status = 4; return HAWK_OK; }
+  if (x->ncar == 0 || x->ncar + n >= (1ull << 32) - 2 || n < 2) { cl.status = 4; return HAWK_OK; }
   PoolScope tmp;
   const uint32_t n_var = x->n_var;
   const uint32_t ch_bound = hawk_cl_chunk_bound(x->ncar, n);
@@ -192,12 +198,18 @@
   while (tsize < 2u * inst_bound && tsize < (1u << 30)) tsize <<= 1;
   uint32_t tsmall = std::min<uint32_t>(1u << 16, tsize);
   { const uint64_t expect = cl.last_uniq ? (uint64_t)cl.last_uniq * 2 : (uint64_t)inst_bound / 8; while (tsmall < expect && tsmall < tsize) tsmall <<= 1; }
-  const uint32_t u_bound0 = n_var + std::min<uint32_t>(tsmall, inst_bound);
+  if (const char* e0 = getenv("HAWK_CLUSTER_TABLE0")) {
+    const unsigned long long v = strtoull(e0, nullptr, 10);
+    if (v >= 2 && (v & (v - 1)) == 0) tsmall = (uint32_t)std::min<unsigned long long>(v, tsize);
+  }
+  const uint32_t tsz = full_table ? tsize : tsmall;
+  const bool small = tsz < tsize;
+  const uint32_t u_bound = n_var + std::min<uint32_t>(tsz, inst_bound);
   auto up = [](size_t v) { return (v + 255) & ~(size_t)255; };
   const size_t z_status = 0, z_counters = 256, z_results = 512, z_cnt = 768,
                z_claim = z_cnt + up(((size_t)ch_bound + 4) * 8), z_vdesc = z_claim + up((size_t)bm_words * 4),
-               z_span2 = z_vdesc + up((size_t)std::max<uint32_t>(n_var, 1) * 8), z_tab = z_span2 + up((size_t)u_bound0 * 4),
-               z_end = z_tab + (size_t)tsmall * hawk_cl_slot_bytes();
+               z_span2 = z_vdesc + up((size_t)std::max<uint32_t>(n_var, 1) * 8), z_tab = z_span2 + up((size_t)u_bound * 4),
+               z_end = z_tab + (size_t)tsz * hawk_cl_slot_bytes();
   char* d_zero;
   TEMPCHK(tmp, &d_zero, z_end);
   uint32_t* const d_status = reinterpret_cast<uint32_t*>(d_zero + z_status);
@@ -207,6 +219,8 @@
   uint32_t* const d_lcnt = d_cnt + ((ch_bound + 3) & ~3u);
   uint32_t* const d_claim = reinterpret_cast<uint32_t*>(d_zero + z_claim);
   void* const d_vdesc = d_zero + z_vdesc;
+  uint32_t* const d_span2 = reinterpret_cast<uint32_t*>(d_zero + z_span2);
+  void* const d_tab = d_zero + z_tab;
   uint32_t *d_ch_off, *d_ch_row, *d_base, *d_lbase, *d_state;
   void* d_list;
   TEMPCHK(tmp, &d_ch_off, (size_t)(n + 1) * 4);
@@ -218,14 +232,16 @@
   int rc;
   if ((rc = cl.inst_uid.reserve((size_t)inst_bound * 4)) || (rc = cl.inst_o.reserve((size_t)inst_bound * 4)) ||
       (rc = cl.inst_row.reserve((size_t)inst_bound * 4)) || (rc = cl.inst_pa.reserve((size_t)inst_bound * 4)) ||
-      (rc = cl.inst_rb.reserve((size_t)inst_bound * 4)))
+      (rc = cl.inst_rb.reserve((size_t)inst_bound * 4)) || (rc = cl.live.reserve(16)) ||
+      (rc = cl.u_rec.reserve((size_t)u_bound * 4)) || (rc = cl.u_n.reserve((size_t)u_bound * 4)) || (rc = cl.u_row.reserve((size_t)u_bound * 4)) ||
+      (rc = cl.u_o.reserve((size_t)u_bound * 4)) || (rc = cl.u_seg.reserve((size_t)u_bound * 4)))
     return rc;
   uint32_t* const t_uid = cl.inst_uid.as<uint32_t>();
   uint32_t* const t_row = cl.inst_row.as<uint32_t>();
   int32_t* const t_o = cl.inst_o.as<int32_t>();
   int32_t* const t_pa = cl.inst_pa.as<int32_t>();
   int32_t* const t_rb = cl.inst_rb.as<int32_t>();
-  HIPCHK(hipEventRecord(ctx->ev[EV_BUILD_BEGIN], st));
+  HIPCHK(hipEventRecord(ctx->ev[HAWK_EV_BUILD_BEGIN], st));
   HIPCHK(hipMemsetAsync(d_zero, 0, z_end, st));
   hawk_launch_cl_chunks(st, x->off.as<uint64_t>(), x->m_is_ref.as<uint8_t>(), x->m_ss.as<int32_t>(), x->m_se.as<int32_t>(), n, d_ch_off, d_ch_row);
   hawk_launch_cl_count(st, x->heads.p, x->off.as<uint64_t>(), x->hlen.as<uint32_t>(), x->m_ss.as<int32_t>(), x->m_se.as<int32_t>(), d_ch_off, d_ch_row, n,
@@ -233,62 +249,69 @@
   hawk_launch_scan2_u32(st, d_cnt, d_lcnt, ch_bound, d_base, d_lbase);
   const uint32_t* const d_n_inst = d_base + ch_bound;
   const uint32_t* const d_n_list = d_lbase + ch_bound;
-  unsigned long long res[8] = {0, 0, 0, 0, 0, 0, 0, 0};
-  uint32_t status = 0, n_inst = 0, n_uniq = 0, n_real = 0;
-  auto pass = [&](uint32_t tsz, uint32_t max_probe, uint32_t fail_bit, bool first) -> int {
-    const uint32_t u_bound = n_var + std::min<uint32_t>(tsz, inst_bound);
-    uint32_t* d_span2 = reinterpret_cast<uint32_t*>(d_zero + z_span2);
-    void* d_tab = d_zero + z_tab;
-    if (!first) {
-      TEMPCHK(tmp, &d_span2, (size_t)u_bound * 4);
-      TEMPCHK(tmp, &d_tab, (size_t)tsz * hawk_cl_slot_bytes());
-      HIPCHK(hipMemsetAsync(d_tab, 0, (size_t)tsz * hawk_cl_slot_bytes(), st));
-      HIPCHK(hipMemsetAsync(d_span2, 0, (size_t)u_bound * 4, st));
-      HIPCHK(hipMemsetAsync(d_zero + z_counters, 0, z_cnt - z_counters, st));
-      HIPCHK(hipMemsetAsync(d_zero + z_claim, 0, z_span2 - z_claim, st));
+  const uint32_t max_probe = small ? 64u : 0xffffffffu, fail_bit = small ? 8u : 2u;
+  hawk_launch_cl_fill(st, x->heads.p, x->off.as<uint64_t>(), x->hlen.as<uint32_t>(), x->m_ss.as<int32_t>(), x->m_se.as<int32_t>(), n, d_ch_off, d_ch_row,
+                      ch_bound, d_base, d_lbase, t_o, t_row, t_pa, t_rb, t_uid, d_vdesc, d_claim, n_var, d_list, d_status);
+  hawk_launch_cl_finish(st, inst_bound, d_n_inst, d_n_list, d_counters, d_results, n_var, u_bound, d_tab, tsz - 1, max_probe, fail_bit, d_list, d_state, d_vdesc, x->heads.p,
+                        t_uid, t_row, x->m_seg_off.as<uint32_t>(), x->m_seg_rel.as<uint32_t>(), cl.u_rec.as<uint32_t>(), cl.u_n.as<uint32_t>(),
+                        cl.u_row.as<uint32_t>(), cl.u_o.as<int32_t>(), cl.u_seg.as<uint32_t>(), d_span2, d_status, cl.live.as<uint32_t>());
+  HIPCHK(hipMemcpyAsync(static_cast<char*>(ctx->pinned) + HAWK_PINNED_DICT, d_results, 64, hipMemcpyDeviceToHost, st));
+  HIPCHK(hipEventRecord(ctx->ev[HAWK_EV_BUILD_END], st));
+  HIPCHK(hipGetLastError());
+  cl.pending = true; cl.q_small = small; cl.q_inst_bound = inst_bound; cl.q_u_bound = u_bound;
+  ctx->dict_pending = x;
+  return HAWK_OK;
+}
+
+int hawk_dict_resolve(hawk_xplan* x, bool arrived, bool* redo) {
+  auto& cl = x->cl;
+  if (redo) *redo = false;
+  if (!cl.pending) return HAWK_OK;
+  hawk_ctx* ctx = x->ctx;
+  bool repeated = false;
+  for (;;) {
+    if (!arrived) { HIPCHK(hipSetDevice(ctx->device)); HIPCHK(hipStreamSynchronize(ctx->stream)); HIPCHK(hipGetLastError()); }
+    cl.pending = false;
+    if (ctx->dict_pending == x) ctx->dict_pending = nullptr;
+    const unsigned long long* res = reinterpret_cast<const unsigned long long*>(static_cast<const char*>(ctx->pinned) + HAWK_PINNED_DICT);
+    float ms = 0.f;
+    (void)hipEventElapsedTime(&ms, ctx->ev[HAWK_EV_BUILD_BEGIN], ctx->ev[HAWK_EV_BUILD_END]);
+    cl.build_ms += ms;
+    const uint32_t status = (uint32_t)res[4];
+    if ((status & 8u) && cl.q_small && !repeated) {
+      repeated = true; arrived = false;
+      cl.built = false;
+      const int rc = hawk_dict_queue(x, true);
+      if (rc) return rc;
+      if (cl.pending) continue;
     }
-    int rc2;
-    if ((rc2 = cl.u_rec.reserve((size_t)u_bound * 4)) || (rc2 = cl.u_n.reserve((size_t)u_bound * 4)) || (rc2 = cl.u_row.reserve((size_t)u_bound * 4)) ||
-        (rc2 = cl.u_o.reserve((size_t)u_bound * 4)) || (rc2 = cl.u_seg.reserve((size_t)u_bound * 4)))
-      return rc2;
-    hawk_launch_cl_fill(st, x->heads.p, x->off.as<uint64_t>(), x->hlen.as<uint32_t>(), x->m_ss.as<int32_t>(), x->m_se.as<int32_t>(), n, d_ch_off, d_ch_row,
-                        ch_bound, d_base, d_lbase, t_o, t_row, t_pa, t_rb, t_uid, d_vdesc, d_claim, n_var, d_list, d_status);
-    hawk_launch_cl_finish(st, inst_bound, d_n_inst, d_n_list, d_counters, d_results, n_var, u_bound, d_tab, tsz - 1, max_probe, fail_bit, d_list, d_state, d_vdesc, x->heads.p,
-                          t_uid, t_row, x->m_seg_off.as<uint32_t>(), x->m_seg_rel.as<uint32_t>(), cl.u_rec.as<uint32_t>(), cl.u_n.as<uint32_t>(),
-                          cl.u_row.as<uint32_t>(), cl.u_o.as<int32_t>(), cl.u_seg.as<uint32_t>(), d_span2, d_status);
-    HIPCHK(hipMemcpyAsync(res, d_results, 64, hipMemcpyDeviceToHost, st));
-    HIPCHK(hipEventRecord(ctx->ev[EV_BUILD_END], st));
-    HIPCHK(hipStreamSynchronize(st));
-    HIPCHK(hipGetLastError());
-    n_inst = (uint32_t)res[0]; status = (uint32_t)res[4];
-    n_uniq = std::min<uint32_t>(n_var + (uint32_t)res[1], u_bound);
-    n_real = (uint32_t)(res[1] + res[2]);
-    return HAWK_OK;
-  };
-  if ((rc = pass(tsmall, tsmall < tsize ? 64u : 0xffffffffu, tsmall < tsize ? 8u : 2u, true))) return rc;
-  if (status & 8u) {
-    status &= ~8u;
-    HIPCHK(hipMemcpyAsync(d_status, &status, 4, hipMemcpyHostToDevice, st));
-    if ((rc = pass(tsize, 0xffffffffu, 2u, false))) return rc;
-  }
-  if (n_inst == 0) { cl.status = 4; return HAWK_OK; }
-  if (n_inst > inst_bound) { snprintf(hawk_hip_err_buf(), 256, "hawk_xplan_view: instance count beyond its bound"); return HAWK_E_HIP; }
-  cl.n_inst = n_inst; cl.n_uniq = n_uniq; cl.n_real = n_real; cl.last_uniq = (uint32_t)res[1];
-  (void)hipEventElapsedTime(&cl.build_ms, ctx->ev[EV_BUILD_BEGIN], ctx->ev[EV_BUILD_END]);
-  cl.slots = n_uniq ? res[3] : 0;
-  cl.status = status;
-  const char* e1 = getenv("HAWK_CLUSTER_MAX_SLOTS");
-  const char* e2 = getenv("HAWK_CLUSTER_MIN_SHARE");
-  const uint64_t max_slots = e1 ? strtoull(e1, nullptr, 10) : (1ull << 27);
-  const double min_share = e2 ? atof(e2) : 3.0;
-  if (!status && (cl.slots > max_slots || (double)n_inst < min_share * (double)std::max<uint32_t>(n_real, 1))) cl.status = 4;
+    if (redo) *redo = repeated;
+    const uint32_t n_inst = (uint32_t)res[0];
+    if (n_inst == 0) { cl.status = 4; break; }
+    if (n_inst > cl.q_inst_bound) { snprintf(hawk_hip_err_buf(), 256, "hawk_xplan_view: instance count beyond its bound"); return HAWK_E_HIP; }
+    cl.n_inst = n_inst;
+    cl.n_uniq = std::min<uint32_t>(x->n_var + (uint32_t)res[1], cl.q_u_bound);
+    cl.n_real = (uint32_t)(res[1] + res[2]); cl.last_uniq = (uint32_t)res[1];
+    cl.slots = cl.n_uniq ? res[3] : 0;
+    cl.status = status;
+    const char* e1 = getenv("HAWK_CLUSTER_MAX_SLOTS");
+    const char* e2 = getenv("HAWK_CLUSTER_MIN_SHARE");
+    const uint64_t max_slots = e1 ? strtoull(e1, nullptr, 10) : (1ull << 27);
+    const double min_share = e2 ? atof(e2) : 3.0;
+    if (!status && (cl.slots > max_slots || (double)n_inst < min_share * (double)std::max<uint32_t>(cl.n_real, 1))) cl.status = 4;
+    break;
+  }
   cl.usable = cl.status == 0;
-  return HAWK_OK;
-}
-
-int hawk_xplan_cluster_stats(const hawk_xplan* x, uint32_t* usable, uint32_t* n_instances, uint32_t* n_distinct, uint64_t* template_slots,
+  if (redo && !cl.usable) *redo = true;
+  return HAWK_OK;
+}
+
+extern "C" {
+
+int hawk_xplan_cluster_stats(hawk_xplan* x, uint32_t* usable, uint32_t* n_instances, uint32_t* n_distinct, uint64_t* template_slots,
                              float* build_ms, uint32_t* status) {
   if (!x) return HAWK_E_INVALID;
+  { const int rc = hawk_dict_resolve(x, false, nullptr); if (rc) return rc; }
   if (usable) *usable = x->cl.built && x->cl.usable ? 1u : 0u;
   if (n_instances) *n_instances = x->cl.n_inst;
   if (n_distinct) *n_distinct = x->cl.n_real;
@@ -301,8 +324,17 @@
 int hawk_xplan_cluster_rebuild(hawk_xplan* x) {
   if (!x || !x->has_meta || x->ref_index != 0) return HAWK_E_INVALID;
   HIPCHK(hipSetDevice(x->ctx->device));
+  if (x->cl.pending) { const int rc = hawk_dict_resolve(x, false, nullptr); if (rc) return rc; }
   x->cl.built = false;
-  return xplan_build_dict(x);
+  return hawk_dict_queue(x, false);
+}
+
+int hawk_xplan_queue_counters(const hawk_xplan* x, uint64_t* provisional, uint64_t* accepted, uint64_t* redone) {
+  if (!x) return HAWK_E_INVALID;
+  if (provisional) *provisional = x->q_provisional;
+  if (accepted) *accepted = x->q_accepted;
+  if (redone) *redone = x->q_redone;
+  return HAWK_OK;
 }
 
 int hawk_xplan_view(hawk_xplan* x, hawk_hapset** out) {
@@ -316,7 +348,7 @@
   for (int p = 0; p < HAWK_PLANES; ++p) hs->plane[p] = x->ref5[p].as<uint32_t>();
   rc = xplan_install(x, hs);
   if (!rc && hipStreamSynchronize(ctx->stream) != hipSuccess) rc = HAWK_E_HIP;
-  if (!rc) rc = xplan_build_dict(x);
+  if (!rc) rc = hawk_dict_queue(x, false);
   if (rc) { hs->vplan = nullptr; for (int p = 0; p < HAWK_PLANES; ++p) hs->plane[p] = nullptr; hawk_hapset_destroy(hs); return rc; }
   *out = hs;
   return HAWK_OK;
@@ -484,6 +516,8 @@
   x->scan_start.assign(scan_start, scan_start + n);
   x->scan_stop.assign(scan_stop, scan_stop + n);
   x->ref_index = 0; x->n_ref_rows = 1; x->has_meta = true; x->cl.built = false; x->cl.usable = false;
+  x->cl.pending = false;
+  if (ctx->dict_pending == x) ctx->dict_pending = nullptr;
   return HAWK_OK;
 }
 
diff --git a/crispr-hawk_amd/csrc/hawk_csearch.hip b/crispr-hawk_amd/csrc/hawk_csearch.hip
--- a/crispr-hawk_amd/csrc/hawk_csearch.hip
+++ b/crispr-hawk_amd/csrc/hawk_csearch.hip
@@ -406,8 +406,13 @@
   }
 }
 __global__ void k_cl_results(const uint32_t* __restrict__ n_inst, const uint32_t* __restrict__ counters, const unsigned long long* __restrict__ slots_total,
-                             const uint32_t* __restrict__ status, unsigned long long* __restrict__ out) {
-  out[0] = *n_inst; out[1] = counters[0]; out[2] = counters[1]; out[3] = *slots_total; out[4] = *status;
+                             const uint32_t* __restrict__ status, unsigned long long* __restrict__ out, uint32_t inst_bound, uint32_t n_var, uint32_t u_cap,
+                             uint32_t* __restrict__ live) {
+  const uint32_t ni = *n_inst, nt = counters[0], st = *status;
+  out[0] = ni; out[1] = nt; out[2] = counters[1]; out[3] = *slots_total; out[4] = st;
+  const bool whole = st == 0u && ni != 0u && ni <= inst_bound;
+  const uint32_t nu = nt < u_cap - n_var ? n_var + nt : u_cap;
+  live[0] = whole ? ni : 0u; live[1] = whole ? nu : 0u;
 }
 __global__ __launch_bounds__(256) void k_cl_uid(const ClListed* __restrict__ cx_list, const uint32_t* __restrict__ n_list_dev, uint32_t t_end,
                                                 const uint32_t* __restrict__ cx_state, const ClSlot* __restrict__ tab, uint32_t* __restrict__ inst_uid,
@@ -498,7 +503,7 @@
                            unsigned long long* results, uint32_t n_var, uint32_t u_cap, void* tab,
                            uint32_t mask, uint32_t max_probe, uint32_t fail_bit, const void* cx_list, uint32_t* cx_state, const void* var_desc,
                            const void* recs, uint32_t* inst_uid, const uint32_t* inst_row, const uint32_t* seg_off, const uint32_t* seg_rel,
-                           uint32_t* u_rec, uint32_t* u_n, uint32_t* u_row, int32_t* u_o, uint32_t* u_seg, uint32_t* u_span2, uint32_t* status) {
+                           uint32_t* u_rec, uint32_t* u_n, uint32_t* u_row, int32_t* u_o, uint32_t* u_seg, uint32_t* u_span2, uint32_t* status, uint32_t* live) {
   ClUniq cu{u_rec, u_n, u_row, u_o, u_seg, u_span2};
   const uint32_t per = 256 * CL_UID_U;
   const uint32_t head = list_bound < 16 * CL_HEAD_LISTED ? 0u : CL_HEAD_LISTED;
@@ -514,7 +519,8 @@
   if (list_bound)
     hipLaunchKernelGGL(k_cl_uid, dim3((list_bound + per - 1) / per), dim3(256), 0, st, list, n_list_dev, list_bound, cx_state, static_cast<const ClSlot*>(tab),
                        inst_uid, cu, static_cast<const HxHead*>(recs), status);
-  hipLaunchKernelGGL(k_cl_results, dim3(1), dim3(1), 0, st, n_inst_dev, counters, reinterpret_cast<const unsigned long long*>(counters + 4), status, results);
+  hipLaunchKernelGGL(k_cl_results, dim3(1), dim3(1), 0, st, n_inst_dev, counters, reinterpret_cast<const unsigned long long*>(counters + 4), status, results,
+                     list_bound, n_var, u_cap, live);
 }
 
 __device__ __forceinline__ VcRanges cs_ranges(const HapSetDev& hs, const ScanParams& p, uint32_t h) {
@@ -551,13 +557,15 @@
   __shared__ uint32_t s_k[2][256];
   __shared__ uint32_t s_e[256];
   const uint32_t tid = threadIdx.x;
+  const uint32_t n_uniq = cd.live[1];
+  if ((blockIdx.x * 256) / CS_G >= n_uniq) return;
   if (gp.score_cfdon) for (uint32_t i = tid; i < 336; i += 256) s_cfd[i] = gp.cfd_mm[i];
   __syncthreads();
   const uint32_t gl = tid & (CS_G - 1);
   const uint32_t u = (blockIdx.x * 256 + tid) / CS_G;
-  const uint32_t nc_u = u < cd.n_uniq ? cd.u_n[u] : 0u;
+  const uint32_t nc_u = u < n_uniq ? cd.u_n[u] : 0u;
   const bool live = nc_u != 0u;
-  const bool hole = u < cd.n_uniq && !live;
+  const bool hole = u < n_uniq && !live;
   const HxVar* __restrict__ recs = static_cast<const HxVar*>(va.recs_);
   const uint32_t h = live ? cd.u_row[u] : 0u, r0 = live ? cd.u_rec[u] : 0u, nc = live ? nc_u : 1u;
   const uint32_t seg0 = live ? cd.u_seg[u] : hs.seg_off[0], seg_end = hs.seg_off[h + 1];
@@ -856,13 +864,14 @@
   const uint32_t i0 = blockIdx.x * (256 * CS_CNT_U) + threadIdx.x;
   const uint32_t lane = threadIdx.x & (WAVE - 1);
   const bool ovf = *t_count > t_cap;
+  const uint32_t n_inst = cd.live[0], n_uniq = cd.live[1];
   uint32_t uid[CS_CNT_U], below[CS_CNT_U];
   int32_t paf[CS_CNT_U];
   bool in[CS_CNT_U];
 #pragma unroll
   for (int u = 0; u < CS_CNT_U; ++u) {
     const uint32_t i = i0 + u * 256;
-    in[u] = i < cd.n_inst;
+    in[u] = i < n_inst;
     const uint32_t ic = in[u] ? i : 0u;
     uid[u] = cd.inst_uid[ic]; paf[u] = cd.inst_pa[ic];
     below[u] = CL_NONE;
@@ -874,7 +883,7 @@
   for (int u = 0; u < CS_CNT_U; ++u) {
     const bool has = in[u] && uid[u] != CL_NONE;
     r[u] = make_uint4(0u, 0u, 0u, 0u); r2[u] = r[u]; behind0[u] = 0u;
-    if (cd.n_uniq) {
+    if (n_uniq) {
       const uint32_t us = has ? uid[u] : 0u;
       r[u] = res[2 * us]; r2[u] = res[2 * us + 1];
       if (lane == 0 && below[u] != CL_NONE) behind0[u] = res[2 * below[u] + 1].z;
@@ -927,7 +936,7 @@
   __builtin_nontemporal_store(v.z, q + 2); __builtin_nontemporal_store(v.w, q + 3);
 }
 template <int NI, int CE_CH>
-__global__ __launch_bounds__(256) void k_cs_emit_rows(uint32_t n_inst, const uint32_t* __restrict__ inst_row, const int32_t* __restrict__ inst_o,
+__global__ __launch_bounds__(256) void k_cs_emit_rows(const uint32_t* __restrict__ live, const uint32_t* __restrict__ inst_row, const int32_t* __restrict__ inst_o,
                                                       const uint32_t* __restrict__ counts, const uint32_t* __restrict__ inst_tb,
                                                       const CsRow* __restrict__ trows, const uint64_t* __restrict__ offsets,
                                                       const unsigned long long* __restrict__ t_count, uint64_t t_cap, uint4* __restrict__ rows,
@@ -940,6 +949,7 @@
   __shared__ uint32_t s_src[4][2][CE_CH], s_rh[4][2][CE_CH];
   __shared__ int32_t s_rdq[4][2][CE_CH];
   if (*t_count > t_cap) return;
+  const uint32_t n_inst = live[0];
   const uint32_t wv = threadIdx.x / WAVE, lane = threadIdx.x & (WAVE - 1);
   const uint32_t i0 = (blockIdx.x * 4 + wv) * NE;
   if (i0 >= n_inst) return;
@@ -1018,7 +1028,7 @@
                               const unsigned long long* t_count, uint64_t t_cap, void* rows, uint64_t cap, int* status) {
   if (!cd.n_inst) return;
   constexpr int NI = 4, CH = 256;
-  hipLaunchKernelGGL((k_cs_emit_rows<NI, CH>), dim3((cd.n_inst + 256 * NI - 1) / (256 * NI)), dim3(256), 0, st, cd.n_inst, cd.inst_row, cd.inst_o, counts,
+  hipLaunchKernelGGL((k_cs_emit_rows<NI, CH>), dim3((cd.n_inst + 256 * NI - 1) / (256 * NI)), dim3(256), 0, st, cd.live, cd.inst_row, cd.inst_o, counts,
                      inst_tb, static_cast<const CsRow*>(trows), offsets, t_count, t_cap, static_cast<uint4*>(rows), cap, status);
 }
 
diff --git a/crispr-hawk_amd/csrc/hawk_device.h b/crispr-hawk_amd/csrc/hawk_device.h
--- a/crispr-hawk_amd/csrc/hawk_device.h
+++ b/crispr-hawk_amd/csrc/hawk_device.h
@@ -117,6 +117,7 @@
 void hawk_launch_ref_hits(hipStream_t st, const HapSetDev& hs, const ScanParams& p, int32_t ref_index, void* hp);
 struct ClDict {
   uint32_t n_inst, n_uniq;
+  const uint32_t* live;
   const uint32_t* inst_uid;
   const int32_t* inst_o;
   const uint32_t* inst_row;
@@ -149,7 +150,7 @@
                            void* tab , uint32_t mask, uint32_t max_probe, uint32_t fail_bit, const void* cx_list, uint32_t* cx_state,
                            const void* var_desc, const void* recs, uint32_t* inst_uid, const uint32_t* inst_row, const uint32_t* seg_off,
                            const uint32_t* seg_rel, uint32_t* u_rec, uint32_t* u_n, uint32_t* u_row, int32_t* u_o, uint32_t* u_seg, uint32_t* u_span2,
-                           uint32_t* status);
+                           uint32_t* status, uint32_t* live );
 void hawk_launch_cs_templates(hipStream_t st, const HapSetDev& hs, const VcArgs& va, const ClDict& cd, const ScanParams& p, const struct GuideParams& gp,
                               const struct RefInfo& ri, void* res , uint32_t* tbase, void* trows,
                               unsigned long long* t_count, uint64_t t_cap, int* status);
diff --git a/crispr-hawk_amd/csrc/hawk_host.h b/crispr-hawk_amd/csrc/hawk_host.h
--- a/crispr-hawk_amd/csrc/hawk_host.h
+++ b/crispr-hawk_amd/csrc/hawk_host.h
@@ -24,9 +24,11 @@
 struct hawk_ctx {
   int device;
   hipStream_t stream;
-  hipEvent_t ev[10];
+  hipEvent_t ev[12];
   void* pinned = nullptr;
-};
+  struct hawk_xplan* dict_pending = nullptr;
+};
+enum { HAWK_EV_BUILD_BEGIN = 10, HAWK_EV_BUILD_END = 11, HAWK_PINNED_DICT = 256, HAWK_PINNED_BYTES = 512 };
 
 struct SearchStatusBlock {
   int status;
@@ -121,7 +123,7 @@
   DevBuf refbits;
   bool refbits_valid = false;
   uint64_t refbits_key[6] = {0, 0, 0, 0, 0, 0};
-  const struct hawk_xplan* vplan = nullptr;
+  struct hawk_xplan* vplan = nullptr;
   DevBuf vcnt0;
   DevBuf refhp;
   uint64_t cs_tcap = 0;
@@ -163,8 +165,16 @@
     uint32_t status = 0;
     float build_ms = 0.f;
     DevBuf inst_uid, inst_o, inst_row, inst_pa, inst_rb, u_rec, u_n, u_row, u_o, u_seg;
+    bool pending = false;
+    uint64_t gen = 0;
+    bool q_small = false;
+    uint32_t q_inst_bound = 0, q_u_bound = 0;
+    DevBuf live;
   } cl;
-};
+  uint64_t q_provisional = 0, q_accepted = 0, q_redone = 0;
+};
+int hawk_dict_queue(hawk_xplan* x, bool full_table);
+int hawk_dict_resolve(hawk_xplan* x, bool arrived, bool* redo);
 
 struct hawk_gt {
   hawk_ctx* ctx;
@@ -192,6 +202,7 @@
   uint64_t gen;
   DevBuf own[8];
   bool by_cluster = false;
+  uint64_t dict_gen = 0;
   uint32_t plane_tiles = 0;
   uint64_t t_rows = 0;
 };
diff --git a/include/hawk.h b/include/hawk.h
--- a/include/hawk.h
+++ b/include/hawk.h
@@ -70,9 +70,10 @@
 void hawk_xplan_destroy(hawk_xplan* x);
 int hawk_xplan_text(hawk_xplan* x, uint32_t n_rows, const uint32_t* rows, const uint64_t* out_off, char* out, float* kernel_ms);
 int hawk_xplan_view(hawk_xplan* x, hawk_hapset** out);
-int hawk_xplan_cluster_stats(const hawk_xplan* x, uint32_t* usable, uint32_t* n_instances, uint32_t* n_distinct, uint64_t* template_slots,
+int hawk_xplan_cluster_stats(hawk_xplan* x, uint32_t* usable, uint32_t* n_instances, uint32_t* n_distinct, uint64_t* template_slots,
                              float* build_ms, uint32_t* status);
 int hawk_xplan_cluster_rebuild(hawk_xplan* x);
+int hawk_xplan_queue_counters(const hawk_xplan* x, uint64_t* provisional, uint64_t* accepted, uint64_t* redone);
 
 int hawk_pam_scan(hawk_hapset* hs, uint64_t pam_fwd, uint64_t pam_rev, uint32_t pamlen, uint32_t* hits_fwd,
                   uint32_t* hits_rev, uint64_t cap_fwd, uint64_t cap_rev, uint64_t* off_fwd, uint64_t* off_rev);
```

After: 568.8 billion, median of 4. About the same (+1.2%).
